# JosephCatrambone/pixelbox

Measured on NVIDIA B200. Metric: corpus_GB_per_s_scanned, higher is better.
Workload: dtype u8 x s16 -> int32 (IDP.2A), f32 replay on candidates

## Files before the change

include/pixelbox_b200.h:

```cpp
#ifndef PIXELBOX_B200_H
#define PIXELBOX_B200_H

#include <stddef.h>
#include <stdint.h>

#ifdef __cplusplus
extern "C" {
#endif

#if defined(_WIN32)
#define PBX_API __declspec(dllexport)
#else
#define PBX_API __attribute__((visibility("default")))
#endif

#define PBX_OK 0
#define PBX_E_INVALID (-1)
#define PBX_E_DIM (-2)
#define PBX_E_OOM (-3)
#define PBX_E_CUDA (-4)
#define PBX_E_NO_DEVICE (-5)
#define PBX_E_CAPACITY (-6)
#define PBX_E_K (-7)
#define PBX_E_INTERNAL (-8)

#define PBX_MAX_DIM 4096u
#define PBX_MAX_K 2048u
#define PBX_MAX_ROWS 0xFFFFF000ull
#define PBX_MAX_SHARDS 64u

#define PBX_COUNT_EXCHANGE_TIMEOUT 0xFFFFFFFFu
#define PBX_COUNT_EXACT_LAUNCH_FAILED 0xFFFFFFFEu
#define PBX_COUNT_FILTER_UNSORTED 0xFFFFFFFDu

#define PBX_FILTER_INCLUDE 0u
#define PBX_FILTER_EXCLUDE 1u

#define PBX_DEFAULT_MAX_DIST 1e3
#define PBX_DEFAULT_K 100u

typedef struct pbx_corpus pbx_corpus;

typedef struct pbx_hit {
    int64_t image_id;
    float dist;
    int32_t dot;
    int32_t norm2;
    uint32_t flags;
} pbx_hit;

typedef struct pbx_stats {
    uint64_t rows;
    uint64_t capacity_rows;
    uint32_t dim;
    uint32_t row_pitch;
    uint64_t queries;
    uint64_t exact_passes;
    float last_search_ms;
    float last_scan_ms;
    uint64_t last_bytes_scanned;
    int32_t device;
    int32_t sm_count;
    int32_t scan_grid;
    int32_t reserved;
    uint64_t batched_queries;
} pbx_stats;

PBX_API int pbx_corpus_create(uint32_t dim, uint64_t capacity_hint, int device, pbx_corpus** out);
PBX_API void pbx_corpus_destroy(pbx_corpus* c);

PBX_API int pbx_corpus_load(pbx_corpus* c, const int64_t* image_ids, const uint8_t* hashes, uint64_t n);

PBX_API int pbx_corpus_append(pbx_corpus* c, const int64_t* image_ids, const uint8_t* hashes, uint64_t n);
PBX_API int pbx_corpus_flush(pbx_corpus* c);
PBX_API int pbx_corpus_append_device(pbx_corpus* c, const int64_t* d_image_ids, const uint8_t* d_hashes, uint64_t n, void* cuda_stream);

PBX_API int pbx_corpus_remove(pbx_corpus* c, const int64_t* image_ids, uint64_t n, uint64_t* out_removed);

PBX_API int pbx_corpus_fill_synthetic(pbx_corpus* c, uint64_t n, uint64_t seed, uint64_t first_row);

PBX_API int pbx_corpus_size(const pbx_corpus* c, uint64_t* n_rows);
PBX_API int pbx_corpus_dim(const pbx_corpus* c, uint32_t* dim);

PBX_API int pbx_corpus_read_rows(const pbx_corpus* c, uint64_t first, uint64_t n, int64_t* image_ids, uint8_t* hashes);

PBX_API int pbx_corpus_synchronize(pbx_corpus* c);

PBX_API int pbx_search(pbx_corpus* c, const uint8_t* queries, uint32_t nq, uint32_t k, double max_dist,
                       int64_t* out_ids, float* out_dist, int32_t* out_dot, int32_t* out_norm2,
                       uint32_t* out_count);

PBX_API int pbx_search_hits(pbx_corpus* c, const uint8_t* queries, uint32_t nq, uint32_t k, double max_dist,
                            pbx_hit* out_hits, uint32_t* out_count);

PBX_API int pbx_search_device(pbx_corpus* c, const uint8_t* d_queries, uint32_t nq, uint32_t k, double max_dist,
                              pbx_hit* d_hits, uint32_t* d_count, void* cuda_stream);

PBX_API int pbx_search_filtered(pbx_corpus* c, const uint8_t* queries, uint32_t nq, uint32_t k, double max_dist,
                                int64_t* out_ids, float* out_dist, int32_t* out_dot, int32_t* out_norm2, uint32_t* out_count,
                                const int64_t* filter_ids, uint64_t n_filter, uint32_t filter_mode);
PBX_API int pbx_search_device_filtered(pbx_corpus* c, const uint8_t* d_queries, uint32_t nq, uint32_t k, double max_dist,
                                       pbx_hit* d_hits, uint32_t* d_count, void* cuda_stream,
                                       const int64_t* d_filter_ids, uint64_t n_filter, uint32_t filter_mode);

PBX_API int pbx_merge_hits(const pbx_hit* gathered, const uint32_t* counts, uint32_t n_shards, uint32_t nq, uint32_t k,
                           pbx_hit* out_hits, uint32_t* out_count);

PBX_API int pbx_merge_hits_device(int device, const pbx_hit* d_gathered, const uint32_t* d_counts, uint32_t n_shards,
                                  uint32_t nq, uint32_t k, pbx_hit* d_out_hits, uint32_t* d_out_count, void* cuda_stream);

typedef struct pbx_sharded pbx_sharded;
PBX_API int pbx_sharded_create(uint32_t dim, uint64_t capacity_hint, const int* devices, int n_devices, pbx_sharded** out);
PBX_API void pbx_sharded_destroy(pbx_sharded* s);
PBX_API int pbx_sharded_load(pbx_sharded* s, const int64_t* image_ids, const uint8_t* hashes, uint64_t n);
PBX_API int pbx_sharded_append(pbx_sharded* s, const int64_t* image_ids, const uint8_t* hashes, uint64_t n);
PBX_API int pbx_sharded_remove(pbx_sharded* s, const int64_t* image_ids, uint64_t n, uint64_t* out_removed);
PBX_API int pbx_sharded_fill_synthetic(pbx_sharded* s, uint64_t rows_per_shard, uint64_t seed);
PBX_API int pbx_sharded_size(const pbx_sharded* s, uint64_t* n_rows);
PBX_API int pbx_sharded_shards(const pbx_sharded* s, uint32_t* n_shards);
PBX_API int pbx_sharded_shard(pbx_sharded* s, uint32_t index, pbx_corpus** out);
PBX_API int pbx_sharded_search(pbx_sharded* s, const uint8_t* queries, uint32_t nq, uint32_t k, double max_dist,
                               int64_t* out_ids, float* out_dist, int32_t* out_dot, int32_t* out_norm2, uint32_t* out_count);
PBX_API int pbx_sharded_search_hits(pbx_sharded* s, const uint8_t* queries, uint32_t nq, uint32_t k, double max_dist,
                                    pbx_hit* out_hits, uint32_t* out_count);
PBX_API int pbx_sharded_search_filtered(pbx_sharded* s, const uint8_t* queries, uint32_t nq, uint32_t k, double max_dist,
                                        int64_t* out_ids, float* out_dist, int32_t* out_dot, int32_t* out_norm2, uint32_t* out_count,
                                        const int64_t* filter_ids, uint64_t n_filter, uint32_t filter_mode);

typedef struct pbx_exchange pbx_exchange;
PBX_API int pbx_exchange_create(int device, uint32_t rank, uint32_t world, uint32_t max_records, uint32_t max_queries,
                                pbx_exchange** out);
PBX_API int pbx_exchange_handle(pbx_exchange* x, void* out_handle_64_bytes);
PBX_API int pbx_exchange_connect(pbx_exchange* x, const void* all_handles );
PBX_API int pbx_exchange_allgather_merge(pbx_exchange* x, const pbx_hit* d_local, uint32_t nq, uint32_t k, pbx_hit* d_out,
                                         uint32_t* d_out_count, void* cuda_stream);
PBX_API int pbx_exchange_search_hits(pbx_exchange* x, pbx_corpus* c, const uint8_t* queries, uint32_t nq, uint32_t k, double max_dist,
                                     pbx_hit* out_hits, uint32_t* out_count);
PBX_API int pbx_exchange_search_hits_filtered(pbx_exchange* x, pbx_corpus* c, const uint8_t* queries, uint32_t nq, uint32_t k,
                                              double max_dist, pbx_hit* out_hits, uint32_t* out_count,
                                              const int64_t* filter_ids, uint64_t n_filter, uint32_t filter_mode);
PBX_API void pbx_exchange_destroy(pbx_exchange* x);

PBX_API int pbx_cosine_distance_pairs(int device, const uint8_t* a, const uint8_t* b, uint64_t n, uint32_t dim,
                                      float* out_dist, int32_t* out_dot, int32_t* out_norm2_a, int32_t* out_norm2_b);

PBX_API int pbx_byte_distance_pairs(int device, const uint8_t* a, const uint8_t* b, uint64_t n, uint32_t dim,
                                    float* out_dist, uint32_t* out_l1);
PBX_API int pbx_hamming_distance_pairs(int device, const uint8_t* a, const uint8_t* b, uint64_t n, uint32_t dim,
                                       float* out_dist, uint32_t* out_bits);

PBX_API int pbx_quantize(int device, const float* embeddings, uint64_t n, uint8_t* out);
PBX_API int pbx_quantize_device(int device, const float* d_embeddings, uint64_t n, uint8_t* d_out, void* cuda_stream);

PBX_API int pbx_get_stats(const pbx_corpus* c, pbx_stats* out);
PBX_API int pbx_set_candidate_slack(pbx_corpus* c, uint32_t slack);
PBX_API int pbx_set_profiling(pbx_corpus* c, int enabled);
PBX_API int pbx_set_batch_min(pbx_corpus* c, uint32_t min_queries);
PBX_API int pbx_set_scan_ctas_per_sm(pbx_corpus* c, uint32_t ctas_per_sm);
PBX_API int pbx_int8_peak(int device, double* out_tops);
PBX_API const char* pbx_last_error(void);
PBX_API const char* pbx_version(void);
PBX_API int pbx_device_count(void);

#ifdef __cplusplus
}
#endif
#endif
```

pixelbox_b200/_native.py:

```python
from __future__ import annotations

import ctypes
import os

import numpy as np

HERE = os.path.dirname(os.path.abspath(__file__))
SO_PATH = os.environ.get("PBX_SO", os.path.join(HERE, "lib", "libpixelbox_b200.so"))

PBX_OK = 0
ERROR_NAMES = {
    -1: "PBX_E_INVALID", -2: "PBX_E_DIM", -3: "PBX_E_OOM", -4: "PBX_E_CUDA", -5: "PBX_E_NO_DEVICE",
    -6: "PBX_E_CAPACITY", -7: "PBX_E_K", -8: "PBX_E_INTERNAL",
}
PBX_MAX_DIM = 4096
PBX_MAX_K = 2048
DEFAULT_MAX_DIST = 1e3
DEFAULT_K = 100
PBX_FILTER_INCLUDE = 0
PBX_FILTER_EXCLUDE = 1
PBX_COUNT_FILTER_UNSORTED = 0xFFFFFFFD

EXPORTS = [
    "pbx_corpus_create", "pbx_corpus_destroy", "pbx_corpus_load", "pbx_corpus_append", "pbx_corpus_flush", "pbx_corpus_append_device",
    "pbx_quantize_device", "pbx_corpus_fill_synthetic", "pbx_corpus_remove", "pbx_sharded_remove",
    "pbx_corpus_size", "pbx_corpus_dim", "pbx_corpus_read_rows", "pbx_corpus_synchronize", "pbx_search", "pbx_search_hits", "pbx_search_device",
    "pbx_search_filtered", "pbx_search_device_filtered", "pbx_sharded_search_filtered", "pbx_exchange_search_hits_filtered",
    "pbx_merge_hits", "pbx_merge_hits_device", "pbx_exchange_create", "pbx_exchange_handle", "pbx_exchange_connect",
    "pbx_exchange_allgather_merge", "pbx_exchange_search_hits", "pbx_exchange_destroy",
    "pbx_sharded_create", "pbx_sharded_destroy", "pbx_sharded_load", "pbx_sharded_append", "pbx_sharded_fill_synthetic", "pbx_sharded_size",
    "pbx_sharded_shards", "pbx_sharded_shard", "pbx_sharded_search", "pbx_sharded_search_hits", "pbx_cosine_distance_pairs", "pbx_byte_distance_pairs", "pbx_hamming_distance_pairs", "pbx_quantize", "pbx_get_stats", "pbx_set_candidate_slack",
    "pbx_set_profiling", "pbx_set_batch_min", "pbx_set_scan_ctas_per_sm", "pbx_int8_peak", "pbx_last_error", "pbx_version", "pbx_device_count",
]

HIT_DTYPE = np.dtype([("image_id", "<i8"), ("dist", "<f4"), ("dot", "<i4"), ("norm2", "<i4"), ("flags", "<u4")], align=True)
assert HIT_DTYPE.itemsize == 24


class PbxStats(ctypes.Structure):
    _fields_ = [
        ("rows", ctypes.c_uint64), ("capacity_rows", ctypes.c_uint64), ("dim", ctypes.c_uint32),
        ("row_pitch", ctypes.c_uint32), ("queries", ctypes.c_uint64), ("exact_passes", ctypes.c_uint64),
        ("last_search_ms", ctypes.c_float), ("last_scan_ms", ctypes.c_float), ("last_bytes_scanned", ctypes.c_uint64),
        ("device", ctypes.c_int32), ("sm_count", ctypes.c_int32), ("scan_grid", ctypes.c_int32), ("reserved", ctypes.c_int32),
        ("batched_queries", ctypes.c_uint64),
    ]


class PbxError(RuntimeError):
    def __init__(self, code: int, message: str):
        self.code = code
        self.name = ERROR_NAMES.get(code, f"PBX_E_{code}")
        super().__init__(f"{self.name}: {message}")


_lib = None


def lib() -> ctypes.CDLL:
    global _lib
    if _lib is not None:
        return _lib
    if not os.path.exists(SO_PATH):
        raise ImportError(f"{SO_PATH} is missing: build it with `python -m pixelbox_b200.build` "
                          "(nvcc, sm_100a). pixelbox_b200 has no CPU or PyTorch fallback.")
    L = ctypes.CDLL(SO_PATH)
    vp, u8p = ctypes.c_void_p, ctypes.c_void_p
    u32, u64, i32, f64 = ctypes.c_uint32, ctypes.c_uint64, ctypes.c_int, ctypes.c_double
    sig = {
        "pbx_corpus_create": (i32, [u32, u64, i32, ctypes.POINTER(vp)]),
        "pbx_corpus_destroy": (None, [vp]),
        "pbx_corpus_load": (i32, [vp, vp, u8p, u64]),
        "pbx_corpus_append": (i32, [vp, vp, u8p, u64]),
        "pbx_corpus_flush": (i32, [vp]),
        "pbx_corpus_append_device": (i32, [vp, vp, vp, u64, vp]),
        "pbx_quantize_device": (i32, [i32, vp, u64, vp, vp]),
        "pbx_corpus_fill_synthetic": (i32, [vp, u64, u64, u64]),
        "pbx_corpus_remove": (i32, [vp, vp, u64, ctypes.POINTER(u64)]),
        "pbx_sharded_remove": (i32, [vp, vp, u64, ctypes.POINTER(u64)]),
        "pbx_corpus_size": (i32, [vp, ctypes.POINTER(u64)]),
        "pbx_corpus_dim": (i32, [vp, ctypes.POINTER(u32)]),
        "pbx_corpus_read_rows": (i32, [vp, u64, u64, vp, u8p]),
        "pbx_corpus_synchronize": (i32, [vp]),
        "pbx_search": (i32, [vp, u8p, u32, u32, f64, vp, vp, vp, vp, vp]),
        "pbx_search_hits": (i32, [vp, u8p, u32, u32, f64, vp, vp]),
        "pbx_search_device": (i32, [vp, vp, u32, u32, f64, vp, vp, vp]),
        "pbx_search_filtered": (i32, [vp, u8p, u32, u32, f64, vp, vp, vp, vp, vp, vp, u64, u32]),
        "pbx_search_device_filtered": (i32, [vp, vp, u32, u32, f64, vp, vp, vp, vp, u64, u32]),
        "pbx_merge_hits": (i32, [vp, vp, u32, u32, u32, vp, vp]),
        "pbx_merge_hits_device": (i32, [i32, vp, vp, u32, u32, u32, vp, vp, vp]),
        "pbx_exchange_create": (i32, [i32, u32, u32, u32, u32, ctypes.POINTER(vp)]),
        "pbx_exchange_handle": (i32, [vp, vp]),
        "pbx_exchange_connect": (i32, [vp, vp]),
        "pbx_exchange_allgather_merge": (i32, [vp, vp, u32, u32, vp, vp, vp]),
        "pbx_exchange_search_hits": (i32, [vp, vp, u8p, u32, u32, f64, vp, vp]),
        "pbx_exchange_search_hits_filtered": (i32, [vp, vp, u8p, u32, u32, f64, vp, vp, vp, u64, u32]),
        "pbx_exchange_destroy": (None, [vp]),
        "pbx_sharded_create": (i32, [u32, u64, vp, i32, ctypes.POINTER(vp)]),
        "pbx_sharded_destroy": (None, [vp]),
        "pbx_sharded_load": (i32, [vp, vp, u8p, u64]),
        "pbx_sharded_append": (i32, [vp, vp, u8p, u64]),
        "pbx_sharded_fill_synthetic": (i32, [vp, u64, u64]),
        "pbx_sharded_size": (i32, [vp, ctypes.POINTER(u64)]),
        "pbx_sharded_shards": (i32, [vp, ctypes.POINTER(u32)]),
        "pbx_sharded_shard": (i32, [vp, u32, ctypes.POINTER(vp)]),
        "pbx_sharded_search": (i32, [vp, u8p, u32, u32, f64, vp, vp, vp, vp, vp]),
        "pbx_sharded_search_hits": (i32, [vp, u8p, u32, u32, f64, vp, vp]),
        "pbx_sharded_search_filtered": (i32, [vp, u8p, u32, u32, f64, vp, vp, vp, vp, vp, vp, u64, u32]),
        "pbx_cosine_distance_pairs": (i32, [i32, u8p, u8p, u64, u32, vp, vp, vp, vp]),
        "pbx_byte_distance_pairs": (i32, [i32, u8p, u8p, u64, u32, vp, vp]),
        "pbx_hamming_distance_pairs": (i32, [i32, u8p, u8p, u64, u32, vp, vp]),
        "pbx_quantize": (i32, [i32, vp, u64, u8p]),
        "pbx_get_stats": (i32, [vp, ctypes.POINTER(PbxStats)]),
        "pbx_set_candidate_slack": (i32, [vp, u32]),
        "pbx_set_profiling": (i32, [vp, i32]),
        "pbx_set_batch_min": (i32, [vp, u32]),
        "pbx_set_scan_ctas_per_sm": (i32, [vp, u32]),
        "pbx_int8_peak": (i32, [i32, ctypes.POINTER(ctypes.c_double)]),
        "pbx_last_error": (ctypes.c_char_p, []),
        "pbx_version": (ctypes.c_char_p, []),
        "pbx_device_count": (i32, []),
    }
    for name, (res, args) in sig.items():
        fn = getattr(L, name)
        fn.restype = res
        fn.argtypes = args
    _lib = L
    return L


def check(rc: int) -> None:
    if rc != PBX_OK:
        raise PbxError(rc, lib().pbx_last_error().decode("utf-8", "replace"))


def filter_args(within, excluding):
    if within is not None and excluding is not None:
        raise ValueError("pass `within` or `excluding`, not both")
    ids = within if within is not None else excluding
    ids = np.ascontiguousarray(np.asarray(ids, dtype=np.int64)).reshape(-1)
    return ids, (PBX_FILTER_INCLUDE if within is not None else PBX_FILTER_EXCLUDE)


def ptr(a) -> ctypes.c_void_p:
    if a is None:
        return ctypes.c_void_p(0)
    return ctypes.c_void_p(a.ctypes.data)
```

pixelbox_b200/csrc/api.cu:

```cuda
#include <atomic>
#include <algorithm>
#include <cmath>
#include <cstdarg>
#include <cstdio>
#include <cstdlib>
#include <cstring>
#include <limits>
#include <mutex>
#include <new>
#include <type_traits>
#include <vector>

#include "finalize.cuh"
#include "batch.cuh"
#include "remove.cuh"

using namespace pbx;

static thread_local char g_err[512] = "";

static int fail(int code, const char* fmt, ...) {
    va_list ap;
    va_start(ap, fmt);
    vsnprintf(g_err, sizeof(g_err), fmt, ap);
    va_end(ap);
    return code;
}

#define CU_TRY(expr)                                                                               \
    do {                                                                                           \
        cudaError_t e__ = (expr);                                                                  \
        if (e__ != cudaSuccess)                                                                    \
            return fail(e__ == cudaErrorMemoryAllocation ? PBX_E_OOM : PBX_E_CUDA, "%s failed: %s (%s:%d)", #expr, \
                        cudaGetErrorString(e__), __FILE__, __LINE__);                              \
    } while (0)

struct VmmApi {
    CUresult (*reserve)(CUdeviceptr*, size_t, size_t, CUdeviceptr, unsigned long long) = nullptr;
    CUresult (*free_)(CUdeviceptr, size_t) = nullptr;
    CUresult (*create)(CUmemGenericAllocationHandle*, size_t, const CUmemAllocationProp*, unsigned long long) = nullptr;
    CUresult (*release)(CUmemGenericAllocationHandle) = nullptr;
    CUresult (*map)(CUdeviceptr, size_t, size_t, CUmemGenericAllocationHandle, unsigned long long) = nullptr;
    CUresult (*unmap)(CUdeviceptr, size_t) = nullptr;
    CUresult (*set_access)(CUdeviceptr, size_t, const CUmemAccessDesc*, size_t) = nullptr;
    CUresult (*granularity)(size_t*, const CUmemAllocationProp*, CUmemAllocationGranularity_flags) = nullptr;
    bool ok = false;
};
static const VmmApi& vmm_api() {
    static VmmApi api;
    static std::once_flag once;
    std::call_once(once, [] {
        if (getenv("PBX_NO_VMM")) return;
        cudaDriverEntryPointQueryResult q;
        auto get = [&](const char* name, void** fn) { return cudaGetDriverEntryPoint(name, fn, cudaEnableDefault, &q) == cudaSuccess && *fn != nullptr; };
        api.ok = get("cuMemAddressReserve", (void**)&api.reserve) && get("cuMemAddressFree", (void**)&api.free_) && get("cuMemCreate", (void**)&api.create) &&
                 get("cuMemRelease", (void**)&api.release) && get("cuMemMap", (void**)&api.map) && get("cuMemUnmap", (void**)&api.unmap) &&
                 get("cuMemSetAccess", (void**)&api.set_access) && get("cuMemGetAllocationGranularity", (void**)&api.granularity);
        cudaGetLastError();
    });
    return api;
}
struct VmmArray {
    CUdeviceptr base = 0;
    size_t reserved = 0, mapped = 0, gran = 0;
    std::vector<std::pair<CUmemGenericAllocationHandle, size_t>> chunks;
};
static CUmemAllocationProp vmm_prop(int device) {
    CUmemAllocationProp prop = {};
    prop.type = CU_MEM_ALLOCATION_TYPE_PINNED;
    prop.location.type = CU_MEM_LOCATION_TYPE_DEVICE;
    prop.location.id = device;
    return prop;
}
static bool vmm_reserve(VmmArray& a, int device, size_t bytes) {
    const VmmApi& api = vmm_api();
    const CUmemAllocationProp prop = vmm_prop(device);
    if (api.granularity(&a.gran, &prop, CU_MEM_ALLOC_GRANULARITY_RECOMMENDED) != CUDA_SUCCESS || a.gran == 0) return false;
    a.reserved = (bytes + a.gran - 1) / a.gran * a.gran;
    return api.reserve(&a.base, a.reserved, 0, 0, 0) == CUDA_SUCCESS;
}
static int vmm_grow(VmmArray& a, int device, size_t need, size_t* from, size_t* to) {
    *from = *to = a.mapped;
    if (need <= a.mapped) return PBX_OK;
    if (need > a.reserved) return fail(PBX_E_CAPACITY, "shard outgrew the address range reserved for it (%zu > %zu bytes)", need, a.reserved);
    const VmmApi& api = vmm_api();
    const size_t add = (need - a.mapped + a.gran - 1) / a.gran * a.gran;
    const CUmemAllocationProp prop = vmm_prop(device);
    CUmemGenericAllocationHandle h;
    CUresult r = api.create(&h, add, &prop, 0);
    if (r != CUDA_SUCCESS) return fail(PBX_E_OOM, "cannot back %zu more bytes on device %d (cuMemCreate: %d)", add, device, (int)r);
    r = api.map(a.base + a.mapped, add, 0, h, 0);
    if (r == CUDA_SUCCESS) {
        CUmemAccessDesc acc = {};
        acc.location.type = CU_MEM_LOCATION_TYPE_DEVICE;
        acc.location.id = device;
        acc.flags = CU_MEM_ACCESS_FLAGS_PROT_READWRITE;
        r = api.set_access(a.base + a.mapped, add, &acc, 1);
        if (r != CUDA_SUCCESS) api.unmap(a.base + a.mapped, add);
    }
    if (r != CUDA_SUCCESS) { api.release(h); return fail(PBX_E_CUDA, "mapping %zu bytes failed (%d)", add, (int)r); }
    a.chunks.emplace_back(h, add);
    *to = a.mapped + add;
    a.mapped += add;
    return PBX_OK;
}
static void vmm_release(VmmArray& a) {
    const VmmApi& api = vmm_api();
    if (a.base) {
        if (a.mapped) api.unmap(a.base, a.mapped);
        for (auto& c : a.chunks) api.release(c.first);
        api.free_(a.base, a.reserved);
    }
    a = VmmArray();
}

struct pbx_corpus {
    int device = 0;
    int sm_count = 0;
    uint32_t dim = 0, pitch = 0, pitch16 = 0;
    std::atomic<uint64_t> n{0};
    std::atomic<uint64_t> capacity{0};
    uint8_t* d_rows = nullptr;
    float* d_inv = nullptr;
    int* d_rsum = nullptr;
    float4* d_bmeta = nullptr;
    bool use_vmm = false;
    VmmArray v_rows, v_inv, v_rsum, v_ids, v_bmeta;
    uint64_t reserved_rows = 0;
    std::vector<uint8_t> pend_rows;
    std::vector<int64_t> pend_ids;
    std::atomic<uint64_t> pending{0};
    int64_t* d_ids = nullptr;

    cudaStream_t stream = nullptr;
    cudaStream_t copy_stream = nullptr;
    cudaEvent_t ev_chain = nullptr;
    cudaEvent_t ev_t0 = nullptr, ev_t1 = nullptr;
    cudaEvent_t ev_s0 = nullptr, ev_s1 = nullptr;
    float last_scan_ms = 0.f;
    bool chain_valid = false;

    uint32_t max_nq = 0;
    uint8_t* d_queries = nullptr;
    int16_t* d_q16 = nullptr;
    uint8_t* d_qbytes = nullptr;
    QueryHeader* d_qh = nullptr;
    SearchStatus* d_status = nullptr;
    unsigned char* d_split = nullptr;
    bool split_finalize = true;
    size_t split_min_bytes = 256u * 1024u;
    pbx_hit* d_hits = nullptr;
    size_t hits_cap = 0;
    void* d_cand = nullptr;
    size_t cand_bytes = 0;
    uint32_t* d_cand_cnt = nullptr;
    uint32_t* d_tile_counter = nullptr;
    uint32_t* d_hist = nullptr;
    unsigned long long* d_exact_passes = nullptr;
    uint32_t* d_allow = nullptr;
    size_t allow_words = 0;
    u64* d_filter_words = nullptr;
    int64_t* d_filter_ids = nullptr;
    size_t filter_ids_cap = 0;
    const uint32_t* cur_allow = nullptr;
    const u64* cur_allowed = nullptr;
    uint8_t* h_queries = nullptr;
    size_t h_queries_cap = 0;
    pbx_hit* h_hits = nullptr;
    size_t h_hits_cap = 0;
    bool zero_copy = true;
    uint32_t* h_flag = nullptr;
    uint32_t flag_seq = 0;
    uint32_t* cur_done_flag = nullptr;
    uint32_t cur_done_seq = 0;
    uint8_t* h_stage = nullptr;
    size_t h_stage_cap = 0, stage_rows = 0;
    cudaEvent_t ev_stage[2] = {nullptr, nullptr};

    std::mutex mu;
    std::mutex append_mu;
    std::mutex grow_mu;
    cudaStream_t grow_stream = nullptr;

    uint32_t slack = 0;
    uint32_t ctas_per_sm = 0;
    uint64_t queries = 0;
    float last_search_ms = 0.f;
    uint64_t last_bytes = 0;
    int last_grid = 0;
    uint32_t last_n = 0;
    uint64_t rows_generation = 0;
    uint32_t batch_pad = 0;
    uint8_t* d_qpad = nullptr;
    int* d_colterm = nullptr;
    float* d_thr = nullptr;
    uint32_t* d_bcnt = nullptr;
    uint32_t* d_boverflow = nullptr;
    u64* d_bcand = nullptr;
    uint32_t batch_cap = 0;
    uint32_t* d_bhist = nullptr;
    float* d_binvq = nullptr;
    float* d_seedlb = nullptr;
    CUtensorMap map_rows, map_q;
    uint64_t map_rows_gen = ~0ull;
    uint32_t map_q_pad = 0, map_q_box = 0, map_rows_box = 0;
    uint32_t batch_cg = 0;

    uint32_t batch_min = 2;
    uint64_t batched_queries = 0;
    bool scan_timed = false;
    bool profiling = false;
};

constexpr size_t kStageMinRows = 2048;
static int ensure_stage(pbx_corpus* c, size_t rows_per_slot);

static uint32_t default_keep(uint32_t k, uint32_t slack) {
    uint32_t s = slack ? slack : std::max<uint32_t>(156u, k / 4u);
    uint32_t keep = k + s;
    if (!slack) keep = (keep + 31u) & ~31u;
    return std::min<uint32_t>(keep, kMaxKeep);
}

static uint32_t batch_keep(uint32_t k, uint32_t slack) {
    if (slack) return std::min<uint32_t>(k + slack, kMaxKeep);
    const uint32_t keep = (k + std::max<uint32_t>(28u, k / 4u) + 31u) & ~31u;
    return std::min<uint32_t>(keep, kMaxKeep);
}

static float certificate_margin(uint32_t dim) {
    return (float)((4.0 * dim + 3232.0) * std::ldexp(1.0, -24));
}

static int free_corpus_buffers(pbx_corpus* c) {
    if (c->use_vmm) {
        vmm_release(c->v_rows); vmm_release(c->v_inv); vmm_release(c->v_rsum); vmm_release(c->v_ids); vmm_release(c->v_bmeta);
        c->d_rows = nullptr; c->d_inv = nullptr; c->d_ids = nullptr; c->d_rsum = nullptr; c->d_bmeta = nullptr;
        c->capacity = 0;
        c->use_vmm = false;
        return PBX_OK;
    }
    cudaFree(c->d_rows); cudaFree(c->d_inv); cudaFree(c->d_ids); cudaFree(c->d_rsum); cudaFree(c->d_bmeta);
    c->d_rows = nullptr; c->d_inv = nullptr; c->d_ids = nullptr; c->d_rsum = nullptr; c->d_bmeta = nullptr;
    c->capacity = 0;
    return PBX_OK;
}

static int reserve_rows_vmm(pbx_corpus* c, uint64_t want) {
    struct Arr { VmmArray* a; size_t elem; } arrs[5] = {{&c->v_rows, (size_t)c->pitch}, {&c->v_inv, sizeof(float)}, {&c->v_rsum, sizeof(int)},
                                                        {&c->v_ids, sizeof(int64_t)}, {&c->v_bmeta, sizeof(float4)}};
    for (int i = 0; i < 5; ++i) {
        const size_t need = i == 4 ? (size_t)(want / 32) * arrs[i].elem : (size_t)want * arrs[i].elem;
        size_t from = 0, to = 0;
        int rc = vmm_grow(*arrs[i].a, c->device, need, &from, &to);
        if (rc != PBX_OK) return rc;
        if (to > from) CU_TRY(cudaMemsetAsync(reinterpret_cast<void*>(arrs[i].a->base + from), 0, to - from, c->grow_stream));
    }
    CU_TRY(cudaStreamSynchronize(c->grow_stream));
    c->capacity = want;
    return PBX_OK;
}

static int reserve_rows(pbx_corpus* c, uint64_t rows) {
    if (rows <= c->capacity) return PBX_OK;
    if (rows > PBX_MAX_ROWS) return fail(PBX_E_CAPACITY, "shard would hold %llu rows (max %llu)", (unsigned long long)rows, (unsigned long long)PBX_MAX_ROWS);
    const uint64_t cap_now = c->capacity.load();
    uint64_t want = std::max<uint64_t>(rows, cap_now + cap_now / 2);
    if (cap_now) want = std::max<uint64_t>(want, cap_now + (32u << 20) / c->pitch);
    want = (want + kTileRows - 1) / kTileRows * kTileRows;
    if (c->use_vmm) {
        want = std::min<uint64_t>(want, c->reserved_rows);
        if (rows > c->reserved_rows) return fail(PBX_E_CAPACITY, "shard would hold %llu rows; its address range was reserved for %llu", (unsigned long long)rows, (unsigned long long)c->reserved_rows);
        int rc = reserve_rows_vmm(c, want);
        if (rc != PBX_OK && want > rows) {
            want = (rows + kTileRows - 1) / kTileRows * kTileRows;
            rc = reserve_rows_vmm(c, want);
        }
        return rc;
    }
    uint8_t* nr = nullptr; float* ni = nullptr; int64_t* nid = nullptr; int* ns = nullptr; float4* nb = nullptr;
    auto alloc_all = [&](uint64_t rows_) {
        cudaError_t e_ = cudaMalloc(&nr, rows_ * c->pitch);
        if (e_ == cudaSuccess) e_ = cudaMalloc(&ni, rows_ * sizeof(float));
        if (e_ == cudaSuccess) e_ = cudaMalloc(&nid, rows_ * sizeof(int64_t));
        if (e_ == cudaSuccess) e_ = cudaMalloc(&ns, rows_ * sizeof(int));
        if (e_ == cudaSuccess) e_ = cudaMalloc(&nb, rows_ / 32 * sizeof(float4));
        return e_;
    };
    auto free_all = [&]() {
        cudaFree(nr); cudaFree(ni); cudaFree(nid); cudaFree(ns); cudaFree(nb);
        nr = nullptr; ni = nullptr; nid = nullptr; ns = nullptr; nb = nullptr;
        cudaGetLastError();
    };
    cudaError_t e = alloc_all(want);
    if (e != cudaSuccess && want > rows) {
        free_all();
        want = (rows + kTileRows - 1) / kTileRows * kTileRows;
        e = alloc_all(want);
    }
    if (e != cudaSuccess) {
        free_all();
        return fail(PBX_E_OOM, "cannot allocate %llu rows x %u bytes on device %d: %s", (unsigned long long)want, c->pitch, c->device, cudaGetErrorString(e));
    }
    const uint64_t n = c->n.load();
    e = cudaDeviceSynchronize();
    if (e == cudaSuccess && n) {
        e = cudaMemcpyAsync(nr, c->d_rows, n * c->pitch, cudaMemcpyDeviceToDevice, c->stream);
        if (e == cudaSuccess) e = cudaMemcpyAsync(ni, c->d_inv, n * sizeof(float), cudaMemcpyDeviceToDevice, c->stream);
        if (e == cudaSuccess) e = cudaMemcpyAsync(nid, c->d_ids, n * sizeof(int64_t), cudaMemcpyDeviceToDevice, c->stream);
        if (e == cudaSuccess) e = cudaMemcpyAsync(ns, c->d_rsum, n * sizeof(int), cudaMemcpyDeviceToDevice, c->stream);
    }
// ... 47 lines not shown
        CU_TRY(cudaMalloc(&c->d_hits, need * sizeof(pbx_hit)));
        c->hits_cap = need;
    }
    if (need > c->h_hits_cap) {
        cudaFreeHost(c->h_hits);
        c->h_hits = nullptr; c->h_hits_cap = 0;
        CU_TRY(cudaMallocHost(&c->h_hits, need * sizeof(pbx_hit)));
        c->h_hits_cap = need;
    }
    return PBX_OK;
}

static int ensure_cand(pbx_corpus* c, size_t bytes) {
    if (bytes <= c->cand_bytes) return PBX_OK;
    CU_TRY(cudaDeviceSynchronize());
    cudaFree(c->d_cand); c->d_cand = nullptr; c->cand_bytes = 0;
    CU_TRY(cudaMalloc(&c->d_cand, bytes));
    c->cand_bytes = bytes;
    return PBX_OK;
}

static int ensure_filter_scratch(pbx_corpus* c, size_t words, uint64_t n_ids) {
    if (!c->d_filter_words) CU_TRY(cudaMalloc(&c->d_filter_words, 2 * sizeof(u64)));
    if (words > c->allow_words) {
        words = std::max(words, c->allow_words + c->allow_words / 2);
        CU_TRY(cudaDeviceSynchronize());
        cudaFree(c->d_allow); c->d_allow = nullptr; c->allow_words = 0;
        CU_TRY(cudaMalloc(&c->d_allow, words * sizeof(uint32_t)));
        c->allow_words = words;
    }
    if (n_ids > c->filter_ids_cap) {
        const uint64_t want = std::max<uint64_t>(n_ids, c->filter_ids_cap + c->filter_ids_cap / 2);
        CU_TRY(cudaDeviceSynchronize());
        cudaFree(c->d_filter_ids); c->d_filter_ids = nullptr; c->filter_ids_cap = 0;
        CU_TRY(cudaMalloc(&c->d_filter_ids, want * sizeof(int64_t)));
        c->filter_ids_cap = want;
    }
    return PBX_OK;
}

template <typename Kern>
static cudaError_t allow_smem(Kern kern, size_t bytes) {
    return cudaFuncSetAttribute(kern, cudaFuncAttributeMaxDynamicSharedMemorySize, (int)bytes);
}
constexpr uint64_t kBatchMaxRows = 0x7FFFF000ull;
constexpr uint32_t kBatchSegTilesLarge = 98304;
constexpr uint32_t kBatchSeedTiles = 256;
constexpr size_t kBatchSmemLimit = 232448 - 1024;
static cudaError_t init_kernel_attributes() {
    const size_t scan_cap = 8192 * sizeof(KeyX) + PBX_MAX_DIM * 2 + 1024;
    const size_t fin_cap = 200 * 1024;
    cudaError_t e = cudaSuccess;
#define PBX_ALLOW(LL, CC)                                                                                       \
    if (e == cudaSuccess) e = allow_smem(scan_kernel<LL, CC, false>, scan_cap);                                 \
    if (e == cudaSuccess) e = allow_smem(scan_kernel<LL, CC, false, scan_minb(LL * CC), false, true>, scan_cap); \
    if (e == cudaSuccess) e = allow_smem(scan_kernel<LL, CC, true>, scan_cap);
    PBX_ALLOW(1, 1) PBX_ALLOW(2, 1) PBX_ALLOW(4, 1) PBX_ALLOW(8, 1) PBX_ALLOW(16, 1) PBX_ALLOW(32, 1) PBX_ALLOW(32, 2) PBX_ALLOW(32, 4)
#undef PBX_ALLOW
#define PBX_ALLOW_M(LL, CC, MM)                                                                   \
    if (e == cudaSuccess) e = allow_smem(scan_kernel<LL, CC, false, MM>, scan_cap);               \
    if (e == cudaSuccess) e = allow_smem(scan_kernel<LL, CC, false, MM, false, true>, scan_cap);  \
    if (e == cudaSuccess) e = allow_smem(scan_kernel<LL, CC, true, MM>, scan_cap);
    PBX_EXTRA_SHAPES(PBX_ALLOW_M)
#undef PBX_ALLOW_M
#define PBX_ALLOW_R(LL, CC, MM)                                                                  \
    if (e == cudaSuccess) e = allow_smem(scan_kernel<LL, CC, false, MM, true>, scan_cap);        \
    if (e == cudaSuccess) e = allow_smem(scan_kernel<LL, CC, false, MM, true, true>, scan_cap);
    PBX_RAGGED_SHAPES(PBX_ALLOW_R)
#undef PBX_ALLOW_R
    if (e == cudaSuccess) e = allow_smem(scan_kernel<16, 1, false, 3>, scan_cap);
    if (e == cudaSuccess) e = allow_smem(scan_kernel<16, 1, false, 4>, scan_cap);
    if (e == cudaSuccess) e = allow_smem(scan_kernel<16, 1, false, 3, false, true>, scan_cap);
    if (e == cudaSuccess) e = allow_smem(scan_kernel<16, 1, false, 4, false, true>, scan_cap);
    if (e == cudaSuccess) e = allow_smem(scan_generic_kernel<false>, scan_cap);
    if (e == cudaSuccess) e = allow_smem(scan_generic_kernel<true>, scan_cap);
    if (e == cudaSuccess) e = allow_smem(prep_seed_kernel, PBX_MAX_DIM * 2 + 1024);
    if (e == cudaSuccess) e = allow_smem(finalize_kernel<false>, fin_cap);
    if (e == cudaSuccess) e = allow_smem(replay_kernel, (size_t)PBX_MAX_DIM * 6 + (size_t)kReplayRows * (kReplaySlice16 + 2) * 16);
    if (e == cudaSuccess) e = allow_smem(finalize_kernel<true>, fin_cap);
    if (e == cudaSuccess) e = allow_smem(batch_mma_kernel<1, false>, kBatchSmemLimit);
    if (e == cudaSuccess) e = allow_smem(batch_mma_kernel<1, true>, kBatchSmemLimit);
    if (e == cudaSuccess) e = allow_smem(batch_mma_kernel<2, false>, kBatchSmemLimit);
    if (e == cudaSuccess) e = allow_smem(batch_mma_kernel<2, true>, kBatchSmemLimit);
    if (e == cudaSuccess) e = allow_smem(batch_finalize_kernel, batch_finalize_smem(1024));
    if (e == cudaSuccess) e = allow_smem(batch_seed_select_kernel, (size_t)kBatchSeedTiles * 8u * sizeof(u64));
    if (e == cudaSuccess) e = allow_smem(batch_tighten_kernel, kBatchCapLarge * sizeof(u64));
    if (e == cudaSuccess) e = allow_smem(finalize_exact_kernel, fin_cap);
    return e;
}

extern "C" int pbx_device_count(void) {
    int n = 0;
    if (cudaGetDeviceCount(&n) != cudaSuccess) { cudaGetLastError(); return 0; }
    int ok = 0;
    for (int d = 0; d < n; ++d) {
        int major = 0;
        if (cudaDeviceGetAttribute(&major, cudaDevAttrComputeCapabilityMajor, d) == cudaSuccess && major == 10) ok++;
    }
    return ok;
}

extern "C" const char* pbx_last_error(void) { return g_err; }
extern "C" const char* pbx_version(void) { return "pixelbox_b200 0.1.0 (sm_100a)"; }

extern "C" int pbx_corpus_create(uint32_t dim, uint64_t capacity_hint, int device, pbx_corpus** out) {
    if (!out) return fail(PBX_E_INVALID, "out is NULL");
    *out = nullptr;
    if (dim == 0 || dim > PBX_MAX_DIM) return fail(PBX_E_DIM, "dim %u outside [1, %u]", dim, PBX_MAX_DIM);
    int ndev = 0;
    if (cudaGetDeviceCount(&ndev) != cudaSuccess || ndev == 0) {
        cudaGetLastError();
        return fail(PBX_E_NO_DEVICE, "no CUDA device visible: pixelbox_b200 has no CPU fallback");
    }
    if (device < 0 || device >= ndev) return fail(PBX_E_INVALID, "device %d out of range (have %d)", device, ndev);
    int major = 0, minor = 0;
    CU_TRY(cudaDeviceGetAttribute(&major, cudaDevAttrComputeCapabilityMajor, device));
    CU_TRY(cudaDeviceGetAttribute(&minor, cudaDevAttrComputeCapabilityMinor, device));
    if (major != 10) return fail(PBX_E_NO_DEVICE, "device %d is sm_%d%d; this library is built for sm_100a (B200) only", device, major, minor);
    CU_TRY(cudaSetDevice(device));
    pbx_corpus* c = new (std::nothrow) pbx_corpus();
    if (!c) return fail(PBX_E_OOM, "host allocation failed");
    c->device = device;
    c->dim = dim;
    c->split_finalize = getenv("PBX_NO_SPLIT_FINALIZE") == nullptr;
    if (const char* e = getenv("PBX_SPLIT_MIN_BYTES")) c->split_min_bytes = (size_t)atoll(e);
    c->zero_copy = getenv("PBX_NO_ZEROCOPY") == nullptr;
    if (const char* e = getenv("PBX_BATCH_CG")) c->batch_cg = atoi(e) == 1 ? 1u : (atoi(e) == 2 ? 2u : 0u);
    c->pitch = (dim + 15u) & ~15u;
    c->pitch16 = c->pitch / 16u;
    cudaDeviceGetAttribute(&c->sm_count, cudaDevAttrMultiProcessorCount, device);
    cudaError_t e = cudaStreamCreateWithFlags(&c->stream, cudaStreamNonBlocking);
    if (e == cudaSuccess) e = cudaStreamCreateWithFlags(&c->copy_stream, cudaStreamNonBlocking);
    if (e == cudaSuccess) e = cudaStreamCreateWithFlags(&c->grow_stream, cudaStreamNonBlocking);
    if (e == cudaSuccess) e = cudaEventCreateWithFlags(&c->ev_chain, cudaEventDisableTiming);
    if (e == cudaSuccess) e = cudaEventCreate(&c->ev_t0);
    if (e == cudaSuccess) e = cudaEventCreate(&c->ev_t1);
    if (e == cudaSuccess) e = cudaEventCreate(&c->ev_s0);
    if (e == cudaSuccess) e = cudaEventCreate(&c->ev_s1);
    if (e == cudaSuccess) e = cudaEventCreateWithFlags(&c->ev_stage[0], cudaEventDisableTiming);
    if (e == cudaSuccess) e = cudaEventCreateWithFlags(&c->ev_stage[1], cudaEventDisableTiming);
    if (e == cudaSuccess) e = init_kernel_attributes();
    if (e == cudaSuccess) {
        size_t cur = 0;
        if (cudaDeviceGetLimit(&cur, cudaLimitDevRuntimePendingLaunchCount) == cudaSuccess && cur < 8192)
            e = cudaDeviceSetLimit(cudaLimitDevRuntimePendingLaunchCount, 8192);
    }
    if (e == cudaSuccess) e = cudaMallocHost(&c->h_flag, 64);
    if (e == cudaSuccess) *c->h_flag = 0;
    if (e == cudaSuccess) e = cudaMalloc(&c->d_cand_cnt, kMaxScanGrid * sizeof(uint32_t));
    if (e == cudaSuccess) e = cudaMalloc(&c->d_tile_counter, 512);
    if (e == cudaSuccess) e = cudaMemset(c->d_tile_counter, 0, 512);
    if (e == cudaSuccess) e = cudaMalloc(&c->d_hist, 2 * kHistBins * sizeof(uint32_t));
    if (e == cudaSuccess) e = cudaMemset(c->d_hist, 0, 2 * kHistBins * sizeof(uint32_t));
    if (e == cudaSuccess) { c->d_exact_passes = reinterpret_cast<unsigned long long*>(reinterpret_cast<char*>(c->d_tile_counter) + 256); }
    if (e != cudaSuccess) {
        int rc = fail(PBX_E_CUDA, "corpus setup failed: %s", cudaGetErrorString(e));
        pbx_corpus_destroy(c);
        return rc;
    }
    if (vmm_api().ok) {
        size_t free_b = 0, total_b = 0;
        cudaMemGetInfo(&free_b, &total_b);
        const uint64_t per_row = (uint64_t)c->pitch + 4 + 4 + 8 + 1;
        uint64_t max_rows = std::min<uint64_t>(PBX_MAX_ROWS, std::max<uint64_t>((uint64_t)total_b / per_row, capacity_hint) + kTileRows);
        max_rows = (max_rows + kTileRows - 1) / kTileRows * kTileRows;
        c->use_vmm = vmm_reserve(c->v_rows, device, max_rows * c->pitch) && vmm_reserve(c->v_inv, device, max_rows * sizeof(float)) &&
                     vmm_reserve(c->v_rsum, device, max_rows * sizeof(int)) && vmm_reserve(c->v_ids, device, max_rows * sizeof(int64_t)) &&
                     vmm_reserve(c->v_bmeta, device, max_rows / 32 * sizeof(float4));
        if (c->use_vmm) {
            c->reserved_rows = max_rows;
            c->d_rows = reinterpret_cast<uint8_t*>(c->v_rows.base); c->d_inv = reinterpret_cast<float*>(c->v_inv.base);
            c->d_rsum = reinterpret_cast<int*>(c->v_rsum.base); c->d_ids = reinterpret_cast<int64_t*>(c->v_ids.base);
            c->d_bmeta = reinterpret_cast<float4*>(c->v_bmeta.base);
        } else {
            vmm_release(c->v_rows); vmm_release(c->v_inv); vmm_release(c->v_rsum); vmm_release(c->v_ids); vmm_release(c->v_bmeta);
        }
    }
    {
        std::lock_guard<std::mutex> lk(c->mu);
        int rc = reserve_rows(c, std::max<uint64_t>(capacity_hint, 1));
        if (rc == PBX_OK) rc = ensure_stage(c, kStageMinRows);
        if (rc != PBX_OK) { pbx_corpus_destroy(c); return rc; }
    }
    *out = c;
    return PBX_OK;
}

extern "C" void pbx_corpus_destroy(pbx_corpus* c) {
    if (!c) return;
    cudaSetDevice(c->device);
    cudaDeviceSynchronize();
    free_corpus_buffers(c);
    cudaFree(c->d_queries); cudaFree(c->d_q16); cudaFree(c->d_qbytes); cudaFree(c->d_qh); cudaFree(c->d_status); cudaFree(c->d_split);
    cudaFree(c->d_qpad); cudaFree(c->d_colterm); cudaFree(c->d_thr); cudaFree(c->d_bcnt); cudaFree(c->d_boverflow); cudaFree(c->d_bcand);
    cudaFree(c->d_bhist); cudaFree(c->d_binvq); cudaFree(c->d_seedlb);
    cudaFree(c->d_hits); cudaFree(c->d_cand); cudaFree(c->d_cand_cnt); cudaFree(c->d_tile_counter); cudaFree(c->d_hist);
    cudaFree(c->d_allow); cudaFree(c->d_filter_words); cudaFree(c->d_filter_ids);
    cudaFreeHost(c->h_queries); cudaFreeHost(c->h_hits); cudaFreeHost(c->h_stage); cudaFreeHost(c->h_flag);
    if (c->ev_chain) cudaEventDestroy(c->ev_chain);
    if (c->ev_t0) cudaEventDestroy(c->ev_t0);
    if (c->ev_t1) cudaEventDestroy(c->ev_t1);
    if (c->ev_s0) cudaEventDestroy(c->ev_s0);
    if (c->ev_s1) cudaEventDestroy(c->ev_s1);
    if (c->ev_stage[0]) cudaEventDestroy(c->ev_stage[0]);
    if (c->ev_stage[1]) cudaEventDestroy(c->ev_stage[1]);
    if (c->stream) cudaStreamDestroy(c->stream);
    if (c->copy_stream) cudaStreamDestroy(c->copy_stream);
    if (c->grow_stream) cudaStreamDestroy(c->grow_stream);
    cudaGetLastError();
    delete c;
}

extern "C" int pbx_corpus_size(const pbx_corpus* c, uint64_t* n_rows) {
    if (!c || !n_rows) return fail(PBX_E_INVALID, "NULL argument");
    *n_rows = c->n.load() + c->pending.load(std::memory_order_acquire);
    return PBX_OK;
}
extern "C" int pbx_corpus_synchronize(pbx_corpus* c) {
    if (!c) return fail(PBX_E_INVALID, "corpus is NULL");
    CU_TRY(cudaSetDevice(c->device));
    CU_TRY(cudaStreamSynchronize(c->stream));
    return PBX_OK;
}
extern "C" int pbx_corpus_dim(const pbx_corpus* c, uint32_t* dim) {
    if (!c || !dim) return fail(PBX_E_INVALID, "NULL argument");
    *dim = c->dim;
    return PBX_OK;
}

static int ensure_stage(pbx_corpus* c, size_t rows_per_slot) {
    const size_t per_row = (size_t)c->pitch + sizeof(int64_t);
    const size_t need = rows_per_slot * per_row * 2;
    if (c->h_stage_cap >= need) return PBX_OK;
    CU_TRY(cudaStreamSynchronize(c->copy_stream));
    cudaFreeHost(c->h_stage); c->h_stage = nullptr; c->h_stage_cap = 0; c->stage_rows = 0;
    CU_TRY(cudaMallocHost(&c->h_stage, need));
    c->h_stage_cap = need;
    c->stage_rows = rows_per_slot;
    return PBX_OK;
}

static int upload_rows(pbx_corpus* c, uint64_t at, const int64_t* ids, const uint8_t* hashes, uint64_t n) {
    const size_t max_stage_rows = std::max<size_t>(kStageMinRows, (size_t)(8u << 20) / c->pitch);
    const size_t per_row = (size_t)c->pitch + sizeof(int64_t);
    {
        size_t want = kStageMinRows;
        while (want < n && want < max_stage_rows) want *= 2;
        int rc0 = ensure_stage(c, std::min(want, max_stage_rows));
        if (rc0 != PBX_OK) return rc0;
    }
    const size_t stage_rows = c->stage_rows;
    cudaEvent_t* done = c->ev_stage;
    int rc = PBX_OK;
    uint64_t off = 0;
    int slot = 0;
    bool used[2] = {false, false};
    while (off < n && rc == PBX_OK) {
        const uint64_t m = std::min<uint64_t>(stage_rows, n - off);
        uint8_t* hs = c->h_stage + (size_t)slot * stage_rows * per_row;
        int64_t* hid = reinterpret_cast<int64_t*>(hs + stage_rows * c->pitch);
        if (used[slot]) cudaEventSynchronize(done[slot]);
        if (c->pitch == c->dim) {
            memcpy(hs, hashes + off * c->dim, m * c->dim);
        } else {
            memset(hs, 0, m * c->pitch);
            for (uint64_t r = 0; r < m; ++r) memcpy(hs + r * c->pitch, hashes + (off + r) * c->dim, c->dim);
        }
        memcpy(hid, ids + off, m * sizeof(int64_t));
        cudaError_t e = cudaMemcpyAsync(c->d_rows + (at + off) * c->pitch, hs, m * c->pitch, cudaMemcpyHostToDevice, c->copy_stream);
        if (e == cudaSuccess) e = cudaMemcpyAsync(c->d_ids + at + off, hid, m * sizeof(int64_t), cudaMemcpyHostToDevice, c->copy_stream);
        if (e == cudaSuccess) {
            const unsigned warps_per_block = 8;
            const unsigned blocks = (unsigned)((m + warps_per_block - 1) / warps_per_block);
            row_meta_kernel<<<blocks, warps_per_block * 32, 0, c->copy_stream>>>(reinterpret_cast<const uint4*>(c->d_rows), c->pitch16, c->dim,
                                                                                at + off, m, c->d_inv, c->d_rsum);
            e = cudaGetLastError();
        }
        if (e == cudaSuccess) e = cudaEventRecord(done[slot], c->copy_stream);
        if (e != cudaSuccess) rc = fail(PBX_E_CUDA, "row upload failed: %s", cudaGetErrorString(e));
        used[slot] = true;
        slot ^= 1;
        off += m;
    }
    if (rc == PBX_OK && n) {
        const uint64_t b0 = at / 32, b1 = (at + n + 31) / 32;
        block_meta_kernel<<<(unsigned)((b1 - b0 + 7) / 8), 256, 0, c->copy_stream>>>(c->d_inv, c->d_rsum, c->dim, b0, b1 - b0, at + n, c->d_bmeta);
        if (cudaGetLastError() != cudaSuccess) rc = fail(PBX_E_CUDA, "block metadata launch failed");
    }
    cudaError_t e = cudaStreamSynchronize(c->copy_stream);
    if (rc == PBX_OK && e != cudaSuccess) rc = fail(PBX_E_CUDA, "row upload failed: %s", cudaGetErrorString(e));
    return rc;
}

static int append_locked(pbx_corpus* c, const int64_t* image_ids, const uint8_t* hashes, uint64_t n) {
    CU_TRY(cudaSetDevice(c->device));
    const uint64_t at = c->n.load();
    if (at + n > c->capacity) {
        int rc;
        if (c->use_vmm) {
            rc = grow_mapped(c, at + n);
        } else {
            std::lock_guard<std::mutex> lk(c->mu);
            rc = reserve_rows(c, at + n);
        }
        if (rc != PBX_OK) return rc;
    }
    int rc = upload_rows(c, at, image_ids, hashes, n);
// ... 82 lines not shown
    if (n && (!image_ids || !hashes)) return fail(PBX_E_INVALID, "NULL ids or hashes with n > 0");
    std::lock_guard<std::mutex> alk(c->append_mu);
    {
        std::lock_guard<std::mutex> lk(c->mu);
        CU_TRY(cudaSetDevice(c->device));
        CU_TRY(cudaDeviceSynchronize());
        c->n.store(0);
        c->pend_ids.clear(); c->pend_rows.clear(); c->pending.store(0);
    }
    return n ? append_locked(c, image_ids, hashes, n) : PBX_OK;
}

extern "C" int pbx_corpus_fill_synthetic(pbx_corpus* c, uint64_t n, uint64_t seed, uint64_t first_row) {
    if (!c) return fail(PBX_E_INVALID, "corpus is NULL");
    std::lock_guard<std::mutex> alk(c->append_mu);
    std::lock_guard<std::mutex> lk(c->mu);
    CU_TRY(cudaSetDevice(c->device));
    CU_TRY(cudaDeviceSynchronize());
    c->n.store(0);
    c->pend_ids.clear(); c->pend_rows.clear(); c->pending.store(0);
    int rc = c->use_vmm ? grow_mapped(c, std::max<uint64_t>(n, 1)) : reserve_rows(c, std::max<uint64_t>(n, 1));
    if (rc != PBX_OK) return rc;
    if (n == 0) return PBX_OK;
    const uint64_t step = 1ull << 24;
    for (uint64_t off = 0; off < n; off += step) {
        const uint64_t m = std::min<uint64_t>(step, n - off);
        synth_fill_kernel<<<c->sm_count * 8, 256, 0, c->stream>>>(c->d_rows, c->pitch, c->dim, off, m, seed, first_row + off, c->d_ids);
        const unsigned blocks = (unsigned)((m + 7) / 8);
        row_meta_kernel<<<blocks, 256, 0, c->stream>>>(reinterpret_cast<const uint4*>(c->d_rows), c->pitch16, c->dim, off, m, c->d_inv, c->d_rsum);
        const uint64_t b0 = off / 32, b1 = (off + m + 31) / 32;
        block_meta_kernel<<<(unsigned)((b1 - b0 + 7) / 8), 256, 0, c->stream>>>(c->d_inv, c->d_rsum, c->dim, b0, b1 - b0, off + m, c->d_bmeta);
    }
    CU_TRY(cudaGetLastError());
    CU_TRY(cudaStreamSynchronize(c->stream));
    c->n.store(n);
    return PBX_OK;
}

extern "C" int pbx_corpus_read_rows(const pbx_corpus* cc, uint64_t first, uint64_t n, int64_t* image_ids, uint8_t* hashes) {
    pbx_corpus* c = const_cast<pbx_corpus*>(cc);
    if (!c) return fail(PBX_E_INVALID, "corpus is NULL");
    { int frc = flush_pending(c); if (frc != PBX_OK) return frc; }
    const uint64_t size_now = c->n.load();
    if (n > size_now || first > size_now - n) return fail(PBX_E_INVALID, "rows [%llu, %llu) outside the corpus", (unsigned long long)first, (unsigned long long)(first + n));
    if (n == 0) return PBX_OK;
    std::lock_guard<std::mutex> lk(c->mu);
    CU_TRY(cudaSetDevice(c->device));
    if (image_ids) CU_TRY(cudaMemcpy(image_ids, c->d_ids + first, n * sizeof(int64_t), cudaMemcpyDeviceToHost));
    if (hashes) CU_TRY(cudaMemcpy2D(hashes, c->dim, c->d_rows + first * c->pitch, c->pitch, c->dim, n, cudaMemcpyDeviceToHost));
    return PBX_OK;
}

static int sorted_request(const int64_t* image_ids, uint64_t n, std::vector<int64_t>* out) {
    try { out->assign(image_ids, image_ids + n); } catch (...) { return fail(PBX_E_OOM, "host allocation failed"); }
    if (!std::is_sorted(out->begin(), out->end())) std::sort(out->begin(), out->end());
    out->erase(std::unique(out->begin(), out->end()), out->end());
    return PBX_OK;
}

static int remove_sorted(pbx_corpus* c, const std::vector<int64_t>& req, uint64_t* out_removed) {
    std::lock_guard<std::mutex> alk(c->append_mu);
    int rc = flush_pending_locked(c);
    if (rc != PBX_OK) return rc;
    std::lock_guard<std::mutex> lk(c->mu);
    CU_TRY(cudaSetDevice(c->device));
    const uint64_t n = c->n.load();
    if (n == 0 || req.empty()) return PBX_OK;
    cudaStream_t s = c->copy_stream;
    if (c->chain_valid) CU_TRY(cudaStreamWaitEvent(s, c->ev_chain, 0));
    const uint64_t tiles = (n + kRemoveTileRows - 1) / kRemoveTileRows;
    const size_t req_bytes = req.size() * sizeof(int64_t), flag_bytes = (n + 31) / 32 * sizeof(uint32_t);
    const size_t off_cnt = (req_bytes + 15) / 16 * 16, off_flags = off_cnt + 16, off_tiles = off_flags + (flag_bytes + 15) / 16 * 16;
    unsigned char* scratch = nullptr;
    uint32_t* pairs = nullptr;
    CU_TRY(cudaMallocAsync(reinterpret_cast<void**>(&scratch), off_tiles + 2 * tiles * sizeof(uint32_t), s));
    int64_t* d_req = reinterpret_cast<int64_t*>(scratch);
    u64* d_removed = reinterpret_cast<u64*>(scratch + off_cnt);
    uint32_t* d_pairs = reinterpret_cast<uint32_t*>(scratch + off_cnt + 8);
    uint32_t* d_flags = reinterpret_cast<uint32_t*>(scratch + off_flags);
    uint32_t* d_tile_holes = reinterpret_cast<uint32_t*>(scratch + off_tiles);
    uint32_t* d_tile_srcs = d_tile_holes + tiles;
    u64 m = 0;
    cudaError_t e = cudaMemcpyAsync(d_req, req.data(), req_bytes, cudaMemcpyHostToDevice, s);
    if (e == cudaSuccess) e = cudaMemsetAsync(d_removed, 0, sizeof(u64), s);
    if (e == cudaSuccess) {
        mark_ids_kernel<<<(unsigned)tiles, kRemoveTileRows, 0, s>>>(c->d_ids, n, d_req, req.size(), 0u, d_flags, d_removed);
        e = cudaGetLastError();
    }
    if (e == cudaSuccess) e = cudaMemcpyAsync(&m, d_removed, sizeof(u64), cudaMemcpyDeviceToHost, s);
    if (e == cudaSuccess) e = cudaStreamSynchronize(s);
    if (e == cudaSuccess && m > n) { cudaFreeAsync(scratch, s); cudaStreamSynchronize(s); return fail(PBX_E_INTERNAL, "removal counted %llu of %llu rows", (unsigned long long)m, (unsigned long long)n); }
    const uint64_t n_keep = n - m;
    const uint64_t max_pairs = std::min<uint64_t>(m, n_keep);
    if (e == cudaSuccess && max_pairs) e = cudaMallocAsync(reinterpret_cast<void**>(&pairs), 2 * max_pairs * sizeof(uint32_t), s);
    if (e == cudaSuccess && max_pairs) {
        uint32_t* d_holes = pairs;
        uint32_t* d_srcs = pairs + max_pairs;
        remove_count_kernel<<<(unsigned)tiles, kRemoveTileRows, 0, s>>>(d_flags, n, n_keep, d_tile_holes, d_tile_srcs);
        remove_scan_kernel<<<1, 1024, 0, s>>>(d_tile_holes, d_tile_srcs, (uint32_t)tiles, d_pairs);
        remove_place_kernel<<<(unsigned)tiles, kRemoveTileRows, 0, s>>>(d_flags, n, n_keep, d_tile_holes, d_tile_srcs, d_holes, d_srcs);
        const uint64_t chunks = max_pairs * c->pitch16;
        const unsigned grid = (unsigned)std::min<uint64_t>((chunks + 255) / 256, (uint64_t)c->sm_count * 8);
        remove_move_kernel<<<grid, 256, 0, s>>>(d_holes, d_srcs, d_pairs, c->pitch16, reinterpret_cast<uint4*>(c->d_rows), c->d_ids, c->d_inv, c->d_rsum);
        e = cudaGetLastError();
    }
    if (e == cudaSuccess && m && n_keep) {
        const uint64_t blocks = (n_keep + 31) / 32;
        block_meta_kernel<<<(unsigned)((blocks + 7) / 8), 256, 0, s>>>(c->d_inv, c->d_rsum, c->dim, 0, blocks, n_keep, c->d_bmeta);
        e = cudaGetLastError();
    }
    if (pairs) cudaFreeAsync(pairs, s);
    cudaFreeAsync(scratch, s);
    const cudaError_t e2 = cudaStreamSynchronize(s);
    if (e == cudaSuccess) e = e2;
    if (e != cudaSuccess) return fail(PBX_E_CUDA, "removal failed: %s", cudaGetErrorString(e));
    c->n.store(n_keep);
    if (out_removed) *out_removed = m;
    return PBX_OK;
}

extern "C" int pbx_corpus_remove(pbx_corpus* c, const int64_t* image_ids, uint64_t n, uint64_t* out_removed) {
    if (out_removed) *out_removed = 0;
    if (!c) return fail(PBX_E_INVALID, "corpus is NULL");
    if (n && !image_ids) return fail(PBX_E_INVALID, "NULL image_ids with n > 0");
    if (n == 0) return PBX_OK;
    std::vector<int64_t> req;
    int rc = sorted_request(image_ids, n, &req);
    return rc == PBX_OK ? remove_sorted(c, req, out_removed) : rc;
}

__global__ void empty_result_kernel(pbx_hit* hits, uint32_t* counts, uint32_t nq, uint32_t k) {
    const uint32_t total = nq * k;
    for (uint32_t i = blockIdx.x * blockDim.x + threadIdx.x; i < total; i += gridDim.x * blockDim.x) {
        pbx_hit h; h.image_id = INT64_MAX; h.dist = __int_as_float(0x7f800000); h.dot = 0; h.norm2 = 0; h.flags = 0;
        hits[i] = h;
    }
    for (uint32_t i = blockIdx.x * blockDim.x + threadIdx.x; i < nq; i += gridDim.x * blockDim.x) counts[i] = 0;
}

template <typename P>
static cudaError_t launch_pdl(void (*kern)(const P), int grid, int block, size_t smem, cudaStream_t s, const P& params) {
    cudaLaunchConfig_t cfg = {};
    cfg.gridDim = dim3((unsigned)grid);
    cfg.blockDim = dim3((unsigned)block);
    cfg.dynamicSmemBytes = smem;
    cfg.stream = s;
    cudaLaunchAttribute attr[1];
    attr[0].id = cudaLaunchAttributeProgrammaticStreamSerialization;
    attr[0].val.programmaticStreamSerializationAllowed = 1;
    cfg.attrs = attr;
    cfg.numAttrs = 1;
    return cudaLaunchKernelEx(&cfg, kern, params);
}

template <bool EXACT, bool FILTER>
static cudaError_t launch_scan_as(const pbx_corpus* c, const ScanParams& p, int grid, size_t smem, cudaStream_t s) {
    static_assert(!(EXACT && FILTER), "the exact pass has no FILTER instantiation");
#define PBX_SCAN_CASE(LL, CC)                                                                                                     \
    {                                                                                                                             \
        return launch_pdl<ScanParams>(scan_kernel<LL, CC, EXACT, scan_minb(LL * CC), false, FILTER>, grid, kScanThreads, smem, s, p); \
    }
    switch (c->pitch16) {
        case 1: PBX_SCAN_CASE(1, 1)
        case 2: PBX_SCAN_CASE(2, 1)
        case 4: PBX_SCAN_CASE(4, 1)
        case 8: PBX_SCAN_CASE(8, 1)
        case 16:
            if constexpr (!EXACT) {
                if (c->ctas_per_sm == 3 || c->ctas_per_sm == 0) return launch_pdl<ScanParams>(scan_kernel<16, 1, false, 3, false, FILTER>, grid, kScanThreads, smem, s, p);
                if (c->ctas_per_sm >= 4) return launch_pdl<ScanParams>(scan_kernel<16, 1, false, 4, false, FILTER>, grid, kScanThreads, smem, s, p);
            }
            PBX_SCAN_CASE(16, 1)
        case 32: PBX_SCAN_CASE(32, 1)
        case 64: PBX_SCAN_CASE(32, 2)
        case 128: PBX_SCAN_CASE(32, 4)
#define PBX_SCAN_CASE_M(LL, CC, MM) case (LL) * (CC): return launch_pdl<ScanParams>(scan_kernel<LL, CC, EXACT, MM, false, FILTER>, grid, kScanThreads, smem, s, p);
        PBX_EXTRA_SHAPES(PBX_SCAN_CASE_M)
#undef PBX_SCAN_CASE_M
        default: {
            if constexpr (!EXACT) {
#define PBX_SCAN_CASE_R(LL, CC, MM) \
    if (c->pitch16 <= (LL) * (CC)) return launch_pdl<ScanParams>(scan_kernel<LL, CC, false, MM, true, FILTER>, grid, kScanThreads, smem, s, p);
                PBX_RAGGED_SHAPES(PBX_SCAN_CASE_R)
#undef PBX_SCAN_CASE_R
            }
            size_t sm = smem + (size_t)c->pitch16 * 32;
            return launch_pdl<ScanParams>(scan_generic_kernel<EXACT>, grid, kScanThreads, sm, s, p);
        }
    }
#undef PBX_SCAN_CASE
}

template <bool EXACT>
static cudaError_t launch_scan(const pbx_corpus* c, const ScanParams& p, int grid, size_t smem, cudaStream_t s) {
    if constexpr (!EXACT) {
        if (p.allow) return launch_scan_as<false, true>(c, p, grid, smem, s);
    }
    return launch_scan_as<EXACT, false>(c, p, grid, smem, s);
}

static bool fast_shape(uint32_t pitch16) {
    if ((pitch16 & (pitch16 - 1)) == 0 && pitch16 <= 256) return true;
#define PBX_IS_SHAPE(LL, CC, MM) if (pitch16 == (LL) * (CC)) return true;
    PBX_EXTRA_SHAPES(PBX_IS_SHAPE)
#undef PBX_IS_SHAPE
    return false;
}

static int scan_grid(const pbx_corpus* c) {
    const bool pow2 = (c->pitch16 & (c->pitch16 - 1)) == 0;
    uint32_t per_sm = c->ctas_per_sm ? c->ctas_per_sm
                      : c->pitch16 >= 256          ? 1u
                      : (c->pitch16 > 128 && !fast_shape(c->pitch16)) ? 1u
                      : (c->pitch16 < 8 && !pow2)  ? 4u
                      : !pow2                      ? 2u
                      : (c->pitch16 == 16 || c->pitch16 == 4) ? 3u : (c->pitch16 > 16) ? 2u : 4u;
    int g = c->sm_count * (int)per_sm;
    return std::min<int>(g, (int)kMaxScanGrid);
}

typedef CUresult (*EncodeTiledFn)(CUtensorMap*, CUtensorMapDataType, cuuint32_t, void*, const cuuint64_t*, const cuuint64_t*,
                                  const cuuint32_t*, const cuuint32_t*, CUtensorMapInterleave, CUtensorMapSwizzle,
                                  CUtensorMapL2promotion, CUtensorMapFloatOOBfill);

static EncodeTiledFn encode_tiled_fn() {
    static EncodeTiledFn fn = nullptr;
    if (!fn) {
        void* p = nullptr;
        cudaDriverEntryPointQueryResult qres;
        if (cudaGetDriverEntryPoint("cuTensorMapEncodeTiled", &p, cudaEnableDefault, &qres) == cudaSuccess) fn = (EncodeTiledFn)p;
    }
    return fn;
}

static int make_u8_map(CUtensorMap* m, void* base, uint64_t rows, uint32_t pitch, uint32_t w, uint32_t box_rows) {
    EncodeTiledFn enc = encode_tiled_fn();
    if (!enc) return fail(PBX_E_CUDA, "cuTensorMapEncodeTiled is not available from this driver");
    cuuint64_t dims[2] = {(cuuint64_t)pitch, (cuuint64_t)rows};
    cuuint64_t strides[1] = {(cuuint64_t)pitch};
    cuuint32_t box[2] = {w, box_rows};
    cuuint32_t estr[2] = {1, 1};
    const CUtensorMapSwizzle sw = w == 128 ? CU_TENSOR_MAP_SWIZZLE_128B : (w == 64 ? CU_TENSOR_MAP_SWIZZLE_64B : CU_TENSOR_MAP_SWIZZLE_32B);
    CUresult r = enc(m, CU_TENSOR_MAP_DATA_TYPE_UINT8, 2, base, dims, strides, box, estr, CU_TENSOR_MAP_INTERLEAVE_NONE, sw,
                     CU_TENSOR_MAP_L2_PROMOTION_L2_256B, CU_TENSOR_MAP_FLOAT_OOB_FILL_NONE);
    if (r != CUDA_SUCCESS) return fail(PBX_E_CUDA, "cuTensorMapEncodeTiled failed (%d)", (int)r);
    return PBX_OK;
}

struct BatchPlan {
    uint32_t cg;
    uint32_t tn;
    uint32_t w, kc;
    uint32_t qg;
    uint32_t groups;
    uint32_t nq_pad;
    uint32_t stages;
    size_t smem;
    int grid;
};

static bool batch_plan(const pbx_corpus* c, uint32_t nq, uint32_t cg, BatchPlan* out) {
    BatchPlan bp;
    const uint32_t pitch = c->pitch;
    if (pitch % 32 != 0 || pitch > 1024) return false;
    bp.cg = cg;
    bp.tn = 256u;
    bp.w = pitch % 128 == 0 ? 128u : (pitch % 64 == 0 ? 64u : 32u);
    bp.kc = pitch / bp.w;
    const uint32_t stage_bytes = (bp.tn / bp.cg) * bp.w;
    uint32_t want = ((nq + bp.cg - 1) / bp.cg + 127u) / 128u * 128u;
    uint32_t qg = std::min<uint32_t>(std::min<uint32_t>(want, kBatchMaxQG), std::max<uint32_t>(128u, (128u * 1024u / pitch) / 128u * 128u));
    for (;; qg -= 128) {
        const size_t fixed = 1024 + (size_t)qg * pitch + batch_smem_fixed(qg, bp.tn);
        if (fixed < kBatchSmemLimit) {
            const uint32_t stages = (uint32_t)std::min<size_t>(kBatchMaxStages, (kBatchSmemLimit - fixed) / stage_bytes);
            const uint32_t need = qg > 128 ? bp.kc + 1 : 2u;
            if (stages >= need) {
                bp.qg = qg; bp.stages = stages; bp.smem = fixed + (size_t)stages * stage_bytes;
                break;
            }
        }
        if (qg == 128) return false;
    }
    bp.groups = (nq + bp.cg * bp.qg - 1) / (bp.cg * bp.qg);
    bp.nq_pad = bp.groups * bp.cg * bp.qg;
    const uint32_t clusters = std::max<uint32_t>(bp.groups, ((uint32_t)c->sm_count / bp.cg) / bp.groups * bp.groups);
    bp.grid = (int)(clusters * bp.cg);
    *out = bp;
    return true;
}

static uint32_t batch_cap_for(uint32_t keep) { return keep * 8u <= kBatchCap ? kBatchCap : kBatchCapLarge; }

static void batch_seed_geometry(uint32_t n, uint32_t tn, uint32_t* n_tiles, uint32_t* step) {
    const uint32_t full = n / tn;
    *n_tiles = std::min<uint32_t>(full, kBatchSeedTiles);
    *step = *n_tiles ? full / *n_tiles : 1u;
}

static bool batch_choose(const pbx_corpus* c, uint32_t nq, uint32_t n, uint32_t keep, BatchPlan* out) {
    const uint32_t first = c->batch_cg ? c->batch_cg : (nq <= 128u ? 1u : 2u);
    const uint32_t order[2] = {first, 3u - first};
    for (int i = 0; i < (c->batch_cg ? 1 : 2); ++i) {
        BatchPlan bp;
        if (!batch_plan(c, nq, order[i], &bp)) continue;
        if (!c->batch_cg && i == 0 && order[i] == 1u && bp.stages < 4u) continue;
        uint32_t seed_tiles, seed_step;
        batch_seed_geometry(n, bp.tn, &seed_tiles, &seed_step);
        if (seed_tiles * (bp.tn / 32u) < keep + keep / 2u) continue;
        *out = bp;
        return true;
    }
    return false;
}

static bool batch_eligible(const pbx_corpus* c, uint32_t nq, uint32_t n, uint32_t k) {
    const uint32_t keep = batch_keep(k, c->slack);
    BatchPlan bp;
    return nq >= c->batch_min && keep * 8u <= kBatchCapLarge && n <= kBatchMaxRows && batch_choose(c, std::min<uint32_t>(nq, 1024u), n, keep, &bp);
}

static int ensure_batch_scratch(pbx_corpus* c, uint32_t nq_pad, uint32_t cap) {
    if (nq_pad <= c->batch_pad && cap <= c->batch_cap) return PBX_OK;
    nq_pad = std::max(nq_pad, c->batch_pad);
    cap = std::max(cap, c->batch_cap);
    CU_TRY(cudaDeviceSynchronize());
    cudaFree(c->d_qpad); cudaFree(c->d_colterm); cudaFree(c->d_thr); cudaFree(c->d_bcnt); cudaFree(c->d_boverflow); cudaFree(c->d_bcand);
    cudaFree(c->d_bhist); cudaFree(c->d_binvq); c->d_bhist = nullptr; c->d_binvq = nullptr;
    c->d_qpad = nullptr; c->d_colterm = nullptr; c->d_thr = nullptr; c->d_bcnt = nullptr; c->d_boverflow = nullptr; c->d_bcand = nullptr;
    c->batch_pad = 0; c->map_q_pad = 0; c->batch_cap = 0;
    CU_TRY(cudaMalloc(&c->d_qpad, (size_t)nq_pad * c->pitch));
    CU_TRY(cudaMalloc(&c->d_colterm, (size_t)nq_pad * sizeof(int)));
    CU_TRY(cudaMalloc(&c->d_thr, (size_t)nq_pad * sizeof(float)));
    CU_TRY(cudaMalloc(&c->d_bcnt, (size_t)nq_pad * sizeof(uint32_t)));
    CU_TRY(cudaMalloc(&c->d_boverflow, (size_t)nq_pad * sizeof(uint32_t)));
    CU_TRY(cudaMalloc(&c->d_bcand, (size_t)nq_pad * cap * sizeof(u64)));
    CU_TRY(cudaMalloc(&c->d_bhist, (size_t)nq_pad * kBatchHistBins * sizeof(uint32_t)));
    CU_TRY(cudaMalloc(&c->d_binvq, (size_t)nq_pad * sizeof(float)));
    cudaFree(c->d_seedlb); c->d_seedlb = nullptr;
    CU_TRY(cudaMalloc(&c->d_seedlb, (size_t)kBatchSeedTiles * 8u * nq_pad * sizeof(float)));
    c->batch_pad = nq_pad;
    c->batch_cap = cap;
    return PBX_OK;
}

static bool finalize_stage_layout(size_t avail_bytes, uint32_t keep, uint32_t pitch16, uint32_t* group, uint32_t* slice16, size_t* bytes) {
    uint32_t g = std::min<uint32_t>(keep, (uint32_t)kFinalThreads);
    if (g == 0) g = 1;
    while (g > 32 && avail_bytes / g < 48) g /= 2;
    if (avail_bytes / g < 48) return false;
    const uint32_t s16 = (uint32_t)std::min<size_t>(pitch16, (avail_bytes / g - 32) / 16);
// ... 137 lines not shown
        BatchFinalizeParams fp;
        memset(&fp, 0, sizeof(fp));
        fp.x = exact_launch(xs);
        fp.bcand = c->d_bcand; fp.bcnt = c->d_bcnt; fp.boverflow = c->d_boverflow; fp.bticket = c->d_tile_counter + 100;
        fp.bcap = cap; fp.nq = nq; fp.keep = keep; fp.k = k; fp.n = n; fp.n_allowed = c->cur_allowed; fp.dim = c->dim; fp.pitch = pitch;
        fp.rows = c->d_rows; fp.ids = c->d_ids; fp.qbytes = c->d_qbytes; fp.q16 = c->d_q16; fp.qh = c->d_qh;
        fp.max_dist = max_dist; fp.margin = certificate_margin(c->dim);
        fp.hits = d_hits; fp.count = d_count; fp.status = c->d_status;
        batch_finalize_kernel<<<nq, (keep + 31u) & ~31u, batch_finalize_smem(pitch), s>>>(fp);
        CU_TRY(cudaGetLastError());
    } else {
        const uint32_t chunk = kFinalThreads;
        const uint32_t cap_merge = std::max<uint32_t>(next_pow2(keep + chunk), kBatchCap);
        const size_t off_sorted = (size_t)cap_merge * sizeof(u64);
        const size_t off_dots = 2 * off_sorted;
        const size_t off_q = (off_dots + (size_t)keep * 20 + 15) & ~(size_t)15;
        const size_t off_stage = (off_q + (size_t)pitch * 6 + 15) & ~(size_t)15;
        const size_t fin_budget = 200 * 1024;
        uint32_t stage_rows = 0, slice16 = 0;
        size_t stage_bytes = 0;
        if (off_stage >= fin_budget || !finalize_stage_layout(fin_budget - off_stage, keep, pitch / 16, &stage_rows, &slice16, &stage_bytes))
            return fail(PBX_E_INTERNAL, "finalize layout does not fit shared memory (k=%u dim=%u)", k, c->dim);
        const size_t fin_smem = off_stage + stage_bytes;
        FinalizeParams fp;
        memset(&fp, 0, sizeof(fp));
        fp.grid = (uint32_t)grid_scan; fp.keep = keep; fp.cap = cap_merge; fp.chunk = chunk; fp.k = k; fp.n = n; fp.n_allowed = c->cur_allowed;
        fp.dim = c->dim; fp.pitch = pitch; fp.stage_rows = stage_rows; fp.slice16 = slice16;
        fp.off_sorted = (uint32_t)off_sorted; fp.off_ent = 0; fp.off_dots = (uint32_t)off_dots; fp.off_q = (uint32_t)off_q; fp.off_stage = (uint32_t)off_stage;
        fp.rows = c->d_rows; fp.ids = c->d_ids; fp.qbytes = c->d_qbytes; fp.q16 = c->d_q16; fp.qh = c->d_qh;
        fp.max_dist = max_dist; fp.margin = certificate_margin(c->dim);
        fp.hits = d_hits; fp.count = d_count; fp.status = c->d_status; fp.tile_counter = c->d_tile_counter;
        fp.hist = c->d_hist; fp.cand = nullptr; fp.cand_cnt = nullptr;
        fp.bcand = c->d_bcand; fp.bcnt = c->d_bcnt; fp.boverflow = c->d_boverflow; fp.bticket = c->d_tile_counter + 100;
        fp.bcap = cap; fp.nq = nq;
        fp.x = exact_launch(xs);
        finalize_kernel<true><<<nq, kFinalThreads, fin_smem, s>>>(fp);
        CU_TRY(cudaGetLastError());
    }
#ifndef PBX_USE_CDP
    {
        std::vector<SearchStatus> hs(nq);
        CU_TRY(cudaStreamSynchronize(s));
        CU_TRY(cudaMemcpy(hs.data(), c->d_status, (size_t)nq * sizeof(SearchStatus), cudaMemcpyDeviceToHost));
        for (uint32_t q = 0; q < nq; ++q) {
            if (!hs[q].need_exact) continue;
            const ExactSetup xq = exact_setup(c, q, k, max_dist, n, d_hits, d_count);
            CU_TRY(launch_scan<true>(c, xq.scan, xq.grid, xq.scan_smem, s));
            finalize_exact_kernel<<<1, kFinalThreads, xq.fin_smem, s>>>(xq.fin);
            CU_TRY(cudaGetLastError());
        }
    }
#endif
    c->batched_queries += nq;
    c->last_grid = bp.grid;
    return PBX_OK;
}

struct SearchFilter {
    const int64_t* ids;
    uint64_t n;
    uint32_t mode;
    bool device;
};

static int check_filter_args(const int64_t* ids, uint64_t n, uint32_t mode) {
    if (n && !ids) return fail(PBX_E_INVALID, "filter_ids is NULL with n_filter = %llu", (unsigned long long)n);
    if (mode != PBX_FILTER_INCLUDE && mode != PBX_FILTER_EXCLUDE) return fail(PBX_E_INVALID, "unknown filter mode %u", mode);
    if (n > PBX_MAX_ROWS) return fail(PBX_E_INVALID, "n_filter = %llu exceeds PBX_MAX_ROWS", (unsigned long long)n);
    return PBX_OK;
}

static int host_filter(const int64_t* ids, uint64_t n, uint32_t mode, std::vector<int64_t>* sorted, SearchFilter* f, const SearchFilter** out) {
    *out = nullptr;
    int rc = check_filter_args(ids, n, mode);
    if (rc != PBX_OK) return rc;
    if (mode == PBX_FILTER_EXCLUDE && n == 0) return PBX_OK;
    if (n) { rc = sorted_request(ids, n, sorted); if (rc != PBX_OK) return rc; }
    f->ids = sorted->data(); f->n = sorted->size(); f->mode = mode; f->device = false;
    *out = f;
    return PBX_OK;
}

static int enqueue_filter_mark(pbx_corpus* c, const SearchFilter& f, uint32_t n, cudaStream_t s) {
    const size_t words = ((size_t)n + kTileRows - 1) / kTileRows * kTileRows / 32;
    int rc = ensure_filter_scratch(c, std::max<size_t>(words, 1), f.device ? 0 : f.n);
    if (rc != PBX_OK) return rc;
    const int64_t* d_set = f.ids;
    if (!f.device && f.n) {
        CU_TRY(cudaMemcpyAsync(c->d_filter_ids, f.ids, f.n * sizeof(int64_t), cudaMemcpyHostToDevice, s));
        d_set = c->d_filter_ids;
    }
    CU_TRY(cudaMemsetAsync(c->d_filter_words, 0, 2 * sizeof(u64), s));
    if (f.device && f.n > 1) {
        const unsigned blocks = (unsigned)std::min<uint64_t>((f.n + 255) / 256, (uint64_t)c->sm_count * 8);
        ids_unsorted_kernel<<<blocks, 256, 0, s>>>(d_set, f.n, reinterpret_cast<uint32_t*>(c->d_filter_words + 1));
        CU_TRY(cudaGetLastError());
    }
    if (n) {
        mark_ids_kernel<<<(n + kMarkTileRows - 1) / kMarkTileRows, kMarkTileRows, 0, s>>>(c->d_ids, n, d_set, f.n,
                                                                                       f.mode == PBX_FILTER_EXCLUDE ? 1u : 0u, c->d_allow, c->d_filter_words);
        CU_TRY(cudaGetLastError());
    }
    c->cur_allow = c->d_allow;
    c->cur_allowed = c->d_filter_words;
    return PBX_OK;
}

static int enqueue_search(pbx_corpus* c, const uint8_t* d_queries, uint32_t nq, uint32_t k, double max_dist, pbx_hit* d_hits,
                          uint32_t* d_count, cudaStream_t s, bool timed, uint32_t* done_flag = nullptr, uint32_t done_seq = 0,
                          const SearchFilter* filter = nullptr) {
    const uint32_t n = (uint32_t)c->n.load();
    c->cur_done_flag = done_flag; c->cur_done_seq = done_seq;
    c->cur_allow = nullptr; c->cur_allowed = nullptr;
    c->last_n = n;
    c->scan_timed = false;
    if (c->chain_valid) CU_TRY(cudaStreamWaitEvent(s, c->ev_chain, 0));
    if (timed) CU_TRY(cudaEventRecord(c->ev_t0, s));
    if (filter) {
        int rc = enqueue_filter_mark(c, *filter, n, s);
        if (rc != PBX_OK) return rc;
    }
    if (n == 0) {
        empty_result_kernel<<<64, 256, 0, s>>>(d_hits, d_count, nq, k);
        CU_TRY(cudaGetLastError());
    } else if (batch_eligible(c, nq, n, k)) {
        for (uint32_t q0 = 0; q0 < nq; q0 += 1024) {
            const uint32_t b = std::min<uint32_t>(1024u, nq - q0);
            int rc = enqueue_search_batched(c, d_queries + (size_t)q0 * c->dim, b, k, max_dist, d_hits + (size_t)q0 * k, d_count + q0, s, n);
            if (rc != PBX_OK) return rc;
        }
    } else {
        int rc = ensure_query_scratch(c, nq);
        if (rc != PBX_OK) return rc;
        const int grid = scan_grid(c);
        const uint32_t keep = std::min<uint32_t>(default_keep(k, c->slack), kMaxKeep);
        const uint32_t cap_scan = next_pow2(keep + 2 * kTileRows);
        const int seed_grid = c->sm_count;
        const bool seeded = (uint64_t)n >= (uint64_t)seed_grid * kSeedThreads * 8;
        const uint32_t chunk = std::min<uint32_t>(4u, std::max<uint32_t>(1u, (2u * (uint32_t)grid + kFinalThreads - 1) / kFinalThreads)) * kFinalThreads;
        const uint32_t cap_merge = next_pow2(keep + chunk);
        rc = ensure_cand(c, (size_t)std::max<uint32_t>(keep, k) * grid * sizeof(KeyX));
        if (rc != PBX_OK) return rc;
        const float margin = certificate_margin(c->dim);
        const size_t off_sorted = (size_t)cap_merge * sizeof(u64);
        const size_t off_dots = 2 * off_sorted;
        const size_t off_q = (off_dots + (size_t)keep * 20 + 15) & ~(size_t)15;
        const size_t off_stage = (off_q + (size_t)c->pitch * 6 + 15) & ~(size_t)15;
        const size_t fin_budget = 200 * 1024;
        uint32_t stage_rows = 0, slice16 = 0;
        size_t stage_bytes = 0;
        if (off_stage >= fin_budget || !finalize_stage_layout(fin_budget - off_stage, keep, c->pitch16, &stage_rows, &slice16, &stage_bytes))
            return fail(PBX_E_INTERNAL, "finalize layout does not fit shared memory (k=%u dim=%u)", k, c->dim);
        const size_t fin_smem = off_stage + stage_bytes;

        for (uint32_t q = 0; q < nq; ++q) {
            ScanParams sp;
            sp.rows = reinterpret_cast<const uint4*>(c->d_rows);
            sp.inv_norm = c->d_inv;
            sp.ids = c->d_ids;
            sp.n = n;
            sp.pitch16 = c->pitch16;
            sp.dim = c->dim;
            sp.q16 = c->d_q16 + (size_t)q * c->pitch;
            sp.qbytes = c->d_qbytes + (size_t)q * c->pitch;
            sp.qh = c->d_qh + q;
            sp.keep = keep;
            sp.cap = cap_scan;
            sp.cand = c->d_cand;
            sp.cand_cnt = c->d_cand_cnt;
            sp.tile_counter = c->d_tile_counter;
            sp.hist = c->d_hist;
            sp.status = c->d_status + q;
            sp.max_dist = max_dist;
            sp.allow = c->cur_allow;
            {
                PrepSeedParams ps;
                ps.query = d_queries + (size_t)q * c->dim;
                ps.dim = c->dim; ps.pitch = c->pitch; ps.pitch16 = c->pitch16;
                ps.q16 = c->d_q16 + (size_t)q * c->pitch;
                ps.qbytes = c->d_qbytes + (size_t)q * c->pitch;
                ps.qh = c->d_qh + q;
                ps.rows = sp.rows; ps.inv_norm = sp.inv_norm; ps.n = n; ps.keep = keep;
                ps.do_seed = seeded ? 1u : 0u;
                ps.seed_hist = c->d_hist + kHistBins; ps.ticket = c->d_tile_counter + 96; ps.gbin = c->d_tile_counter + 32;
                ps.allow = c->cur_allow;
                CU_TRY(launch_pdl<PrepSeedParams>(prep_seed_kernel, seeded ? seed_grid : 1, kSeedThreads, (size_t)c->pitch * 2, s, ps));
            }
            const bool time_scan = timed && q + 1 == nq;
            if (time_scan) CU_TRY(cudaEventRecord(c->ev_s0, s));
            CU_TRY(launch_scan<false>(c, sp, grid, (size_t)cap_scan * sizeof(u64), s));
            if (time_scan) { CU_TRY(cudaEventRecord(c->ev_s1, s)); c->scan_timed = true; }

            FinalizeParams fp;
            fp.cand = reinterpret_cast<const u64*>(c->d_cand);
            fp.cand_cnt = c->d_cand_cnt;
            fp.grid = (uint32_t)grid;
            fp.keep = keep;
            fp.cap = cap_merge;
            fp.k = k;
            fp.n = n;
            fp.n_allowed = c->cur_allowed;
            fp.dim = c->dim;
            fp.pitch = c->pitch;
            fp.rows = c->d_rows;
            fp.ids = c->d_ids;
            fp.qbytes = sp.qbytes;
            fp.q16 = sp.q16;
            fp.chunk = chunk;
            fp.hist = c->d_hist;
            fp.stage_rows = stage_rows;
            fp.slice16 = slice16;
            fp.off_sorted = (uint32_t)off_sorted;
            fp.off_ent = 0;
            fp.off_dots = (uint32_t)off_dots;
            fp.off_q = (uint32_t)off_q;
            fp.off_stage = (uint32_t)off_stage;
            fp.qh = c->d_qh + q;
            fp.max_dist = max_dist;
            fp.margin = margin;
            fp.hits = d_hits + (size_t)q * k;
            fp.count = d_count + q;
            fp.status = c->d_status + q;
            fp.tile_counter = c->d_tile_counter;
            fp.done_flag = c->cur_done_flag; fp.done_seq = c->cur_done_seq;
            const ExactSetup xs = exact_setup(c, q, k, max_dist, n, d_hits, d_count);
            const ScanParams& spx = xs.scan;
            const FinalizeExactParams& xp = xs.fin;
            (void)spx; (void)xp;
            fp.x = exact_launch(xs);
            fp.phase = 0;
            fp.x_keys = reinterpret_cast<u64*>(c->d_split);
            fp.x_sbs = reinterpret_cast<float*>(c->d_split + (size_t)kMaxKeep * 8);
            fp.x_fdots = fp.x_sbs + kMaxKeep;
            fp.x_dots = reinterpret_cast<int*>(fp.x_fdots + kMaxKeep);
            fp.x_norms = fp.x_dots + kMaxKeep;
            fp.x_meta = reinterpret_cast<uint32_t*>(fp.x_norms + kMaxKeep);
            if (c->split_finalize && (size_t)keep * c->pitch >= c->split_min_bytes) {
                fp.phase = 1;
                CU_TRY(launch_pdl<FinalizeParams>(finalize_kernel<false>, 1, kFinalThreads, fin_smem, s, fp));
                ReplayParams rp;
                rp.keys = fp.x_keys; rp.meta = fp.x_meta; rp.rows = c->d_rows; rp.qbytes = sp.qbytes; rp.q16 = sp.q16; rp.qh = sp.qh;
                rp.dim = c->dim; rp.pitch = c->pitch;
                rp.sbs = fp.x_sbs; rp.fdots = fp.x_fdots; rp.dots = fp.x_dots; rp.norms = fp.x_norms;
                const size_t rsm = (size_t)c->pitch * 6 + (size_t)kReplayRows * (kReplaySlice16 + 2) * 16;
                replay_kernel<<<(keep + kReplayRows - 1) / kReplayRows, kReplayThreads, rsm, s>>>(rp);
                CU_TRY(cudaGetLastError());
                fp.phase = 2;
                finalize_kernel<false><<<1, kFinalThreads, fin_smem, s>>>(fp);
                CU_TRY(cudaGetLastError());
            } else {
                CU_TRY(launch_pdl<FinalizeParams>(finalize_kernel<false>, 1, kFinalThreads, fin_smem, s, fp));
            }
#ifndef PBX_USE_CDP
            CU_TRY(launch_scan<true>(c, spx, grid, xs.scan_smem, s));
            finalize_exact_kernel<<<1, kFinalThreads, xs.fin_smem, s>>>(xp);
            CU_TRY(cudaGetLastError());
#endif
        }
        c->last_grid = grid;
    }
    if (filter && filter->device) {
        filter_unsorted_count_kernel<<<(nq + 255) / 256, 256, 0, s>>>(reinterpret_cast<const uint32_t*>(c->d_filter_words + 1), d_count, nq,
                                                                      PBX_COUNT_FILTER_UNSORTED);
        CU_TRY(cudaGetLastError());
    }
    if (timed) CU_TRY(cudaEventRecord(c->ev_t1, s));
    CU_TRY(cudaEventRecord(c->ev_chain, s));
    c->chain_valid = true;
    c->queries += nq;
    c->last_bytes = (uint64_t)n * c->dim * nq;
    return PBX_OK;
}

static int check_search_args(const pbx_corpus* c, const void* queries, uint32_t nq, uint32_t k) {
    if (!c) return fail(PBX_E_INVALID, "corpus is NULL");
    if (nq && !queries) return fail(PBX_E_INVALID, "queries is NULL");
    if (k == 0) return fail(PBX_E_INVALID, "k must be >= 1");
    if (k > PBX_MAX_K) return fail(PBX_E_K, "k = %u exceeds PBX_MAX_K = %u", k, PBX_MAX_K);
    return PBX_OK;
}

static int search_device_impl(pbx_corpus* c, const uint8_t* d_queries, uint32_t nq, uint32_t k, double max_dist, pbx_hit* d_hits,
                              uint32_t* d_count, void* cuda_stream, const SearchFilter* filter) {
    int rc = check_search_args(c, d_queries, nq, k);
    if (rc != PBX_OK) return rc;
    if (nq == 0) return PBX_OK;
    if (!d_hits || !d_count) return fail(PBX_E_INVALID, "NULL output");
    rc = flush_pending(c);
    if (rc != PBX_OK) return rc;
    std::lock_guard<std::mutex> lk(c->mu);
    CU_TRY(cudaSetDevice(c->device));
    cudaStream_t s = cuda_stream ? static_cast<cudaStream_t>(cuda_stream) : c->stream;
    return enqueue_search(c, d_queries, nq, k, max_dist, d_hits, d_count, s, false, nullptr, 0, filter);
}

extern "C" int pbx_search_device(pbx_corpus* c, const uint8_t* d_queries, uint32_t nq, uint32_t k, double max_dist, pbx_hit* d_hits,
                                 uint32_t* d_count, void* cuda_stream) {
    return search_device_impl(c, d_queries, nq, k, max_dist, d_hits, d_count, cuda_stream, nullptr);
}

extern "C" int pbx_search_device_filtered(pbx_corpus* c, const uint8_t* d_queries, uint32_t nq, uint32_t k, double max_dist, pbx_hit* d_hits,
                                          uint32_t* d_count, void* cuda_stream, const int64_t* d_filter_ids, uint64_t n_filter,
                                          uint32_t filter_mode) {
    int rc = check_filter_args(d_filter_ids, n_filter, filter_mode);
    if (rc != PBX_OK) return rc;
    const SearchFilter f = {d_filter_ids, n_filter, filter_mode, true};
    return search_device_impl(c, d_queries, nq, k, max_dist, d_hits, d_count, cuda_stream,
                              filter_mode == PBX_FILTER_EXCLUDE && n_filter == 0 ? nullptr : &f);
}

static int search_hits_impl(pbx_corpus* c, const uint8_t* queries, uint32_t nq, uint32_t k, double max_dist, pbx_hit* out_hits,
                            uint32_t* out_count, const SearchFilter* filter) {
    int rc = check_search_args(c, queries, nq, k);
    if (rc != PBX_OK) return rc;
    if (nq == 0) return PBX_OK;
    if (!out_hits || !out_count) return fail(PBX_E_INVALID, "NULL output");
    rc = flush_pending(c);
    if (rc != PBX_OK) return rc;
    std::lock_guard<std::mutex> lk(c->mu);
    CU_TRY(cudaSetDevice(c->device));
    const uint32_t batch_max = 1024;
    float total_ms = 0.f;
    uint64_t total_bytes = 0;
    for (uint32_t q0 = 0; q0 < nq; q0 += batch_max) {
        const uint32_t b = std::min<uint32_t>(batch_max, nq - q0);
        rc = ensure_query_scratch(c, b);
        if (rc != PBX_OK) return rc;
        rc = ensure_hits(c, (size_t)b * k, b);
        if (rc != PBX_OK) return rc;
        const size_t qbytes = (size_t)b * c->dim;
        if (qbytes > c->h_queries_cap) {
            cudaFreeHost(c->h_queries); c->h_queries = nullptr; c->h_queries_cap = 0;
            CU_TRY(cudaMallocHost(&c->h_queries, std::max<size_t>(qbytes, 64 * 1024)));
            c->h_queries_cap = std::max<size_t>(qbytes, 64 * 1024);
        }
        memcpy(c->h_queries, queries + (size_t)q0 * c->dim, qbytes);
        const uint32_t n_now0 = (uint32_t)c->n.load();
        const bool direct = c->zero_copy && b == 1 && n_now0 > 0 && !batch_eligible(c, 1, n_now0, k);
        const uint8_t* q_dev = c->d_queries;
        pbx_hit* hits_dev = c->d_hits;
        if (direct) {
            void* dh = nullptr;
            if (cudaHostGetDevicePointer(&dh, c->h_hits, 0) == cudaSuccess) hits_dev = static_cast<pbx_hit*>(dh);
            else cudaGetLastError();
        }
        const bool polled = direct && hits_dev != c->d_hits;
        CU_TRY(cudaMemcpyAsync(c->d_queries, c->h_queries, qbytes, cudaMemcpyHostToDevice, c->stream));
        uint32_t* d_cnt = reinterpret_cast<uint32_t*>(hits_dev + (size_t)b * k);
        uint32_t* h_cnt = reinterpret_cast<uint32_t*>(c->h_hits + (size_t)b * k);
        const size_t back_bytes = (size_t)b * k * sizeof(pbx_hit) + (size_t)b * sizeof(uint32_t);
        uint32_t* flag_dev = nullptr;
        if (polled) {
            void* df = nullptr;
            if (cudaHostGetDevicePointer(&df, c->h_flag, 0) != cudaSuccess) return fail(PBX_E_CUDA, "completion flag is not device-visible");
            flag_dev = static_cast<uint32_t*>(df);
            ++c->flag_seq;
        }
        rc = enqueue_search(c, q_dev, b, k, max_dist, hits_dev, d_cnt, c->stream, c->profiling, flag_dev, c->flag_seq, filter);
        if (rc != PBX_OK) return rc;
        if (polled) {
            volatile uint32_t* flag = c->h_flag;
            for (uint32_t spins = 1; *flag != c->flag_seq; ++spins) {
                if ((spins & 0xFFFFu) == 0) {
                    const cudaError_t qe = cudaStreamQuery(c->stream);
                    if (qe == cudaSuccess) break;
                    if (qe != cudaErrorNotReady) return fail(PBX_E_CUDA, "search failed: %s", cudaGetErrorString(qe));
                }
            }
            std::atomic_thread_fence(std::memory_order_acquire);
            if (*flag != c->flag_seq) return fail(PBX_E_INTERNAL, "search finished without publishing its result");
            if (c->profiling) CU_TRY(cudaEventSynchronize(c->ev_t1));
        } else {
            CU_TRY(cudaMemcpyAsync(c->h_hits, c->d_hits, back_bytes, cudaMemcpyDeviceToHost, c->stream));
            CU_TRY(cudaStreamSynchronize(c->stream));
        }
        {
            uint32_t failed = 0;
            const uint32_t n_now = (uint32_t)c->n.load();
            for (uint32_t q = 0; q < b; ++q) {
                if (h_cnt[q] != PBX_COUNT_EXACT_LAUNCH_FAILED) continue;
                c->cur_done_flag = nullptr;
                const ExactSetup xs = exact_setup(c, q, k, max_dist, std::min<uint32_t>(n_now, c->last_n), hits_dev, d_cnt);
                CU_TRY(launch_scan<true>(c, xs.scan, xs.grid, xs.scan_smem, c->stream));
                finalize_exact_kernel<<<1, kFinalThreads, xs.fin_smem, c->stream>>>(xs.fin);
                CU_TRY(cudaGetLastError());
                ++failed;
            }
            if (failed) {
                if (!polled) CU_TRY(cudaMemcpyAsync(c->h_hits, c->d_hits, back_bytes, cudaMemcpyDeviceToHost, c->stream));
                CU_TRY(cudaStreamSynchronize(c->stream));
// ... 328 lines not shown
}

extern "C" int pbx_cosine_distance_pairs(int device, const uint8_t* a, const uint8_t* b, uint64_t n, uint32_t dim, float* out_dist,
                                         int32_t* out_dot, int32_t* out_norm2_a, int32_t* out_norm2_b) {
    if (dim == 0 || dim > PBX_MAX_DIM) return fail(PBX_E_DIM, "dim %u outside [1, %u]", dim, PBX_MAX_DIM);
    if (n == 0) return PBX_OK;
    if (!a || !b || !out_dist) return fail(PBX_E_INVALID, "NULL argument");
    if (pbx_device_count() == 0) return fail(PBX_E_NO_DEVICE, "no sm_100 device: pixelbox_b200 has no CPU fallback");
    CU_TRY(cudaSetDevice(device));
    uint8_t *da = nullptr, *db = nullptr;
    float* dd = nullptr;
    int* di = nullptr;
    int rc = PBX_OK;
    cudaError_t e = cudaMalloc(&da, n * dim);
    if (e == cudaSuccess) e = cudaMalloc(&db, n * dim);
    if (e == cudaSuccess) e = cudaMalloc(&dd, n * sizeof(float));
    if (e == cudaSuccess) e = cudaMalloc(&di, 3 * n * sizeof(int));
    if (e == cudaSuccess) e = cudaMemcpy(da, a, n * dim, cudaMemcpyHostToDevice);
    if (e == cudaSuccess) e = cudaMemcpy(db, b, n * dim, cudaMemcpyHostToDevice);
    if (e == cudaSuccess) {
        pair_distance_kernel<<<(unsigned)((n + 127) / 128), 128>>>(da, db, n, dim, dd, di, di + n, di + 2 * n);
        e = cudaGetLastError();
    }
    if (e == cudaSuccess) e = cudaMemcpy(out_dist, dd, n * sizeof(float), cudaMemcpyDeviceToHost);
    if (e == cudaSuccess && out_dot) e = cudaMemcpy(out_dot, di, n * sizeof(int), cudaMemcpyDeviceToHost);
    if (e == cudaSuccess && out_norm2_a) e = cudaMemcpy(out_norm2_a, di + n, n * sizeof(int), cudaMemcpyDeviceToHost);
    if (e == cudaSuccess && out_norm2_b) e = cudaMemcpy(out_norm2_b, di + 2 * n, n * sizeof(int), cudaMemcpyDeviceToHost);
    if (e != cudaSuccess) rc = fail(e == cudaErrorMemoryAllocation ? PBX_E_OOM : PBX_E_CUDA, "pair distance failed: %s", cudaGetErrorString(e));
    cudaFree(da); cudaFree(db); cudaFree(dd); cudaFree(di);
    return rc;
}

static int pair_byte_hamming(int device, const uint8_t* a, const uint8_t* b, uint64_t n, uint32_t dim, int which, float* out_dist,
                             uint32_t* out_int) {
    if (dim == 0 || dim > PBX_MAX_DIM) return fail(PBX_E_DIM, "dim %u outside [1, %u]", dim, PBX_MAX_DIM);
    if (n == 0) return PBX_OK;
    if (!a || !b || !out_dist) return fail(PBX_E_INVALID, "NULL argument");
    if (pbx_device_count() == 0) return fail(PBX_E_NO_DEVICE, "no sm_100 device: pixelbox_b200 has no CPU fallback");
    CU_TRY(cudaSetDevice(device));
    uint8_t *da = nullptr, *db = nullptr;
    float* dd = nullptr;
    uint32_t* di = nullptr;
    cudaError_t e = cudaMalloc(&da, n * dim);
    if (e == cudaSuccess) e = cudaMalloc(&db, n * dim);
    if (e == cudaSuccess) e = cudaMalloc(&dd, n * sizeof(float));
    if (e == cudaSuccess) e = cudaMalloc(&di, n * sizeof(uint32_t));
    if (e == cudaSuccess) e = cudaMemcpy(da, a, n * dim, cudaMemcpyHostToDevice);
    if (e == cudaSuccess) e = cudaMemcpy(db, b, n * dim, cudaMemcpyHostToDevice);
    if (e == cudaSuccess) {
        const unsigned blocks = (unsigned)((n * 32 + 255) / 256);
        if (which == 0) pair_byte_hamming_kernel<<<blocks, 256>>>(da, db, n, dim, dd, di, nullptr, nullptr);
        else pair_byte_hamming_kernel<<<blocks, 256>>>(da, db, n, dim, nullptr, nullptr, dd, di);
        e = cudaGetLastError();
    }
    if (e == cudaSuccess) e = cudaMemcpy(out_dist, dd, n * sizeof(float), cudaMemcpyDeviceToHost);
    if (e == cudaSuccess && out_int) e = cudaMemcpy(out_int, di, n * sizeof(uint32_t), cudaMemcpyDeviceToHost);
    cudaFree(da); cudaFree(db); cudaFree(dd); cudaFree(di);
    if (e != cudaSuccess) return fail(e == cudaErrorMemoryAllocation ? PBX_E_OOM : PBX_E_CUDA, "pair distance failed: %s", cudaGetErrorString(e));
    return PBX_OK;
}

extern "C" int pbx_byte_distance_pairs(int device, const uint8_t* a, const uint8_t* b, uint64_t n, uint32_t dim, float* out_dist,
                                       uint32_t* out_l1) {
    if (n > (1ull << 26)) return fail(PBX_E_INVALID, "at most 2^26 pairs per call");
    return pair_byte_hamming(device, a, b, n, dim, 0, out_dist, out_l1);
}

extern "C" int pbx_hamming_distance_pairs(int device, const uint8_t* a, const uint8_t* b, uint64_t n, uint32_t dim, float* out_dist,
                                          uint32_t* out_bits) {
    if (n > (1ull << 26)) return fail(PBX_E_INVALID, "at most 2^26 pairs per call");
    return pair_byte_hamming(device, a, b, n, dim, 1, out_dist, out_bits);
}

extern "C" int pbx_quantize(int device, const float* embeddings, uint64_t n, uint8_t* out) {
    if (n == 0) return PBX_OK;
    if (!embeddings || !out) return fail(PBX_E_INVALID, "NULL argument");
    if (pbx_device_count() == 0) return fail(PBX_E_NO_DEVICE, "no sm_100 device: pixelbox_b200 has no CPU fallback");
    CU_TRY(cudaSetDevice(device));
    float* din = nullptr;
    uint8_t* dout = nullptr;
    cudaError_t e = cudaMalloc(&din, n * sizeof(float));
    if (e == cudaSuccess) e = cudaMalloc(&dout, n);
    if (e == cudaSuccess) e = cudaMemcpy(din, embeddings, n * sizeof(float), cudaMemcpyHostToDevice);
    if (e == cudaSuccess) {
        quantize_kernel<<<(unsigned)std::min<uint64_t>((n + 255) / 256, 65535), 256>>>(din, n, dout);
        e = cudaGetLastError();
    }
    if (e == cudaSuccess) e = cudaMemcpy(out, dout, n, cudaMemcpyDeviceToHost);
    cudaFree(din); cudaFree(dout);
    if (e != cudaSuccess) return fail(e == cudaErrorMemoryAllocation ? PBX_E_OOM : PBX_E_CUDA, "quantize failed: %s", cudaGetErrorString(e));
    return PBX_OK;
}

extern "C" int pbx_quantize_device(int device, const float* d_embeddings, uint64_t n, uint8_t* d_out, void* cuda_stream) {
    if (n == 0) return PBX_OK;
    if (!d_embeddings || !d_out) return fail(PBX_E_INVALID, "NULL argument");
    if (pbx_device_count() == 0) return fail(PBX_E_NO_DEVICE, "no sm_100 device: pixelbox_b200 has no CPU fallback");
    CU_TRY(cudaSetDevice(device));
    quantize_kernel<<<(unsigned)std::min<uint64_t>((n + 255) / 256, 65535), 256, 0, static_cast<cudaStream_t>(cuda_stream)>>>(d_embeddings, n, d_out);
    CU_TRY(cudaGetLastError());
    return PBX_OK;
}

extern "C" int pbx_int8_peak(int device, double* out_tops) {
    if (!out_tops) return fail(PBX_E_INVALID, "out_tops is NULL");
    if (pbx_device_count() == 0) return fail(PBX_E_NO_DEVICE, "no sm_100 device: pixelbox_b200 has no CPU fallback");
    CU_TRY(cudaSetDevice(device));
    int sms = 0;
    CU_TRY(cudaDeviceGetAttribute(&sms, cudaDevAttrMultiProcessorCount, device));
    sms &= ~1;
    const size_t smem = 4 * 128 * 128 + 1024;
    CU_TRY(cudaFuncSetAttribute(batch_peak_kernel, cudaFuncAttributeMaxDynamicSharedMemorySize, (int)smem));
    cudaLaunchConfig_t cfg = {};
    cfg.gridDim = dim3((unsigned)sms);
    cfg.blockDim = dim3(128);
    cfg.dynamicSmemBytes = smem;
    cudaLaunchAttribute attr[1];
    attr[0].id = cudaLaunchAttributeClusterDimension;
    attr[0].val.clusterDim.x = 2; attr[0].val.clusterDim.y = 1; attr[0].val.clusterDim.z = 1;
    cfg.attrs = attr;
    cfg.numAttrs = 1;
    cudaEvent_t e0 = nullptr, e1 = nullptr;
    CU_TRY(cudaEventCreate(&e0));
    CU_TRY(cudaEventCreate(&e1));
    const int iters = 20000;
    float best = 0.f;
    cudaError_t e = cudaSuccess;
    for (int rep = 0; rep < 4 && e == cudaSuccess; ++rep) {
        e = cudaEventRecord(e0);
        if (e == cudaSuccess) e = cudaLaunchKernelEx(&cfg, batch_peak_kernel, iters);
        if (e == cudaSuccess) e = cudaEventRecord(e1);
        if (e == cudaSuccess) e = cudaEventSynchronize(e1);
        float ms = 0.f;
        if (e == cudaSuccess) e = cudaEventElapsedTime(&ms, e0, e1);
        if (e == cudaSuccess && rep > 0 && (best == 0.f || ms < best)) best = ms;
    }
    cudaEventDestroy(e0); cudaEventDestroy(e1);
    if (e != cudaSuccess) return fail(PBX_E_CUDA, "int8 peak measurement failed: %s", cudaGetErrorString(e));
    *out_tops = 2.0 * 128.0 * 256.0 * 256.0 * (double)iters * (double)sms / ((double)best * 1e-3) / 1e12;
    return PBX_OK;
}

extern "C" int pbx_get_stats(const pbx_corpus* cc, pbx_stats* out) {
    pbx_corpus* c = const_cast<pbx_corpus*>(cc);
    if (!c || !out) return fail(PBX_E_INVALID, "NULL argument");
    std::lock_guard<std::mutex> lk(c->mu);
    memset(out, 0, sizeof(*out));
    out->rows = c->n.load() + c->pending.load();
    out->capacity_rows = c->capacity.load();
    out->reserved = c->use_vmm ? 1 : 0;
    out->dim = c->dim;
    out->row_pitch = c->pitch;
    out->queries = c->queries;
    unsigned long long xp = 0;
    CU_TRY(cudaSetDevice(c->device));
    CU_TRY(cudaMemcpy(&xp, c->d_exact_passes, sizeof(xp), cudaMemcpyDeviceToHost));
    out->exact_passes = xp;
    out->last_search_ms = c->last_search_ms;
    out->last_scan_ms = c->last_scan_ms;
    out->last_bytes_scanned = c->last_bytes;
    out->device = c->device;
    out->sm_count = c->sm_count;
    out->scan_grid = c->last_grid ? c->last_grid : scan_grid(c);
    out->batched_queries = c->batched_queries;
    return PBX_OK;
}

extern "C" int pbx_set_candidate_slack(pbx_corpus* c, uint32_t slack) {
    if (!c) return fail(PBX_E_INVALID, "corpus is NULL");
    std::lock_guard<std::mutex> lk(c->mu);
    c->slack = slack;
    return PBX_OK;
}

extern "C" int pbx_set_profiling(pbx_corpus* c, int enabled) {
    if (!c) return fail(PBX_E_INVALID, "corpus is NULL");
    std::lock_guard<std::mutex> lk(c->mu);
    c->profiling = enabled != 0;
    return PBX_OK;
}

extern "C" int pbx_set_batch_min(pbx_corpus* c, uint32_t min_queries) {
    if (!c) return fail(PBX_E_INVALID, "corpus is NULL");
    std::lock_guard<std::mutex> lk(c->mu);
    c->batch_min = min_queries ? min_queries : 2u;
    return PBX_OK;
}

extern "C" int pbx_set_scan_ctas_per_sm(pbx_corpus* c, uint32_t ctas_per_sm) {
    if (!c) return fail(PBX_E_INVALID, "corpus is NULL");
    if (ctas_per_sm > 8) return fail(PBX_E_INVALID, "ctas_per_sm must be <= 8");
    std::lock_guard<std::mutex> lk(c->mu);
    c->ctas_per_sm = ctas_per_sm;
    return PBX_OK;
}

#ifdef PBX_BATCH_PROF
extern "C" __attribute__((visibility("default"))) int pbx_debug_batch_profile(unsigned long long* out, int reset) {
    if (out && cudaMemcpyFromSymbol(out, g_batch_prof, sizeof(unsigned long long) * 2048 * 12) != cudaSuccess) return -1;
    if (reset) {
        static unsigned long long zeros[2048 * 12];
        if (cudaMemcpyToSymbol(g_batch_prof, zeros, sizeof(zeros)) != cudaSuccess) return -1;
    }
    return 0;
}
#endif
#ifdef PBX_EXP_PROFILE
extern "C" __attribute__((visibility("default"))) int pbx_debug_fin_profile(long long* out) {
    return cudaMemcpyFromSymbol(out, g_fin_prof, sizeof(long long) * 16) == cudaSuccess ? 0 : -1;
}
extern "C" __attribute__((visibility("default"))) int pbx_debug_scan_profile(unsigned long long* out, int reset) {
    if (out && cudaMemcpyFromSymbol(out, g_scan_prof, sizeof(unsigned long long) * kMaxScanGrid * 8) != cudaSuccess) return -1;
    if (reset) {
        static unsigned long long zeros[kMaxScanGrid * 8];
        if (cudaMemcpyToSymbol(g_scan_prof, zeros, sizeof(zeros)) != cudaSuccess) return -1;
    }
    return 0;
}
#endif

#include "sharded.inl"
```

pixelbox_b200/csrc/rerank.cuh:

```cuda
#pragma once
#include "scan.cuh"
#include "../../include/pixelbox_b200.h"

namespace pbx {

struct FinalizeExactParams {
    const KeyX* cand;
    const uint32_t* cand_cnt;
    uint32_t grid;
    uint32_t k;
    uint32_t cap;
    uint32_t dim;
    uint32_t pitch;
    const uint8_t* rows;
    const uint8_t* qbytes;
    pbx_hit* hits;
    uint32_t* count;
    const SearchStatus* status;
    uint32_t* tile_counter;
    unsigned long long* exact_passes;
    uint32_t* done_flag;
    uint32_t done_seq;
};
__global__ void finalize_exact_kernel(const FinalizeExactParams p);
// ... 72 lines not shown
            __syncthreads();
        }
}

__device__ inline void merge_rounds(const FinalizeParams& p, TopBuf<u64>& tb, const uint32_t* s_listcnt, uint32_t maxcnt,
                                    uint32_t* s_pushed) {
    const uint32_t total = maxcnt * p.grid;
    for (uint32_t base = 0; base < total; base += p.chunk) {
        if (*tb.cnt + p.chunk > p.cap) tb.compact();
        const u64 tau = *tb.tau;
        __syncthreads();
        if (threadIdx.x == 0) *s_pushed = 0;
        __syncthreads();
        bool any = false;
        for (uint32_t x = 0; x < p.chunk / kFinalThreads; ++x) {
            const uint32_t e = base + x * kFinalThreads + threadIdx.x;
            bool pass = false;
            u64 key = 0;
            if (e < total) {
                const uint32_t rank = e / p.grid, b = e - rank * p.grid;
                if (rank < s_listcnt[b]) { key = p.cand[e]; pass = key > tau; }
            }
            tb.push_warp(pass, key);
            any |= pass;
        }
        if (any) *s_pushed = 1;
        __syncthreads();
        if (*s_pushed == 0 && p.chunk >= 2 * p.grid) break;
    }
    __syncthreads();
    tb.compact();
}

__device__ __forceinline__ void fold16(const uint4& v, const float* qa, const float* lut, float& s, float& d) {
    const uint32_t w[4] = {v.x, v.y, v.z, v.w};
#pragma unroll
    for (int i = 0; i < 4; ++i) {
        const float4 a = *reinterpret_cast<const float4*>(qa + 4 * i);
        const float av[4] = {a.x, a.y, a.z, a.w};
#pragma unroll
        for (int b = 0; b < 4; ++b) {
            const float fb = lut[(w[i] >> (8 * b)) & 255u];
            s = ref_fold(s, fb, fb);
            d = ref_fold(d, av[b], fb);
        }
    }
}

__device__ __forceinline__ void replay_chunk(const uint4& v, uint32_t ch, uint32_t full, uint32_t dim, const float* s_qa,
                                             const int16_t* s_q16, const float* s_lut, float& s, float& d, int& acc, unsigned& s1,
                                             unsigned& s2) {
    if (ch < full) {
        fold16(v, s_qa + 16 * ch, s_lut, s, d);
    } else {
        const uint32_t w[4] = {v.x, v.y, v.z, v.w};
        for (uint32_t i = 16 * ch; i < dim; ++i) {
            const uint32_t o = i - 16 * ch;
            const float fb = s_lut[(w[o >> 2] >> (8 * (o & 3))) & 255u];
            s = ref_fold(s, fb, fb);
            d = ref_fold(d, s_qa[i], fb);
        }
    }
    const int4 qa4 = *reinterpret_cast<const int4*>(s_q16 + 16 * ch), qb4 = *reinterpret_cast<const int4*>(s_q16 + 16 * ch + 8);
    const int qq[8] = {qa4.x, qa4.y, qa4.z, qa4.w, qb4.x, qb4.y, qb4.z, qb4.w};
    acc = dot16(v, qq, acc);
    s1 = dp4a_uu(v.x, 0x01010101u, s1); s1 = dp4a_uu(v.y, 0x01010101u, s1);
    s1 = dp4a_uu(v.z, 0x01010101u, s1); s1 = dp4a_uu(v.w, 0x01010101u, s1);
    s2 = dp4a_uu(v.x, v.x, s2); s2 = dp4a_uu(v.y, v.y, s2);
    s2 = dp4a_uu(v.z, v.z, s2); s2 = dp4a_uu(v.w, v.w, s2);
}

constexpr uint32_t kReplayRows = 32, kReplayThreads = 256, kReplaySlice16 = 31;
struct ReplayParams {
    const u64* keys;
    const uint32_t* meta;
    const uint8_t* rows;
    const uint8_t* qbytes;
    const int16_t* q16;
    const QueryHeader* qh;
    uint32_t dim, pitch;
    float* sbs;
    float* fdots;
    int* dots;
    int* norms;
};

__global__ void __launch_bounds__(kReplayThreads)
replay_kernel(const ReplayParams p) {
    extern __shared__ __align__(16) unsigned char rsm[];
    float* s_qa = reinterpret_cast<float*>(rsm);
    int16_t* s_q16 = reinterpret_cast<int16_t*>(rsm + 4 * (size_t)p.pitch);
    unsigned char* stage = rsm + 6 * (size_t)p.pitch;
    __shared__ float s_lut[256];
    __shared__ uint32_t s_rows[kReplayRows];
    const uint32_t tid = threadIdx.x;
    const uint32_t nc = p.meta[0];
    const uint32_t c0 = blockIdx.x * kReplayRows;
    if (c0 >= nc) return;
    const uint32_t cb = min(kReplayRows, nc - c0);
    s_lut[tid] = ref_decode(tid);
    if (tid < cb) s_rows[tid] = key64_row(p.keys[c0 + tid]);
    for (uint32_t i = tid; i < p.pitch / 8; i += blockDim.x)
        reinterpret_cast<uint4*>(s_q16)[i] = __ldg(reinterpret_cast<const uint4*>(p.q16) + i);
    __syncthreads();
    for (uint32_t i = tid; i < p.pitch; i += blockDim.x) s_qa[i] = s_lut[p.qbytes[i]];
    __syncthreads();
    const uint32_t pitch16 = p.pitch / 16, full = p.dim >> 4;
    constexpr uint32_t srow = (kReplaySlice16 + 2) * 16;
    float s = 0.0f, d = 0.0f;
    int acc = 0;
    unsigned s1 = 0, s2 = 0;
    for (uint32_t ch0 = 0; ch0 < pitch16; ch0 += kReplaySlice16) {
        const uint32_t w16 = min(kReplaySlice16, pitch16 - ch0);
        const uint32_t total16 = cb * w16;
        for (uint32_t e0 = tid; e0 < total16; e0 += 4 * blockDim.x) {
            uint4 v[4];
#pragma unroll
            for (uint32_t u = 0; u < 4; ++u) {
                const uint32_t e = e0 + u * blockDim.x;
                if (e < total16) {
                    const uint32_t ci = e / w16, ch = e - ci * w16;
                    v[u] = __ldg(reinterpret_cast<const uint4*>(p.rows + (size_t)s_rows[ci] * p.pitch) + ch0 + ch);
                }
            }
#pragma unroll
            for (uint32_t u = 0; u < 4; ++u) {
                const uint32_t e = e0 + u * blockDim.x;
                if (e < total16) {
                    const uint32_t ci = e / w16, ch = e - ci * w16;
                    *reinterpret_cast<uint4*>(stage + (size_t)ci * srow + 16 * ch) = v[u];
                }
            }
        }
        __syncthreads();
        if (tid < cb) {
            const unsigned char* r = stage + (size_t)tid * srow;
            for (uint32_t cl = 0; cl < w16; ++cl)
                replay_chunk(*reinterpret_cast<const uint4*>(r + 16 * cl), ch0 + cl, full, p.dim, s_qa, s_q16, s_lut, s, d, acc, s1, s2);
        }
        __syncthreads();
    }
    if (tid < cb) {
        p.sbs[c0 + tid] = s;
        p.fdots[c0 + tid] = d;
        p.dots[c0 + tid] = 2 * acc - 255 * p.qh->sum_cq;
        p.norms[c0 + tid] = (int)(4u * s2 - 1020u * s1 + 65025u * p.dim);
    }
}


#ifdef PBX_USE_CDP
__device__ inline bool launch_exact_tail(const ExactLaunch& x) {
#define PBX_X_CASE(LL, CC) \
    case LL * CC: scan_kernel<LL, CC, true><<<x.grid, kScanThreads, x.scan_smem, cudaStreamTailLaunch>>>(x.scan); break;
    switch (x.scan.pitch16) {
        PBX_X_CASE(1, 1) PBX_X_CASE(2, 1) PBX_X_CASE(4, 1) PBX_X_CASE(8, 1) PBX_X_CASE(16, 1) PBX_X_CASE(32, 1)
        PBX_X_CASE(32, 2) PBX_X_CASE(32, 4)
#define PBX_X_CASE_M(LL, CC, MM) \
    case (LL) * (CC): scan_kernel<LL, CC, true, MM><<<x.grid, kScanThreads, x.scan_smem, cudaStreamTailLaunch>>>(x.scan); break;
        PBX_EXTRA_SHAPES(PBX_X_CASE_M)
#undef PBX_X_CASE_M
        default:
            scan_generic_kernel<true><<<x.grid, kScanThreads, x.scan_smem + x.scan.pitch16 * 32, cudaStreamTailLaunch>>>(x.scan);
            break;
    }
#undef PBX_X_CASE
    if (cudaGetLastError() != cudaSuccess) return false;
    finalize_exact_kernel<<<1, kFinalThreads, x.fin_smem, cudaStreamTailLaunch>>>(x.fin);
    return cudaGetLastError() == cudaSuccess;
}
#endif

#ifdef PBX_EXP_PROFILE
__device__ long long g_fin_prof[16];
#define PBX_FIN_STAMP(i) do { if (threadIdx.x == 0) g_fin_prof[i] = clock64(); } while (0)
#else
#define PBX_FIN_STAMP(i) do { } while (0)
#endif

__device__ inline void block_order_keys(u64* buf, u64* sorted, uint32_t m) {
    const uint32_t tid = threadIdx.x;
    if (m <= kFinalThreads) {
        const uint32_t tpe = min(32u, (uint32_t)kFinalThreads / next_pow2(m < 2 ? 2 : m));
        const uint32_t e = tid / tpe, sub = tid - e * tpe;
        const u64 me = e < m ? buf[e] : 0ull;
        uint32_t rank = 0;
        if (e < m) {
#pragma unroll 4
            for (uint32_t j = sub; j < m; j += tpe) rank += (buf[j] > me) ? 1u : 0u;
        }
        for (uint32_t off = tpe >> 1; off; off >>= 1) rank += __shfl_xor_sync(0xFFFFFFFFu, rank, off);
        if (e < m && sub == 0) sorted[rank] = me;
        __syncthreads();
    } else if (m <= 2 * kFinalThreads) {
        for (uint32_t t = tid; t < m; t += blockDim.x) {
            const u64 me = buf[t];
            uint32_t rank = 0;
            for (uint32_t j = 0; j < m; ++j) rank += (buf[j] > me) ? 1u : 0u;
            sorted[rank] = me;
        }
        __syncthreads();
    } else {
        const uint32_t m2 = next_pow2(m);
        for (uint32_t i = m + tid; i < m2; i += blockDim.x) buf[i] = 0ull;
        __syncthreads();
        block_sort_desc<u64>(buf, m2);
        for (uint32_t i = tid; i < m; i += blockDim.x) sorted[i] = buf[i];
        __syncthreads();
    }
}

__device__ inline void block_min_key(const u64* a, uint32_t n, u64* s_out, u64* s_scratch ) {
    u64 m = ~0ull;
    for (uint32_t i = threadIdx.x; i < n; i += blockDim.x) m = a[i] < m ? a[i] : m;
    for (int off = 16; off; off >>= 1) {
        const u64 o = __shfl_xor_sync(0xFFFFFFFFu, m, off);
        m = o < m ? o : m;
    }
    if ((threadIdx.x & 31) == 0) s_scratch[threadIdx.x >> 5] = m;
    __syncthreads();
    if (threadIdx.x == 0) {
        u64 r = ~0ull;
        for (uint32_t w = 0; w < (blockDim.x + 31) / 32; ++w) r = s_scratch[w] < r ? s_scratch[w] : r;
        *s_out = r;
    }
    __syncthreads();
}

__device__ inline uint32_t block_candidates(u64* buf, u64* sorted, uint32_t m, uint32_t keep, uint32_t k, uint32_t cap,
                                            uint32_t* s_cnt, u64* s_tau, SelectScratch* s_sel, u64* s_scratch,
                                            float* s_kappa_k, float* s_kappa_last) {
    if (m <= kFinalThreads) {
        block_order_keys(buf, sorted, m);
        const uint32_t nc = m < keep ? m : keep;
        if (threadIdx.x == 0) {
            *s_kappa_k = (nc >= k && k > 0) ? key64_kappa(sorted[k - 1]) : 0.0f;
            *s_kappa_last = nc > 0 ? key64_kappa(sorted[nc - 1]) : 0.0f;
        }
        __syncthreads();
        return nc;
    }
    TopBuf<u64> tb{buf, s_cnt, s_tau, cap, keep};
    if (threadIdx.x == 0) *s_cnt = m;
    __syncthreads();
    if (m > keep) block_select_top(tb, s_sel);
    const uint32_t nc = *s_cnt;
    for (uint32_t i = threadIdx.x; i < nc; i += blockDim.x) sorted[i] = buf[i];
    __syncthreads();
    __shared__ u64 s_min;
    block_min_key(sorted, nc, &s_min, s_scratch);
    if (threadIdx.x == 0) *s_kappa_last = key64_kappa(s_min);
    if (nc > k && k > 0) {
        TopBuf<u64> tk{buf, s_cnt, s_tau, cap, k};
        block_select_top(tk, s_sel);
        block_min_key(buf, k, &s_min, s_scratch);
        if (threadIdx.x == 0) *s_kappa_k = key64_kappa(s_min);
    } else if (threadIdx.x == 0) {
        *s_kappa_k = (nc == k && k > 0) ? key64_kappa(s_min) : 0.0f;
    }
    __syncthreads();
    return nc;
}

template <bool BATCH>
__global__ void __launch_bounds__(kFinalThreads, 1)
finalize_kernel(const FinalizeParams p) {
    PBX_FIN_STAMP(0);
    extern __shared__ __align__(16) unsigned char smem_raw[];
    u64* buf = reinterpret_cast<u64*>(smem_raw);
    u64* sorted = reinterpret_cast<u64*>(smem_raw + p.off_sorted);
    RerankEntry* ent = reinterpret_cast<RerankEntry*>(smem_raw + p.off_ent);
    int* dots = reinterpret_cast<int*>(smem_raw + p.off_dots);
    int* norms = dots + p.keep;
    float* dists = reinterpret_cast<float*>(norms + p.keep);
    float* sbs = dists + p.keep;
    float* fdots = sbs + p.keep;
    float* s_qa = reinterpret_cast<float*>(smem_raw + p.off_q);
    int16_t* s_q16 = reinterpret_cast<int16_t*>(smem_raw + p.off_q + 4 * p.pitch);
    unsigned char* stage = smem_raw + p.off_stage;

    __shared__ uint32_t s_cnt, s_pushed, s_maxcnt, s_nonplateau, s_bstar, s_mprime, s_total, s_odlo, s_odhi;
    __shared__ u64 s_tau;
    __shared__ float s_lut[256];
    __shared__ float s_kappa_k, s_kappa_last, s_sa;
    __shared__ uint32_t s_listcnt[kMaxScanGrid];
    __shared__ uint32_t s_warp[32];
    __shared__ u64 s_scratch64[32];

    const uint32_t tid = threadIdx.x, lane = tid & 31, warp = tid >> 5;
    const uint32_t q = BATCH ? blockIdx.x : 0u;
    const int16_t* q16_g = p.q16 + (size_t)q * p.pitch;
    const uint8_t* qbytes_g = p.qbytes + (size_t)q * p.pitch;
    QueryHeader* qh_g = p.qh + q;
    pbx_hit* hits_g = p.hits + (size_t)q * p.k;
    uint32_t* count_g = p.count + q;
    SearchStatus* status_g = p.status + q;
    __shared__ SelectScratch s_sel;
    if (tid < 256) s_lut[tid] = ref_decode(tid);
    if (tid == 0) { s_cnt = 0; s_tau = 0ull; s_maxcnt = 0; s_nonplateau = 0; s_pushed = 0; s_bstar = 0; s_mprime = 0; s_odlo = 0xFFFFFFFFu; s_odhi = 0u; }
    pdl_wait();
    for (uint32_t i = tid; i < p.pitch / 8; i += blockDim.x)
        reinterpret_cast<uint4*>(s_q16)[i] = __ldg(reinterpret_cast<const uint4*>(q16_g) + i);
    __syncthreads();
    for (uint32_t i = tid; i < p.pitch; i += blockDim.x) s_qa[i] = s_lut[qbytes_g[i]];
    uint32_t nc;
    if (!BATCH && p.phase == 2) {
        nc = p.x_meta[0];
        for (uint32_t i = tid; i < nc; i += blockDim.x) sorted[i] = p.x_keys[i];
        if (tid == 0) { s_kappa_k = __uint_as_float(p.x_meta[1]); s_kappa_last = __uint_as_float(p.x_meta[2]); }
        __syncthreads();
    } else if constexpr (!BATCH) {
        for (uint32_t b = tid; b < p.grid; b += blockDim.x) {
            uint32_t c = p.cand_cnt[b];
            s_listcnt[b] = c;
            atomicMax(&s_maxcnt, c);
        }

        PBX_FIN_STAMP(1);
        constexpr uint32_t BPT = kHistBins / kFinalThreads;
        uint32_t h[BPT];
    #pragma unroll
        for (uint32_t i = 0; i < BPT; ++i) {
            h[i] = __ldcg(p.hist + (size_t)tid * BPT + i);
            p.hist[(size_t)tid * BPT + i] = 0;
        }
        uint32_t mine = 0;
    #pragma unroll
        for (uint32_t i = 0; i < BPT; ++i) mine += h[i];
        uint32_t incl = mine;
    #pragma unroll
        for (int off = 1; off < 32; off <<= 1) {
            uint32_t v = __shfl_down_sync(0xFFFFFFFFu, incl, off);
            if (lane + off < 32) incl += v;
        }
        if (lane == 0) s_warp[warp] = incl;
        __syncthreads();
        uint32_t above = incl - mine;
        for (uint32_t w = warp + 1; w < kFinalThreads / 32; ++w) above += s_warp[w];
        if (tid == 0) { uint32_t t = 0; for (uint32_t w = 0; w < kFinalThreads / 32; ++w) t += s_warp[w]; s_total = t; }
        if (above < p.keep && above + mine >= p.keep) {
            uint32_t run = above;
    #pragma unroll
            for (int i = BPT - 1; i >= 0; --i) {
                run += h[i];
                if (run >= p.keep) { s_bstar = tid * BPT + i; s_mprime = run; break; }
            }
        }
        __syncthreads();
        if (s_total < p.keep && tid == 0) { s_bstar = 0; s_mprime = s_total; }
        __syncthreads();

        PBX_FIN_STAMP(2);
        const uint32_t mprime = s_mprime, bstar = s_bstar;
        if (mprime <= p.cap) {
            for (uint32_t b = tid; b < p.grid; b += blockDim.x) {
                const uint32_t len = s_listcnt[b];
                for (uint32_t r0 = 0; r0 < len; r0 += 4) {
                    u64 key[4];
    #pragma unroll
                    for (uint32_t i = 0; i < 4; ++i) key[i] = (r0 + i < len) ? p.cand[(size_t)(r0 + i) * p.grid + b] : 0ull;
                    uint32_t take = 0;
    #pragma unroll
                    for (uint32_t i = 0; i < 4; ++i)
                        if (take == i && r0 + i < len && kappa_bin(key64_kappa(key[i])) >= bstar) take = i + 1;
                    if (take) {
                        const uint32_t at = atomicAdd(&s_cnt, take);
    #pragma unroll
                        for (uint32_t i = 0; i < 4; ++i) if (i < take) buf[at + i] = key[i];
                    }
                    if (take < 4) break;
                }
            }
            __syncthreads();
            PBX_FIN_STAMP(3);
            const uint32_t m = s_cnt;
            nc = block_candidates(buf, sorted, m, p.keep, p.k, p.cap, &s_cnt, &s_tau, &s_sel, s_scratch64, &s_kappa_k, &s_kappa_last);
        } else {
            TopBuf<u64> tb{buf, &s_cnt, &s_tau, p.cap, p.keep};
            merge_rounds(p, tb, s_listcnt, s_maxcnt, &s_pushed);
            nc = s_cnt < p.keep ? s_cnt : p.keep;
            for (uint32_t i = tid; i < nc; i += blockDim.x) sorted[i] = buf[i];
            __syncthreads();
            if (tid == 0) {
                s_kappa_k = (nc >= p.k && p.k > 0) ? key64_kappa(sorted[p.k - 1]) : 0.0f;
                s_kappa_last = nc > 0 ? key64_kappa(sorted[nc - 1]) : 0.0f;
            }
            __syncthreads();
        }
    } else {
        __syncthreads();
        const uint32_t c = min(min(p.bcnt[q], p.bcap), p.cap);
        const float inv_q = qh_g->inv_q;
        const u64* src = p.bcand + (size_t)q * p.bcap;
        for (uint32_t i = tid; i < c; i += blockDim.x) {
            const u64 e = src[i];
            buf[i] = make_key64(__fmul_rn(key64_kappa(e), inv_q), key64_row(e));
        }
        if (tid == 0) s_cnt = c;
        __syncthreads();
        if (c > p.keep) {
            TopBuf<u64> tb{buf, &s_cnt, &s_tau, p.cap, p.keep};
            block_select_top(tb, &s_sel);
        }
        const uint32_t m = s_cnt;
        nc = block_candidates(buf, sorted, m, p.keep, p.k, p.cap, &s_cnt, &s_tau, &s_sel, s_scratch64, &s_kappa_k, &s_kappa_last);
    }

    PBX_FIN_STAMP(4);
    if (!BATCH && p.phase == 1) {
        for (uint32_t i = tid; i < nc; i += blockDim.x) p.x_keys[i] = sorted[i];
        if (tid == 0) { p.x_meta[0] = nc; p.x_meta[1] = __float_as_uint(s_kappa_k); p.x_meta[2] = __float_as_uint(s_kappa_last); }
        return;
    }
    {
        float* sq = reinterpret_cast<float*>(buf);
        for (uint32_t i = tid; i < p.dim; i += blockDim.x) { const float a = s_qa[i]; sq[i] = __fmul_rn(a, a); }
        __syncthreads();
        if (tid == kFinalThreads - 1) {
            float sa = 0.0f;
            uint32_t i = 0;
            for (; i + 8 <= p.dim; i += 8) {
                const float4 x = *reinterpret_cast<const float4*>(sq + i), y = *reinterpret_cast<const float4*>(sq + i + 4);
                sa = __fadd_rn(sa, x.x); sa = __fadd_rn(sa, x.y); sa = __fadd_rn(sa, x.z); sa = __fadd_rn(sa, x.w);
                sa = __fadd_rn(sa, y.x); sa = __fadd_rn(sa, y.y); sa = __fadd_rn(sa, y.z); sa = __fadd_rn(sa, y.w);
            }
            for (; i < p.dim; ++i) sa = __fadd_rn(sa, sq[i]);
            s_sa = sa;
            qh_g->sa = sa;
        }
    }
    const uint32_t pitch16 = p.pitch / 16, slice16 = p.slice16;
    const uint32_t srow = ((slice16 + 1) | 1u) * 16;
    const uint32_t full = p.dim >> 4;
    const int sum_cq = qh_g->sum_cq;
    constexpr uint32_t kStageBatch = 6;
    if (!BATCH && p.phase == 2) {
        for (uint32_t i = tid; i < nc; i += blockDim.x) {
            sbs[i] = p.x_sbs[i]; fdots[i] = p.x_fdots[i]; dots[i] = p.x_dots[i]; norms[i] = p.x_norms[i];
        }
    } else
    for (uint32_t c0 = 0; c0 < nc; c0 += p.stage_rows) {
        const uint32_t cb = min(p.stage_rows, nc - c0);
        float s = 0.0f, d = 0.0f;
        int acc = 0;
        unsigned s1 = 0, s2 = 0;
        for (uint32_t ch0 = 0; ch0 < pitch16; ch0 += slice16) {
            const uint32_t w16 = min(slice16, pitch16 - ch0);
            const uint32_t total16 = cb * w16;
            for (uint32_t e0 = tid; e0 < total16; e0 += kStageBatch * blockDim.x) {
                uint4 v[kStageBatch];
#pragma unroll
                for (uint32_t u = 0; u < kStageBatch; ++u) {
                    const uint32_t e = e0 + u * blockDim.x;
                    if (e < total16) {
                        const uint32_t ci = e / w16, ch = e - ci * w16;
                        const uint32_t row = key64_row(sorted[c0 + ci]);
                        v[u] = __ldg(reinterpret_cast<const uint4*>(p.rows + (size_t)row * p.pitch) + ch0 + ch);
                    }
                }
#pragma unroll
                for (uint32_t u = 0; u < kStageBatch; ++u) {
                    const uint32_t e = e0 + u * blockDim.x;
                    if (e < total16) {
                        const uint32_t ci = e / w16, ch = e - ci * w16;
                        *reinterpret_cast<uint4*>(stage + (size_t)ci * srow + 16 * ch) = v[u];
                    }
                }
            }
            __syncthreads();
            PBX_FIN_STAMP(5);
            if (tid < cb) {
                const unsigned char* r = stage + (size_t)tid * srow;
                for (uint32_t cl = 0; cl < w16; ++cl)
                    replay_chunk(*reinterpret_cast<const uint4*>(r + 16 * cl), ch0 + cl, full, p.dim, s_qa, s_q16, s_lut, s, d, acc, s1, s2);
            }
            __syncthreads();
        }
        if (tid < cb) {
            sbs[c0 + tid] = s;
            fdots[c0 + tid] = d;
            dots[c0 + tid] = 2 * acc - 255 * sum_cq;
            norms[c0 + tid] = (int)(4u * s2 - 1020u * s1 + 65025u * p.dim);
        }
    }
    __syncthreads();
    PBX_FIN_STAMP(6);
    const float sa = s_sa;
    const uint32_t n2 = next_pow2(nc < 2 ? 2 : nc);
    uint32_t nonplateau = 0;
    int64_t my_id[kMaxKeep / kFinalThreads];
#pragma unroll
    for (uint32_t x = 0; x < kMaxKeep / kFinalThreads; ++x) {
        const uint32_t c = tid + x * kFinalThreads;
        my_id[x] = (c < nc) ? p.ids[key64_row(sorted[c])] : INT64_MAX;
    }
    __syncthreads();
#pragma unroll
    for (uint32_t x = 0; x < kMaxKeep / kFinalThreads; ++x) {
        const uint32_t c = tid + x * kFinalThreads;
        if (c < nc) {
            const float dist = ref_distance(sa, sbs[c], fdots[c]);
            dists[c] = dist;
            RerankEntry e;
            e.od = ord_f32(dist);
            e.slot = c;
            e.id = my_id[x];
            ent[c] = e;
            if (dist < PBX_PLATEAU_DIST) nonplateau++;
        }
    }
    for (uint32_t c = nc + tid; c < n2; c += blockDim.x) {
        RerankEntry e; e.od = 0xFFFFFFFFu; e.slot = 0xFFFFFFFFu; e.id = INT64_MAX;
        ent[c] = e;
    }
    if (nonplateau) atomicAdd(&s_nonplateau, nonplateau);
    if (tid == 0) s_cnt = 0;
    __syncthreads();

    PBX_FIN_STAMP(7);
    uint32_t local = 0;
    if (nc <= kFinalThreads) {
        const uint32_t tpe = min(32u, (uint32_t)kFinalThreads / next_pow2(nc < 2 ? 2 : nc));
        const uint32_t c = tid / tpe, sub = tid - c * tpe;
        RerankEntry me; me.od = 0; me.slot = 0; me.id = 0;
        if (c < nc) me = ent[c];
        uint32_t pos = 0;
        if (c < nc) {
#pragma unroll 4
            for (uint32_t j = sub; j < nc; j += tpe) pos += rerank_before(ent[j], me) ? 1u : 0u;
        }
        for (uint32_t off = tpe >> 1; off; off >>= 1) pos += __shfl_xor_sync(0xFFFFFFFFu, pos, off);
        if (c < nc && sub == 0) {
            const float dist = dists[c];
            const bool ok = (double)dist < p.max_dist;
            if (ok) local = 1;
            if (pos < p.k) {
                pbx_hit hh;
                if (ok) { hh.image_id = me.id; hh.dist = dist; hh.dot = dots[c]; hh.norm2 = norms[c]; hh.flags = 0; }
                else { hh.image_id = INT64_MAX; hh.dist = __int_as_float(0x7f800000); hh.dot = 0; hh.norm2 = 0; hh.flags = 0; }
                hits_g[pos] = hh;
            }
        }
    } else if ((size_t)nc * sizeof(RerankEntry) <= p.off_sorted) {
        RerankEntry* ent2 = reinterpret_cast<RerankEntry*>(sorted);
        uint32_t* s_base = s_listcnt;
        uint32_t* s_cur = s_listcnt + 1024;
        static_assert(kMaxScanGrid >= 2048 && kFinalThreads == 1024, "bucket order borrows s_listcnt as 2 x 1024 counters");
        uint32_t lo = 0xFFFFFFFFu, hi = 0u;
        for (uint32_t c = tid; c < nc; c += blockDim.x) { const uint32_t od = ent[c].od; lo = min(lo, od); hi = max(hi, od); }
        lo = __reduce_min_sync(0xFFFFFFFFu, lo);
        hi = __reduce_max_sync(0xFFFFFFFFu, hi);
        if (lane == 0) { atomicMin(&s_odlo, lo); atomicMax(&s_odhi, hi); }
        s_base[tid] = 0;
        __syncthreads();
        lo = s_odlo;
        const uint32_t range = s_odhi - lo;
        const uint32_t sh = range < 1024u ? 0u : 22u - (uint32_t)__clz(range);
        for (uint32_t c = tid; c < nc; c += blockDim.x) atomicAdd(&s_base[(ent[c].od - lo) >> sh], 1u);
        __syncthreads();
        {
            const uint32_t v = s_base[tid];
            uint32_t incl = v;
#pragma unroll
            for (int off = 1; off < 32; off <<= 1) {
                const uint32_t o = __shfl_up_sync(0xFFFFFFFFu, incl, off);
                if ((int)lane >= off) incl += o;
            }
            if (lane == 31) s_warp[warp] = incl;
            __syncthreads();
            uint32_t before = 0;
            for (uint32_t w = 0; w < warp; ++w) before += s_warp[w];
            const uint32_t excl = before + incl - v;
            __syncthreads();
            s_base[tid] = excl;
            s_cur[tid] = excl;
        }
        __syncthreads();
        for (uint32_t c = tid; c < nc; c += blockDim.x) {
            const RerankEntry e = ent[c];
            ent2[atomicAdd(&s_cur[(e.od - lo) >> sh], 1u)] = e;
        }
        __syncthreads();
        for (uint32_t i = tid; i < nc; i += blockDim.x) {
            const RerankEntry me = ent2[i];
            const uint32_t b = (me.od - lo) >> sh;
            const uint32_t bs = s_base[b], be = s_cur[b];
            uint32_t pos = bs;
            for (uint32_t j = bs; j < be; ++j) pos += rerank_before(ent2[j], me) ? 1u : 0u;
            const float dist = dists[me.slot];
            const bool ok = (double)dist < p.max_dist;
            if (ok) local++;
            if (pos < p.k) {
                pbx_hit hh;
                if (ok) { hh.image_id = me.id; hh.dist = dist; hh.dot = dots[me.slot]; hh.norm2 = norms[me.slot]; hh.flags = 0; }
                else { hh.image_id = INT64_MAX; hh.dist = __int_as_float(0x7f800000); hh.dot = 0; hh.norm2 = 0; hh.flags = 0; }
                hits_g[pos] = hh;
            }
        }
    } else {
        block_sort_rerank(ent, n2);
        for (uint32_t c = tid; c < nc; c += blockDim.x) {
            const RerankEntry e = ent[c];
            const float dist = dists[e.slot];
            const bool ok = (double)dist < p.max_dist;
            if (ok) local++;
            if (c < p.k) {
                pbx_hit hh;
                if (ok) { hh.image_id = e.id; hh.dist = dist; hh.dot = dots[e.slot]; hh.norm2 = norms[e.slot]; hh.flags = 0; }
                else { hh.image_id = INT64_MAX; hh.dist = __int_as_float(0x7f800000); hh.dot = 0; hh.norm2 = 0; hh.flags = 0; }
                hits_g[c] = hh;
            }
        }
    }
    for (uint32_t c = nc + tid; c < p.k; c += blockDim.x) {
        pbx_hit hh; hh.image_id = INT64_MAX; hh.dist = __int_as_float(0x7f800000); hh.dot = 0; hh.norm2 = 0; hh.flags = 0;
        hits_g[c] = hh;
    }
    if (local) atomicAdd(&s_cnt, local);
    __syncthreads();

    PBX_FIN_STAMP(8);
    if (tid == 0) {
        const uint32_t passing = s_cnt;
        *count_g = passing < p.k ? passing : p.k;
        SearchStatus st;
        st.n_candidates = nc;
        st.reserved = 0;
        st.need_exact = 0;
        st.theta = 0.0f;
        const u64 searchable = p.n_allowed ? *p.n_allowed : (u64)p.n;
        if (searchable > nc) {
            const bool plateau_reachable = p.max_dist > (double)PBX_PLATEAU_DIST && s_nonplateau < p.k;
            const bool separated = (double)s_kappa_last < (double)s_kappa_k - (double)p.margin;
            if (plateau_reachable) { st.need_exact = 1; st.theta = -__int_as_float(0x7f800000); }
            else if (!separated) { st.need_exact = 1; st.theta = (float)((double)s_kappa_k - (double)p.margin - 1e-7); }
        }
        if constexpr (BATCH) {
            if (p.boverflow[q]) { st.need_exact = 1; st.theta = -__int_as_float(0x7f800000); }
        }
        *status_g = st;
        if constexpr (!BATCH) {
            p.tile_counter[0] = 0;
            p.tile_counter[32] = 0;
            bool exact_follows = st.need_exact != 0;
#ifdef PBX_USE_CDP
            if (st.need_exact) { __threadfence(); if (!launch_exact_tail(p.x)) { *count_g = PBX_COUNT_EXACT_LAUNCH_FAILED; exact_follows = false; } }
#endif
            if (p.done_flag && !exact_follows) {
                __threadfence_system();
                *reinterpret_cast<volatile uint32_t*>(p.done_flag) = p.done_seq;
            }
        } else {
            if (st.need_exact) atomicAdd(p.bticket + 1, 1u);
            __threadfence();
            if (atomicAdd(p.bticket, 1u) == gridDim.x - 1) {
                *p.bticket = 0;
                __threadfence();
                const uint32_t n_need = *reinterpret_cast<volatile uint32_t*>(p.bticket + 1);
                p.bticket[1] = 0;
#ifdef PBX_USE_CDP
                for (uint32_t qq = 0; n_need && qq < p.nq; ++qq) {
                    if (*reinterpret_cast<volatile uint32_t*>(&p.status[qq].need_exact) == 0) continue;
                    ExactLaunch x = p.x;
                    x.scan.q16 += (size_t)qq * p.pitch;
                    x.scan.qbytes += (size_t)qq * p.pitch;
                    x.scan.qh += qq;
                    x.scan.status += qq;
                    x.fin.qbytes += (size_t)qq * p.pitch;
                    x.fin.hits += (size_t)qq * p.k;
                    x.fin.count += qq;
                    x.fin.status += qq;
                    if (!launch_exact_tail(x)) p.count[qq] = PBX_COUNT_EXACT_LAUNCH_FAILED;
                }
#endif
            }
        }
    }
}

}
```

pixelbox_b200/csrc/scan.cuh:

```cuda
#pragma once
#include "common.cuh"

namespace pbx {

struct QueryHeader {
    int sum_cq;
    int norm2_q;
    float inv_q;
    float sa;
};

struct SearchStatus {
    uint32_t need_exact;
    float theta;
    uint32_t n_candidates;
    uint32_t reserved;
};

struct ScanParams {
    const uint4* rows;
    const float* inv_norm;
    const int64_t* ids;
    uint32_t n;
    uint32_t pitch16;
    uint32_t dim;
    const int16_t* q16;
    const uint8_t* qbytes;
    const QueryHeader* qh;
    uint32_t keep;
    uint32_t cap;
    void* cand;
    uint32_t* cand_cnt;
    uint32_t* tile_counter;
    uint32_t* hist;
    const SearchStatus* status;
    double max_dist;
    const uint32_t* allow;
};

__device__ __forceinline__ int dot16(const uint4& v, const int* q, int acc) {
    acc = dp2a_lo(q[0], v.x, acc); acc = dp2a_hi(q[1], v.x, acc);
    acc = dp2a_lo(q[2], v.y, acc); acc = dp2a_hi(q[3], v.y, acc);
    acc = dp2a_lo(q[4], v.z, acc); acc = dp2a_hi(q[5], v.z, acc);
    acc = dp2a_lo(q[6], v.w, acc); acc = dp2a_hi(q[7], v.w, acc);
    return acc;
}

template <int L>
__device__ __forceinline__ int transpose_reduce(int (&acc)[L], int j) {
#pragma unroll
    for (int off = L / 2; off >= 1; off >>= 1) {
        const bool up = (j & off) != 0;
#pragma unroll
        for (int i = 0; i < off; ++i) {
            int send = up ? acc[i] : acc[i + off];
            int keep = up ? acc[i + off] : acc[i];
            acc[i] = keep + __shfl_xor_sync(0xFFFFFFFFu, send, off);
        }
    }
    return acc[0];
}

struct ReplayOut {
    float sb, dot;
    int idot, inorm;
};

__device__ __forceinline__ void replay_bytes(uint32_t rv, uint32_t qv, int nbytes, const float* lut, float& s, float& d) {
#pragma unroll
    for (int b = 0; b < 4; ++b) {
        if (b < nbytes) {
            const float fb = lut[(rv >> (8 * b)) & 255u], fa = lut[(qv >> (8 * b)) & 255u];
            s = ref_fold(s, fb, fb);
            d = ref_fold(d, fa, fb);
        }
    }
}

template <bool WITH_INTS>
__device__ __forceinline__ ReplayOut replay_row(const uint8_t* __restrict__ row, const uint8_t* q, const int16_t* q16, uint32_t dim,
                                                int sum_cq, const float* lut) {
    const uint4* r4 = reinterpret_cast<const uint4*>(row);
    const uint32_t* q32 = reinterpret_cast<const uint32_t*>(q);
    const int4* q16v = reinterpret_cast<const int4*>(q16);
    const uint32_t full = dim >> 4, chunks = (dim + 15) >> 4;
    float s = 0.0f, d = 0.0f;
    int acc = 0;
    unsigned s1 = 0, s2 = 0;
    const uint4 zero = make_uint4(0, 0, 0, 0);
    uint4 cur[4], nxt[4];
#pragma unroll
    for (int i = 0; i < 4; ++i) cur[i] = ((uint32_t)i < chunks) ? __ldg(r4 + i) : zero;
    for (uint32_t c = 0; c < chunks; c += 4) {
#pragma unroll
        for (int i = 0; i < 4; ++i) nxt[i] = (c + 4 + i < chunks) ? __ldg(r4 + c + 4 + i) : zero;
#pragma unroll
        for (int i = 0; i < 4; ++i) {
            const uint32_t ci = c + i;
            if (ci < chunks) {
                const uint4 v = cur[i];
                if (ci < full) {
                    replay_bytes(v.x, q32[4 * ci + 0], 4, lut, s, d);
                    replay_bytes(v.y, q32[4 * ci + 1], 4, lut, s, d);
                    replay_bytes(v.z, q32[4 * ci + 2], 4, lut, s, d);
                    replay_bytes(v.w, q32[4 * ci + 3], 4, lut, s, d);
                } else {
                    const int rem = (int)(dim - (ci << 4));
                    replay_bytes(v.x, q32[4 * ci + 0], rem, lut, s, d);
                    replay_bytes(v.y, q32[4 * ci + 1], rem - 4, lut, s, d);
                    replay_bytes(v.z, q32[4 * ci + 2], rem - 8, lut, s, d);
                    replay_bytes(v.w, q32[4 * ci + 3], rem - 12, lut, s, d);
                }
                if constexpr (WITH_INTS) {
                    const int4 a = q16v[2 * ci], b = q16v[2 * ci + 1];
                    const int qq[8] = {a.x, a.y, a.z, a.w, b.x, b.y, b.z, b.w};
                    acc = dot16(v, qq, acc);
                    s1 = dp4a_uu(v.x, 0x01010101u, s1); s1 = dp4a_uu(v.y, 0x01010101u, s1);
                    s1 = dp4a_uu(v.z, 0x01010101u, s1); s1 = dp4a_uu(v.w, 0x01010101u, s1);
                    s2 = dp4a_uu(v.x, v.x, s2); s2 = dp4a_uu(v.y, v.y, s2);
                    s2 = dp4a_uu(v.z, v.z, s2); s2 = dp4a_uu(v.w, v.w, s2);
                }
            }
        }
#pragma unroll
        for (int i = 0; i < 4; ++i) cur[i] = nxt[i];
    }
    ReplayOut o;
    o.sb = s;
    o.dot = d;
    o.idot = 2 * acc - 255 * sum_cq;
    o.inorm = (int)(4u * s2 - 1020u * s1 + 65025u * dim);
    return o;
}

#ifdef PBX_EXP_PROFILE
__device__ unsigned long long g_scan_prof[kMaxScanGrid][8];
#define PBX_PROF_ADD(i, v) do { if (threadIdx.x == 0) g_scan_prof[blockIdx.x][i] += (unsigned long long)(v); } while (0)
#else
#define PBX_PROF_ADD(i, v) do { } while (0)
#endif

template <typename K, bool EXACT>
struct ScanShared {
    uint32_t cnt;
    uint32_t done;
    uint32_t gb;
    uint32_t tile[2];
    K tau;
    float lut[EXACT ? 256 : 1];
    SelectScratch sel;
};

constexpr int scan_minb(int pitch16) { return pitch16 >= 16 ? 2 : 4; }

template <int L, int C, bool EXACT, int MINB = scan_minb(L * C), bool RAGGED = false, bool FILTER = false>
__global__ void __launch_bounds__(kScanThreads, MINB)
scan_kernel(const ScanParams p) {
    static_assert(!(FILTER && EXACT), "the exact pass tests the filter at run time");
    using K = typename std::conditional<EXACT, KeyX, u64>::type;
    constexpr int G = 32 / L;
    constexpr int P16 = L * C;
    const uint32_t PR = RAGGED ? p.pitch16 : (uint32_t)P16;
    extern __shared__ __align__(16) unsigned char smem_raw[];
    K* buf = reinterpret_cast<K*>(smem_raw);
    __shared__ ScanShared<K, EXACT> sh;

    pdl_wait();
    pdl_trigger();
    if constexpr (EXACT) {
        if (p.status->need_exact == 0) return;
        sh.lut[threadIdx.x & 255] = ref_decode(threadIdx.x & 255);
    }
    const int lane = threadIdx.x & 31, warp = threadIdx.x >> 5;
    const int g = lane / L, j = lane % L;
#ifdef PBX_EXP_PROFILE
    const long long t_kernel0 = clock64();
#endif

    int q[C][8];
    bool has_chunk[C];
    uint32_t coff[C];
#pragma unroll
    for (int c = 0; c < C; ++c) {
        has_chunk[c] = !RAGGED || (uint32_t)(j + c * L) < PR;
        coff[c] = has_chunk[c] ? (uint32_t)(j + c * L) : PR - 1u;
        const int4* src = reinterpret_cast<const int4*>(p.q16 + (size_t)(has_chunk[c] ? (j + c * L) : 0) * 16);
        int4 a = __ldg(src), b = __ldg(src + 1);
        if (!has_chunk[c]) { a = make_int4(0, 0, 0, 0); b = a; }
        q[c][0] = a.x; q[c][1] = a.y; q[c][2] = a.z; q[c][3] = a.w;
        q[c][4] = b.x; q[c][5] = b.y; q[c][6] = b.z; q[c][7] = b.w;
    }
    const QueryHeader qh = *p.qh;
    const int bias = -255 * qh.sum_cq;
    float theta = 0.0f;
    if constexpr (EXACT) theta = p.status->theta;

    uint32_t* const gbin = p.tile_counter + 32;
    if (threadIdx.x == 0) { sh.cnt = 0; sh.done = 0; sh.gb = EXACT ? 0u : *reinterpret_cast<volatile uint32_t*>(gbin); sh.tau = KeyOps<K>::lowest(); }
    TopBuf<K> tb{buf, &sh.cnt, &sh.tau, p.cap, p.keep};
    __syncthreads();

    uint32_t gb = sh.gb;
    const uint32_t total_warps = gridDim.x * kScanWarps;

    constexpr uint32_t GRAB = (P16 >= 16) ? 1u : 16u / P16;
    const uint32_t n_chunks = (p.n + kChunkRows - 1) / kChunkRows;
    const uint32_t threshold = p.cap - kTileRows;
    uint32_t cur = 0, end = 0, nxt = 0;
    if (lane == 0) nxt = atomicAdd(p.tile_counter, GRAB);
    bool counted = false;
    for (;;) {
        if (cur == end && !counted) {
            cur = __shfl_sync(0xFFFFFFFFu, nxt, 0);
            end = cur + GRAB;
            if (lane == 0 && cur < n_chunks) nxt = atomicAdd(p.tile_counter, GRAB);
            if constexpr (!EXACT) {
                const uint32_t claim = cur / GRAB;
                if (cur < n_chunks && claim >= total_warps && claim % total_warps == 0 &&
                    ((claim / total_warps) & (claim / total_warps - 1)) == 0) {
                    const uint32_t b = hist_threshold_warp(p.hist, p.keep, lane);
                    if (lane == 0 && b) { atomicMax(gbin, b); atomicMax(&sh.gb, b); }
                }
            }
        }
        const bool have = cur < n_chunks;
        if (have && *reinterpret_cast<volatile uint32_t*>(&sh.cnt) <= threshold) {
            const K tau = sh.tau;
            const uint32_t chunk_row0 = cur * kChunkRows;
            ++cur;
            uint32_t gpoll = 0;
            if constexpr (!EXACT) {
                if (warp == 0 && lane == 0) gpoll = *reinterpret_cast<volatile uint32_t*>(gbin);
            }
            constexpr int UNR = (L * C >= 16) ? 1 : kItersPerChunk;
#pragma unroll UNR
            for (int it = 0; it < kItersPerChunk; ++it) {
                const uint32_t row0 = chunk_row0 + (uint32_t)it * kRowsPerWarpIter;
                const uint32_t my_row = row0 + (uint32_t)(j * G + g);
                uint32_t allow_word = 0;
                if constexpr (FILTER) allow_word = __ldg(p.allow + (row0 >> 5));
                float gthr = -__int_as_float(0x7f800000);
                uint32_t gb_new = 0;
                if constexpr (!EXACT) {
                    gthr = bin_threshold(gb);
                    gb_new = *reinterpret_cast<volatile uint32_t*>(&sh.gb);
                }
#ifdef PBX_EXP_NOMETA
                const float inv_r = 1.0e-4f;
#else
                const float inv_r = __ldg(p.inv_norm + my_row);
#endif
                const uint4* base = p.rows + (size_t)row0 * PR + (size_t)g * PR + (RAGGED ? 0 : j);
                int acc[L];
#pragma unroll
                for (int r = 0; r < L; ++r) {
                    int a = 0;
#pragma unroll
                    for (int c = 0; c < C; ++c) {
                        uint4 v = ldg_stream(base + (size_t)(r * G) * PR + (RAGGED ? coff[c] : (uint32_t)(c * L)));
                        a = dot16(v, q[c], a);
                    }
                    acc[r] = a;
                }
                const int s = transpose_reduce<L>(acc, j);
                const int dot_i = 2 * s + bias;
                const float kappa = __fmul_rn(__fmul_rn((float)dot_i, inv_r), qh.inv_q);
                if constexpr (!EXACT) {
                    const u64 key = make_key64(kappa, my_row);
#ifdef PBX_EXP_NOPUSH
                    if (key == 0x1234567ull) buf[0] = key;
#else
                    bool pass = my_row < p.n && key > tau && kappa_shift(kappa) >= gthr;
                    if constexpr (FILTER) pass = pass && ((allow_word >> (my_row & 31u)) & 1u);
                    tb.push_warp(pass, key);
                    if (pass) atomicAdd(p.hist + kappa_bin(kappa), 1u);
#ifdef PBX_EXP_PROFILE
                    if (pass) atomicAdd(&g_scan_prof[blockIdx.x][0], 1ull);
#endif
#endif
                } else {
                    bool pass = false;
                    KeyX key = KeyOps<KeyX>::lowest();
                    if (my_row < p.n && kappa >= theta && row_allowed(p.allow, my_row)) {
                        const ReplayOut ro = replay_row<false>(reinterpret_cast<const uint8_t*>(p.rows) + (size_t)my_row * ((size_t)PR * 16),
                                                               p.qbytes, p.q16, p.dim, qh.sum_cq, sh.lut);
                        float dist = ref_distance(qh.sa, ro.sb, ro.dot);
                        if ((double)dist < p.max_dist) {
                            key = make_keyx(dist, __ldg(p.ids + my_row), my_row);
                            pass = keyx_gt(key, tau);
                        }
                    }
                    tb.push_warp(pass, key);
                }
                if constexpr (!EXACT) gb = max(gb, gb_new);
            }
            if constexpr (!EXACT) {
                if (warp == 0 && lane == 0 && gpoll > sh.gb) sh.gb = gpoll;
            }
            continue;
        }
        if (!have && !counted) {
            counted = true;
            if (lane == 0) atomicAdd(&sh.done, 1u);
        }
#ifdef PBX_EXP_PROFILE
        const long long t_r0 = clock64();
#endif
        __syncthreads();
#ifdef PBX_EXP_PROFILE
        const long long t_r1 = clock64();
        if constexpr (!EXACT) PBX_PROF_ADD(2, t_r1 - t_r0);
#endif
        if (sh.done == (uint32_t)kScanWarps) break;
        if constexpr (EXACT) tb.compact(); else block_select_top(tb, &sh.sel);
#ifdef PBX_EXP_PROFILE
        if constexpr (!EXACT) { PBX_PROF_ADD(3, clock64() - t_r1); PBX_PROF_ADD(1, 1); }
#endif
    }

    if constexpr (!EXACT) {
        const float gfinal = bin_threshold(max(sh.gb, *reinterpret_cast<volatile uint32_t*>(gbin)));
        PBX_PROF_ADD(5, sh.cnt);
        tb.filter_inplace([gfinal](const u64& e) { return kappa_shift(key64_kappa(e)) >= gfinal; });
        if (sh.cnt > p.keep) block_select_top(tb, &sh.sel);
    }
    if constexpr (!EXACT) PBX_PROF_ADD(6, sh.cnt);
    tb.compact();
    const uint32_t c = sh.cnt < p.keep ? sh.cnt : p.keep;
    K* out = reinterpret_cast<K*>(p.cand);
    for (uint32_t i = threadIdx.x; i < c; i += blockDim.x) out[(size_t)i * gridDim.x + blockIdx.x] = buf[i];
    if (threadIdx.x == 0) p.cand_cnt[blockIdx.x] = c;
#ifdef PBX_EXP_PROFILE
    if constexpr (!EXACT) PBX_PROF_ADD(4, clock64() - t_kernel0);
#endif
}

template <bool EXACT>
__global__ void __launch_bounds__(kScanThreads, 2)
scan_generic_kernel(const ScanParams p) {
    using K = typename std::conditional<EXACT, KeyX, u64>::type;
    extern __shared__ __align__(16) unsigned char smem_raw[];
    K* buf = reinterpret_cast<K*>(smem_raw);
    int4* sq = reinterpret_cast<int4*>(smem_raw + (size_t)p.cap * sizeof(K));
    __shared__ ScanShared<K, EXACT> sh;

    if constexpr (EXACT) {
        if (p.status->need_exact == 0) return;
        sh.lut[threadIdx.x & 255] = ref_decode(threadIdx.x & 255);
    }
    for (uint32_t i = threadIdx.x; i < p.pitch16 * 2; i += blockDim.x) sq[i] = __ldg(reinterpret_cast<const int4*>(p.q16) + i);
    const int lane = threadIdx.x & 31, warp = threadIdx.x >> 5;
    const QueryHeader qh = *p.qh;
    const int bias = -255 * qh.sum_cq;
    float theta = 0.0f;
    if constexpr (EXACT) theta = p.status->theta;
    if (threadIdx.x == 0) { sh.cnt = 0; sh.tau = KeyOps<K>::lowest(); }
    TopBuf<K> tb{buf, &sh.cnt, &sh.tau, p.cap, p.keep};
    const uint32_t n_tiles = (p.n + kTileRows - 1) / kTileRows;

    for (;;) {
        __syncthreads();
        if (threadIdx.x == 0) sh.tile[0] = atomicAdd(p.tile_counter, 1u);
        if (sh.cnt + kTileRows > p.cap) tb.compact();
        __syncthreads();
        const uint32_t tile = sh.tile[0];
        if (tile >= n_tiles) break;
        const K tau = sh.tau;
        for (int it = 0; it < kItersPerTile; ++it) {
            const uint32_t my_row = tile * kTileRows + (uint32_t)(it * kScanWarps + warp) * kRowsPerWarpIter + lane;
            const float inv_r = __ldg(p.inv_norm + my_row);
            const uint4* rp = p.rows + (size_t)my_row * p.pitch16;
            int s = 0;
            for (uint32_t c = 0; c < p.pitch16; ++c) {
                uint4 v = __ldg(rp + c);
                int4 a = sq[2 * c], b = sq[2 * c + 1];
                int qq[8] = {a.x, a.y, a.z, a.w, b.x, b.y, b.z, b.w};
                s = dot16(v, qq, s);
            }
            const int dot_i = 2 * s + bias;
            const float kappa = __fmul_rn(__fmul_rn((float)dot_i, inv_r), qh.inv_q);
            if constexpr (!EXACT) {
                const u64 key = make_key64(kappa, my_row);
                const bool pass = my_row < p.n && key > tau && row_allowed(p.allow, my_row);
                tb.push_warp(pass, key);
                if (pass) atomicAdd(p.hist + kappa_bin(kappa), 1u);
            } else {
                bool pass = false;
                KeyX key = KeyOps<KeyX>::lowest();
                if (my_row < p.n && kappa >= theta && row_allowed(p.allow, my_row)) {
                    const ReplayOut ro = replay_row<false>(reinterpret_cast<const uint8_t*>(p.rows) + (size_t)my_row * ((size_t)p.pitch16 * 16),
                                                           p.qbytes, p.q16, p.dim, qh.sum_cq, sh.lut);
                    float dist = ref_distance(qh.sa, ro.sb, ro.dot);
                    if ((double)dist < p.max_dist) {
                        key = make_keyx(dist, __ldg(p.ids + my_row), my_row);
                        pass = keyx_gt(key, tau);
                    }
                }
                tb.push_warp(pass, key);
            }
        }
    }
    tb.compact();
    const uint32_t c = sh.cnt < p.keep ? sh.cnt : p.keep;
    K* out = reinterpret_cast<K*>(p.cand);
    for (uint32_t i = threadIdx.x; i < c; i += blockDim.x) out[(size_t)i * gridDim.x + blockIdx.x] = buf[i];
    if (threadIdx.x == 0) p.cand_cnt[blockIdx.x] = c;
}

}

#define PBX_EXTRA_SHAPES(X)                                                                  \
    X(1, 3, 2) X(2, 3, 2) X(4, 3, 2) X(8, 3, 2) X(16, 3, 2) X(32, 3, 2)                      \
    X(1, 5, 2) X(2, 5, 2) X(4, 5, 2) X(8, 5, 2) X(16, 5, 2) X(32, 5, 2)                      \
    X(32, 6, 2) X(32, 8, 1)

#define PBX_RAGGED_SHAPES(X) X(8, 1, 4) X(16, 1, 2) X(32, 1, 2) X(32, 2, 2) X(32, 4, 2) X(32, 8, 1)
```

Before: 6317.

## Fuse candidate finalize into the last scan block via grid-completion ticket

Adds a fast-finish path where the last scan CTA to finish, detected with an atomic ticket, runs the candidate merge, f32 replay, rerank and certificate itself. This removes the separate finalize kernel launch. If too many candidates survive, it counts a fallback and tail-launches the regular finalize kernel. The path is enabled only when built with CDP and the finalize is not split. The scan kernel's shared-memory budget is enlarged to fit the finish layout, which may reduce occupancy. The prep-seed kernel also switches from a PDL launch to a plain launch.

```diff
diff --git a/include/pixelbox_b200.h b/include/pixelbox_b200.h
--- a/include/pixelbox_b200.h
+++ b/include/pixelbox_b200.h
@@ -64,6 +64,7 @@
     int32_t scan_grid;
     int32_t reserved;
     uint64_t batched_queries;
+    uint64_t finalize_fallbacks;
 } pbx_stats;
 
 PBX_API int pbx_corpus_create(uint32_t dim, uint64_t capacity_hint, int device, pbx_corpus** out);
diff --git a/pixelbox_b200/_native.py b/pixelbox_b200/_native.py
--- a/pixelbox_b200/_native.py
+++ b/pixelbox_b200/_native.py
@@ -43,7 +43,7 @@
         ("row_pitch", ctypes.c_uint32), ("queries", ctypes.c_uint64), ("exact_passes", ctypes.c_uint64),
         ("last_search_ms", ctypes.c_float), ("last_scan_ms", ctypes.c_float), ("last_bytes_scanned", ctypes.c_uint64),
         ("device", ctypes.c_int32), ("sm_count", ctypes.c_int32), ("scan_grid", ctypes.c_int32), ("reserved", ctypes.c_int32),
-        ("batched_queries", ctypes.c_uint64),
+        ("batched_queries", ctypes.c_uint64), ("finalize_fallbacks", ctypes.c_uint64),
     ]
 
 
diff --git a/pixelbox_b200/csrc/api.cu b/pixelbox_b200/csrc/api.cu
--- a/pixelbox_b200/csrc/api.cu
+++ b/pixelbox_b200/csrc/api.cu
@@ -157,6 +157,7 @@
     uint32_t* d_tile_counter = nullptr;
     uint32_t* d_hist = nullptr;
     unsigned long long* d_exact_passes = nullptr;
+    unsigned long long* d_finalize_fallbacks = nullptr;
     uint32_t* d_allow = nullptr;
     size_t allow_words = 0;
     u64* d_filter_words = nullptr;
@@ -510,7 +511,10 @@
     if (e == cudaSuccess) e = cudaMemset(c->d_tile_counter, 0, 512);
     if (e == cudaSuccess) e = cudaMalloc(&c->d_hist, 2 * kHistBins * sizeof(uint32_t));
     if (e == cudaSuccess) e = cudaMemset(c->d_hist, 0, 2 * kHistBins * sizeof(uint32_t));
-    if (e == cudaSuccess) { c->d_exact_passes = reinterpret_cast<unsigned long long*>(reinterpret_cast<char*>(c->d_tile_counter) + 256); }
+    if (e == cudaSuccess) {
+        c->d_exact_passes = reinterpret_cast<unsigned long long*>(reinterpret_cast<char*>(c->d_tile_counter) + 256);
+        c->d_finalize_fallbacks = c->d_exact_passes + 1;
+    }
     if (e != cudaSuccess) {
         int rc = fail(PBX_E_CUDA, "corpus setup failed: %s", cudaGetErrorString(e));
         pbx_corpus_destroy(c);
@@ -899,13 +903,28 @@
     cfg.numAttrs = 1;
     return cudaLaunchKernelEx(&cfg, kern, params);
 }
+template <typename P, typename F>
+static cudaError_t launch_pdl(void (*kern)(const P, const F), int grid, int block, size_t smem, cudaStream_t s, const P& params, const F& f) {
+    cudaLaunchConfig_t cfg = {};
+    cfg.gridDim = dim3((unsigned)grid);
+    cfg.blockDim = dim3((unsigned)block);
+    cfg.dynamicSmemBytes = smem;
+    cfg.stream = s;
+    cudaLaunchAttribute attr[1];
+    attr[0].id = cudaLaunchAttributeProgrammaticStreamSerialization;
+    attr[0].val.programmaticStreamSerializationAllowed = 1;
+    cfg.attrs = attr;
+    cfg.numAttrs = 1;
+    return cudaLaunchKernelEx(&cfg, kern, params, f);
+}
 
 template <bool EXACT, bool FILTER>
-static cudaError_t launch_scan_as(const pbx_corpus* c, const ScanParams& p, int grid, size_t smem, cudaStream_t s) {
+static cudaError_t launch_scan_as(const pbx_corpus* c, const ScanParams& p, const typename ScanFinish<EXACT>::type& f, int grid, size_t smem,
+                                  cudaStream_t s) {
     static_assert(!(EXACT && FILTER), "the exact pass has no FILTER instantiation");
 #define PBX_SCAN_CASE(LL, CC)                                                                                                     \
     {                                                                                                                             \
-        return launch_pdl<ScanParams>(scan_kernel<LL, CC, EXACT, scan_minb(LL * CC), false, FILTER>, grid, kScanThreads, smem, s, p); \
+        return launch_pdl(scan_kernel<LL, CC, EXACT, scan_minb(LL * CC), false, FILTER>, grid, kScanThreads, smem, s, p, f); \
     }
     switch (c->pitch16) {
         case 1: PBX_SCAN_CASE(1, 1)
@@ -914,36 +933,37 @@
         case 8: PBX_SCAN_CASE(8, 1)
         case 16:
             if constexpr (!EXACT) {
-                if (c->ctas_per_sm == 3 || c->ctas_per_sm == 0) return launch_pdl<ScanParams>(scan_kernel<16, 1, false, 3, false, FILTER>, grid, kScanThreads, smem, s, p);
-                if (c->ctas_per_sm >= 4) return launch_pdl<ScanParams>(scan_kernel<16, 1, false, 4, false, FILTER>, grid, kScanThreads, smem, s, p);
+                if (c->ctas_per_sm == 3 || c->ctas_per_sm == 0) return launch_pdl(scan_kernel<16, 1, false, 3, false, FILTER>, grid, kScanThreads, smem, s, p, f);
+                if (c->ctas_per_sm >= 4) return launch_pdl(scan_kernel<16, 1, false, 4, false, FILTER>, grid, kScanThreads, smem, s, p, f);
             }
             PBX_SCAN_CASE(16, 1)
         case 32: PBX_SCAN_CASE(32, 1)
         case 64: PBX_SCAN_CASE(32, 2)
         case 128: PBX_SCAN_CASE(32, 4)
-#define PBX_SCAN_CASE_M(LL, CC, MM) case (LL) * (CC): return launch_pdl<ScanParams>(scan_kernel<LL, CC, EXACT, MM, false, FILTER>, grid, kScanThreads, smem, s, p);
+#define PBX_SCAN_CASE_M(LL, CC, MM) case (LL) * (CC): return launch_pdl(scan_kernel<LL, CC, EXACT, MM, false, FILTER>, grid, kScanThreads, smem, s, p, f);
         PBX_EXTRA_SHAPES(PBX_SCAN_CASE_M)
 #undef PBX_SCAN_CASE_M
         default: {
             if constexpr (!EXACT) {
 #define PBX_SCAN_CASE_R(LL, CC, MM) \
-    if (c->pitch16 <= (LL) * (CC)) return launch_pdl<ScanParams>(scan_kernel<LL, CC, false, MM, true, FILTER>, grid, kScanThreads, smem, s, p);
+    if (c->pitch16 <= (LL) * (CC)) return launch_pdl(scan_kernel<LL, CC, false, MM, true, FILTER>, grid, kScanThreads, smem, s, p, f);
                 PBX_RAGGED_SHAPES(PBX_SCAN_CASE_R)
 #undef PBX_SCAN_CASE_R
             }
             size_t sm = smem + (size_t)c->pitch16 * 32;
-            return launch_pdl<ScanParams>(scan_generic_kernel<EXACT>, grid, kScanThreads, sm, s, p);
+            return launch_pdl(scan_generic_kernel<EXACT>, grid, kScanThreads, sm, s, p, f);
         }
     }
 #undef PBX_SCAN_CASE
 }
 
 template <bool EXACT>
-static cudaError_t launch_scan(const pbx_corpus* c, const ScanParams& p, int grid, size_t smem, cudaStream_t s) {
+static cudaError_t launch_scan(const pbx_corpus* c, const ScanParams& p, int grid, size_t smem, cudaStream_t s,
+                               const typename ScanFinish<EXACT>::type& f = {}) {
     if constexpr (!EXACT) {
-        if (p.allow) return launch_scan_as<false, true>(c, p, grid, smem, s);
-    }
-    return launch_scan_as<EXACT, false>(c, p, grid, smem, s);
+        if (p.allow) return launch_scan_as<false, true>(c, p, f, grid, smem, s);
+    }
+    return launch_scan_as<EXACT, false>(c, p, f, grid, smem, s);
 }
 
 static bool fast_shape(uint32_t pitch16) {
@@ -1387,6 +1407,37 @@
         if (off_stage >= fin_budget || !finalize_stage_layout(fin_budget - off_stage, keep, c->pitch16, &stage_rows, &slice16, &stage_bytes))
             return fail(PBX_E_INTERNAL, "finalize layout does not fit shared memory (k=%u dim=%u)", k, c->dim);
         const size_t fin_smem = off_stage + stage_bytes;
+        const bool split = c->split_finalize && (size_t)keep * c->pitch >= c->split_min_bytes;
+#ifdef PBX_USE_CDP
+        const bool finish = !split && keep <= (uint32_t)kScanThreads;
+#else
+        const bool finish = false;
+#endif
+        size_t scan_smem = (size_t)cap_scan * sizeof(u64);
+        FastFinish ff;
+        memset(&ff, 0, sizeof(ff));
+        if (finish) {
+            const size_t per_sm = (size_t)std::max(1, grid / c->sm_count);
+            constexpr size_t kStaticReserve = 4u << 10;
+            const size_t need = per_sm * (scan_smem + kStaticReserve);
+            size_t carve = 228u << 10;
+            for (size_t step : {32u, 64u, 100u, 132u, 164u, 196u, 228u})
+                if ((step << 10) >= need) { carve = step << 10; break; }
+            const size_t budget = std::min<size_t>(200u << 10, std::max(scan_smem, carve / per_sm - kStaticReserve));
+            const size_t keys = std::max<size_t>({(size_t)kFinishKeys * 8, (size_t)c->pitch * 4, (size_t)next_pow2(keep) * sizeof(RerankEntry)});
+            ff.off_sorted = (uint32_t)keys;
+            ff.off_dots = (uint32_t)(keys + (size_t)kFinishKeys * 8);
+            ff.off_q = (uint32_t)((ff.off_dots + (size_t)keep * 20 + 15) & ~(size_t)15);
+            ff.off_lut = (uint32_t)(ff.off_q + (size_t)c->pitch * 6);
+            ff.off_stage = (uint32_t)((ff.off_lut + 1024 + 15) & ~(size_t)15);
+            size_t finish_stage = 0;
+            if (ff.off_stage >= budget || !finalize_stage_layout(budget - ff.off_stage, keep, c->pitch16, &ff.stage_rows, &ff.slice16, &finish_stage))
+                return fail(PBX_E_INTERNAL, "scan finish layout does not fit shared memory (k=%u dim=%u)", k, c->dim);
+            scan_smem = std::max<size_t>(scan_smem, ff.off_stage + finish_stage);
+            ff.finish = 1;
+            ff.fin_smem = (uint32_t)fin_smem;
+            ff.fallbacks = c->d_finalize_fallbacks;
+        }
 
         for (uint32_t q = 0; q < nq; ++q) {
             ScanParams sp;
@@ -1419,14 +1470,11 @@
                 ps.do_seed = seeded ? 1u : 0u;
                 ps.seed_hist = c->d_hist + kHistBins; ps.ticket = c->d_tile_counter + 96; ps.gbin = c->d_tile_counter + 32;
                 ps.allow = c->cur_allow;
-                CU_TRY(launch_pdl<PrepSeedParams>(prep_seed_kernel, seeded ? seed_grid : 1, kSeedThreads, (size_t)c->pitch * 2, s, ps));
+                prep_seed_kernel<<<seeded ? seed_grid : 1, kSeedThreads, (size_t)c->pitch * 2, s>>>(ps);
+                CU_TRY(cudaGetLastError());
             }
-            const bool time_scan = timed && q + 1 == nq;
-            if (time_scan) CU_TRY(cudaEventRecord(c->ev_s0, s));
-            CU_TRY(launch_scan<false>(c, sp, grid, (size_t)cap_scan * sizeof(u64), s));
-            if (time_scan) { CU_TRY(cudaEventRecord(c->ev_s1, s)); c->scan_timed = true; }
-
-            FinalizeParams fp;
+
+            FinalizeParams& fp = ff.f;
             fp.cand = reinterpret_cast<const u64*>(c->d_cand);
             fp.cand_cnt = c->d_cand_cnt;
             fp.grid = (uint32_t)grid;
@@ -1470,7 +1518,12 @@
             fp.x_dots = reinterpret_cast<int*>(fp.x_fdots + kMaxKeep);
             fp.x_norms = fp.x_dots + kMaxKeep;
             fp.x_meta = reinterpret_cast<uint32_t*>(fp.x_norms + kMaxKeep);
-            if (c->split_finalize && (size_t)keep * c->pitch >= c->split_min_bytes) {
+            const bool time_scan = timed && q + 1 == nq;
+            if (time_scan) CU_TRY(cudaEventRecord(c->ev_s0, s));
+            CU_TRY(launch_scan<false>(c, sp, grid, scan_smem, s, ff));
+            if (time_scan) { CU_TRY(cudaEventRecord(c->ev_s1, s)); c->scan_timed = true; }
+            if (finish) {
+            } else if (split) {
                 fp.phase = 1;
                 CU_TRY(launch_pdl<FinalizeParams>(finalize_kernel<false>, 1, kFinalThreads, fin_smem, s, fp));
                 ReplayParams rp;
@@ -2105,10 +2158,11 @@
     out->dim = c->dim;
     out->row_pitch = c->pitch;
     out->queries = c->queries;
-    unsigned long long xp = 0;
+    unsigned long long xp[2] = {0, 0};
     CU_TRY(cudaSetDevice(c->device));
-    CU_TRY(cudaMemcpy(&xp, c->d_exact_passes, sizeof(xp), cudaMemcpyDeviceToHost));
-    out->exact_passes = xp;
+    CU_TRY(cudaMemcpy(xp, c->d_exact_passes, sizeof(xp), cudaMemcpyDeviceToHost));
+    out->exact_passes = xp[0];
+    out->finalize_fallbacks = xp[1];
     out->last_search_ms = c->last_search_ms;
     out->last_scan_ms = c->last_scan_ms;
     out->last_bytes_scanned = c->last_bytes;
diff --git a/pixelbox_b200/csrc/rerank.cuh b/pixelbox_b200/csrc/rerank.cuh
--- a/pixelbox_b200/csrc/rerank.cuh
+++ b/pixelbox_b200/csrc/rerank.cuh
@@ -248,16 +248,16 @@
 #ifdef PBX_USE_CDP
 __device__ inline bool launch_exact_tail(const ExactLaunch& x) {
 #define PBX_X_CASE(LL, CC) \
-    case LL * CC: scan_kernel<LL, CC, true><<<x.grid, kScanThreads, x.scan_smem, cudaStreamTailLaunch>>>(x.scan); break;
+    case LL * CC: scan_kernel<LL, CC, true><<<x.grid, kScanThreads, x.scan_smem, cudaStreamTailLaunch>>>(x.scan, NoFinish{}); break;
     switch (x.scan.pitch16) {
         PBX_X_CASE(1, 1) PBX_X_CASE(2, 1) PBX_X_CASE(4, 1) PBX_X_CASE(8, 1) PBX_X_CASE(16, 1) PBX_X_CASE(32, 1)
         PBX_X_CASE(32, 2) PBX_X_CASE(32, 4)
 #define PBX_X_CASE_M(LL, CC, MM) \
-    case (LL) * (CC): scan_kernel<LL, CC, true, MM><<<x.grid, kScanThreads, x.scan_smem, cudaStreamTailLaunch>>>(x.scan); break;
+    case (LL) * (CC): scan_kernel<LL, CC, true, MM><<<x.grid, kScanThreads, x.scan_smem, cudaStreamTailLaunch>>>(x.scan, NoFinish{}); break;
         PBX_EXTRA_SHAPES(PBX_X_CASE_M)
 #undef PBX_X_CASE_M
         default:
-            scan_generic_kernel<true><<<x.grid, kScanThreads, x.scan_smem + x.scan.pitch16 * 32, cudaStreamTailLaunch>>>(x.scan);
+            scan_generic_kernel<true><<<x.grid, kScanThreads, x.scan_smem + x.scan.pitch16 * 32, cudaStreamTailLaunch>>>(x.scan, NoFinish{});
             break;
     }
 #undef PBX_X_CASE
@@ -274,10 +274,82 @@
 #define PBX_FIN_STAMP(i) do { } while (0)
 #endif
 
+__device__ __forceinline__ void replay_candidates(const u64* sorted, uint32_t nc, uint32_t stage_rows, uint32_t slice16, uint32_t pitch,
+                                                  uint32_t dim, const uint8_t* rows, const float* s_qa, const int16_t* s_q16,
+                                                  const float* s_lut, unsigned char* stage, int sum_cq, float* sbs, float* fdots,
+                                                  int* dots, int* norms) {
+    const uint32_t tid = threadIdx.x;
+    const uint32_t pitch16 = pitch / 16;
+    const uint32_t srow = ((slice16 + 1) | 1u) * 16;
+    const uint32_t full = dim >> 4;
+    constexpr uint32_t kStageBatch = 6;
+    for (uint32_t c0 = 0; c0 < nc; c0 += stage_rows) {
+        const uint32_t cb = min(stage_rows, nc - c0);
+        float s = 0.0f, d = 0.0f;
+        int acc = 0;
+        unsigned s1 = 0, s2 = 0;
+        for (uint32_t ch0 = 0; ch0 < pitch16; ch0 += slice16) {
+            const uint32_t w16 = min(slice16, pitch16 - ch0);
+            const uint32_t total16 = cb * w16;
+            for (uint32_t e0 = tid; e0 < total16; e0 += kStageBatch * blockDim.x) {
+                uint4 v[kStageBatch];
+#pragma unroll
+                for (uint32_t u = 0; u < kStageBatch; ++u) {
+                    const uint32_t e = e0 + u * blockDim.x;
+                    if (e < total16) {
+                        const uint32_t ci = e / w16, ch = e - ci * w16;
+                        const uint32_t row = key64_row(sorted[c0 + ci]);
+                        v[u] = __ldg(reinterpret_cast<const uint4*>(rows + (size_t)row * pitch) + ch0 + ch);
+                    }
+                }
+#pragma unroll
+                for (uint32_t u = 0; u < kStageBatch; ++u) {
+                    const uint32_t e = e0 + u * blockDim.x;
+                    if (e < total16) {
+                        const uint32_t ci = e / w16, ch = e - ci * w16;
+                        *reinterpret_cast<uint4*>(stage + (size_t)ci * srow + 16 * ch) = v[u];
+                    }
+                }
+            }
+            __syncthreads();
+            PBX_FIN_STAMP(5);
+            if (tid < cb) {
+                const unsigned char* r = stage + (size_t)tid * srow;
+                for (uint32_t cl = 0; cl < w16; ++cl)
+                    replay_chunk(*reinterpret_cast<const uint4*>(r + 16 * cl), ch0 + cl, full, dim, s_qa, s_q16, s_lut, s, d, acc, s1, s2);
+            }
+            __syncthreads();
+        }
+        if (tid < cb) {
+            sbs[c0 + tid] = s;
+            fdots[c0 + tid] = d;
+            dots[c0 + tid] = 2 * acc - 255 * sum_cq;
+            norms[c0 + tid] = (int)(4u * s2 - 1020u * s1 + 65025u * dim);
+        }
+    }
+}
+
+__device__ inline SearchStatus fast_certificate(const FinalizeParams& p, uint32_t nc, uint32_t nonplateau, float kappa_k, float kappa_last) {
+    SearchStatus st;
+    st.n_candidates = nc;
+    st.reserved = 0;
+    st.need_exact = 0;
+    st.theta = 0.0f;
+    const u64 searchable = p.n_allowed ? *p.n_allowed : (u64)p.n;
+    if (searchable > nc) {
+        const bool plateau_reachable = p.max_dist > (double)PBX_PLATEAU_DIST && nonplateau < p.k;
+        const bool separated = (double)kappa_last < (double)kappa_k - (double)p.margin;
+        if (plateau_reachable) { st.need_exact = 1; st.theta = -__int_as_float(0x7f800000); }
+        else if (!separated) { st.need_exact = 1; st.theta = (float)((double)kappa_k - (double)p.margin - 1e-7); }
+    }
+    return st;
+}
+
+template <uint32_t NT>
 __device__ inline void block_order_keys(u64* buf, u64* sorted, uint32_t m) {
     const uint32_t tid = threadIdx.x;
-    if (m <= kFinalThreads) {
-        const uint32_t tpe = min(32u, (uint32_t)kFinalThreads / next_pow2(m < 2 ? 2 : m));
+    if (m <= NT) {
+        const uint32_t tpe = min(32u, NT / next_pow2(m < 2 ? 2 : m));
         const uint32_t e = tid / tpe, sub = tid - e * tpe;
         const u64 me = e < m ? buf[e] : 0ull;
         uint32_t rank = 0;
@@ -288,7 +360,7 @@
         for (uint32_t off = tpe >> 1; off; off >>= 1) rank += __shfl_xor_sync(0xFFFFFFFFu, rank, off);
         if (e < m && sub == 0) sorted[rank] = me;
         __syncthreads();
-    } else if (m <= 2 * kFinalThreads) {
+    } else if (m <= 2 * NT) {
         for (uint32_t t = tid; t < m; t += blockDim.x) {
             const u64 me = buf[t];
             uint32_t rank = 0;
@@ -323,11 +395,12 @@
     __syncthreads();
 }
 
+template <uint32_t NT>
 __device__ inline uint32_t block_candidates(u64* buf, u64* sorted, uint32_t m, uint32_t keep, uint32_t k, uint32_t cap,
                                             uint32_t* s_cnt, u64* s_tau, SelectScratch* s_sel, u64* s_scratch,
                                             float* s_kappa_k, float* s_kappa_last) {
-    if (m <= kFinalThreads) {
-        block_order_keys(buf, sorted, m);
+    if (m <= NT) {
+        block_order_keys<NT>(buf, sorted, m);
         const uint32_t nc = m < keep ? m : keep;
         if (threadIdx.x == 0) {
             *s_kappa_k = (nc >= k && k > 0) ? key64_kappa(sorted[k - 1]) : 0.0f;
@@ -470,7 +543,7 @@
             __syncthreads();
             PBX_FIN_STAMP(3);
             const uint32_t m = s_cnt;
-            nc = block_candidates(buf, sorted, m, p.keep, p.k, p.cap, &s_cnt, &s_tau, &s_sel, s_scratch64, &s_kappa_k, &s_kappa_last);
+            nc = block_candidates<kFinalThreads>(buf, sorted, m, p.keep, p.k, p.cap, &s_cnt, &s_tau, &s_sel, s_scratch64, &s_kappa_k, &s_kappa_last);
         } else {
             TopBuf<u64> tb{buf, &s_cnt, &s_tau, p.cap, p.keep};
             merge_rounds(p, tb, s_listcnt, s_maxcnt, &s_pushed);
@@ -499,7 +572,7 @@
             block_select_top(tb, &s_sel);
         }
         const uint32_t m = s_cnt;
-        nc = block_candidates(buf, sorted, m, p.keep, p.k, p.cap, &s_cnt, &s_tau, &s_sel, s_scratch64, &s_kappa_k, &s_kappa_last);
+        nc = block_candidates<kFinalThreads>(buf, sorted, m, p.keep, p.k, p.cap, &s_cnt, &s_tau, &s_sel, s_scratch64, &s_kappa_k, &s_kappa_last);
     }
 
     PBX_FIN_STAMP(4);
@@ -525,59 +598,13 @@
             qh_g->sa = sa;
         }
     }
-    const uint32_t pitch16 = p.pitch / 16, slice16 = p.slice16;
-    const uint32_t srow = ((slice16 + 1) | 1u) * 16;
-    const uint32_t full = p.dim >> 4;
-    const int sum_cq = qh_g->sum_cq;
-    constexpr uint32_t kStageBatch = 6;
     if (!BATCH && p.phase == 2) {
         for (uint32_t i = tid; i < nc; i += blockDim.x) {
             sbs[i] = p.x_sbs[i]; fdots[i] = p.x_fdots[i]; dots[i] = p.x_dots[i]; norms[i] = p.x_norms[i];
         }
-    } else
-    for (uint32_t c0 = 0; c0 < nc; c0 += p.stage_rows) {
-        const uint32_t cb = min(p.stage_rows, nc - c0);
-        float s = 0.0f, d = 0.0f;
-        int acc = 0;
-        unsigned s1 = 0, s2 = 0;
-        for (uint32_t ch0 = 0; ch0 < pitch16; ch0 += slice16) {
-            const uint32_t w16 = min(slice16, pitch16 - ch0);
-            const uint32_t total16 = cb * w16;
-            for (uint32_t e0 = tid; e0 < total16; e0 += kStageBatch * blockDim.x) {
-                uint4 v[kStageBatch];
-#pragma unroll
-                for (uint32_t u = 0; u < kStageBatch; ++u) {
-                    const uint32_t e = e0 + u * blockDim.x;
-                    if (e < total16) {
-                        const uint32_t ci = e / w16, ch = e - ci * w16;
-                        const uint32_t row = key64_row(sorted[c0 + ci]);
-                        v[u] = __ldg(reinterpret_cast<const uint4*>(p.rows + (size_t)row * p.pitch) + ch0 + ch);
-                    }
-                }
-#pragma unroll
-                for (uint32_t u = 0; u < kStageBatch; ++u) {
-                    const uint32_t e = e0 + u * blockDim.x;
-                    if (e < total16) {
-                        const uint32_t ci = e / w16, ch = e - ci * w16;
-                        *reinterpret_cast<uint4*>(stage + (size_t)ci * srow + 16 * ch) = v[u];
-                    }
-                }
-            }
-            __syncthreads();
-            PBX_FIN_STAMP(5);
-            if (tid < cb) {
-                const unsigned char* r = stage + (size_t)tid * srow;
-                for (uint32_t cl = 0; cl < w16; ++cl)
-                    replay_chunk(*reinterpret_cast<const uint4*>(r + 16 * cl), ch0 + cl, full, p.dim, s_qa, s_q16, s_lut, s, d, acc, s1, s2);
-            }
-            __syncthreads();
-        }
-        if (tid < cb) {
-            sbs[c0 + tid] = s;
-            fdots[c0 + tid] = d;
-            dots[c0 + tid] = 2 * acc - 255 * sum_cq;
-            norms[c0 + tid] = (int)(4u * s2 - 1020u * s1 + 65025u * p.dim);
-        }
+    } else {
+        replay_candidates(sorted, nc, p.stage_rows, p.slice16, p.pitch, p.dim, p.rows, s_qa, s_q16, s_lut, stage, qh_g->sum_cq,
+                          sbs, fdots, dots, norms);
     }
     __syncthreads();
     PBX_FIN_STAMP(6);
@@ -719,18 +746,7 @@
     if (tid == 0) {
         const uint32_t passing = s_cnt;
         *count_g = passing < p.k ? passing : p.k;
-        SearchStatus st;
-        st.n_candidates = nc;
-        st.reserved = 0;
-        st.need_exact = 0;
-        st.theta = 0.0f;
-        const u64 searchable = p.n_allowed ? *p.n_allowed : (u64)p.n;
-        if (searchable > nc) {
-            const bool plateau_reachable = p.max_dist > (double)PBX_PLATEAU_DIST && s_nonplateau < p.k;
-            const bool separated = (double)s_kappa_last < (double)s_kappa_k - (double)p.margin;
-            if (plateau_reachable) { st.need_exact = 1; st.theta = -__int_as_float(0x7f800000); }
-            else if (!separated) { st.need_exact = 1; st.theta = (float)((double)s_kappa_k - (double)p.margin - 1e-7); }
-        }
+        SearchStatus st = fast_certificate(p, nc, s_nonplateau, s_kappa_k, s_kappa_last);
         if constexpr (BATCH) {
             if (p.boverflow[q]) { st.need_exact = 1; st.theta = -__int_as_float(0x7f800000); }
         }
@@ -774,4 +790,195 @@
     }
 }
 
-}
+constexpr uint32_t kFinishKeys = 512;
+
+struct FastFinish {
+    FinalizeParams f;
+    uint32_t finish;
+    uint32_t fin_smem;
+    uint32_t stage_rows, slice16;
+    uint32_t off_sorted, off_dots, off_q, off_lut, off_stage;
+    unsigned long long* fallbacks;
+};
+
+__device__ inline void finish_publish(const FinalizeParams& p, bool exact_follows) {
+    if (p.done_flag && !exact_follows) {
+        __threadfence_system();
+        *reinterpret_cast<volatile uint32_t*>(p.done_flag) = p.done_seq;
+    }
+}
+
+__device__ __noinline__ void scan_finish(const FastFinish& x, unsigned char* smem) {
+    constexpr uint32_t NT = kScanThreads, BPT = kHistBins / NT;
+    const FinalizeParams& p = x.f;
+    u64* buf = reinterpret_cast<u64*>(smem);
+    u64* sorted = reinterpret_cast<u64*>(smem + x.off_sorted);
+    RerankEntry* ent = reinterpret_cast<RerankEntry*>(smem);
+    int* dots = reinterpret_cast<int*>(smem + x.off_dots);
+    int* norms = dots + p.keep;
+    float* dists = reinterpret_cast<float*>(norms + p.keep);
+    float* sbs = dists + p.keep;
+    float* fdots = sbs + p.keep;
+    float* s_qa = reinterpret_cast<float*>(smem + x.off_q);
+    int16_t* s_q16 = reinterpret_cast<int16_t*>(smem + x.off_q + 4 * p.pitch);
+    float* s_lut = reinterpret_cast<float*>(smem + x.off_lut);
+    unsigned char* stage = smem + x.off_stage;
+    __shared__ uint32_t f_cnt, f_bstar, f_mprime, f_total, f_nonplateau;
+    __shared__ uint32_t f_warp[NT / 32];
+    __shared__ u64 f_tau, f_scratch[NT / 32];
+    __shared__ float f_kappa_k, f_kappa_last, f_sa;
+    __shared__ SelectScratch f_sel;
+    const uint32_t tid = threadIdx.x, lane = tid & 31, warp = tid >> 5;
+
+    uint32_t h[BPT], mine = 0;
+#pragma unroll
+    for (uint32_t i = 0; i < BPT; i += 4) {
+        const uint4 v = __ldcg(reinterpret_cast<const uint4*>(p.hist + (size_t)tid * BPT + i));
+        h[i] = v.x; h[i + 1] = v.y; h[i + 2] = v.z; h[i + 3] = v.w;
+    }
+#pragma unroll
+    for (uint32_t i = 0; i < BPT; ++i) mine += h[i];
+    uint32_t incl = mine;
+#pragma unroll
+    for (int off = 1; off < 32; off <<= 1) {
+        const uint32_t v = __shfl_down_sync(0xFFFFFFFFu, incl, off);
+        if (lane + off < 32) incl += v;
+    }
+    if (lane == 0) f_warp[warp] = incl;
+    if (tid == 0) { f_cnt = 0; f_nonplateau = 0; f_bstar = 0; f_mprime = 0; f_tau = 0ull; p.tile_counter[112] = 0; }
+    __syncthreads();
+    uint32_t above = incl - mine;
+    for (uint32_t w = warp + 1; w < NT / 32; ++w) above += f_warp[w];
+    if (tid == 0) { uint32_t t = 0; for (uint32_t w = 0; w < NT / 32; ++w) t += f_warp[w]; f_total = t; }
+    if (above < p.keep && above + mine >= p.keep) {
+        uint32_t run = above;
+#pragma unroll
+        for (int i = BPT - 1; i >= 0; --i) {
+            run += h[i];
+            if (run >= p.keep) { f_bstar = tid * BPT + i; f_mprime = run; break; }
+        }
+    }
+    __syncthreads();
+    if (f_total < p.keep && tid == 0) { f_bstar = 0; f_mprime = f_total; }
+    __syncthreads();
+    const uint32_t mprime = f_mprime, bstar = f_bstar;
+    if (mprime > kFinishKeys) {
+        if (tid == 0) {
+            atomicAdd(x.fallbacks, 1ull);
+            bool launched = false;
+#ifdef PBX_USE_CDP
+            finalize_kernel<false><<<1, kFinalThreads, x.fin_smem, cudaStreamTailLaunch>>>(p);
+            launched = cudaGetLastError() == cudaSuccess;
+#endif
+            if (!launched) {
+                for (uint32_t i = 0; i < kHistBins; ++i) p.hist[i] = 0;
+                p.tile_counter[0] = 0;
+                p.tile_counter[32] = 0;
+                SearchStatus st; st.need_exact = 1; st.theta = -__int_as_float(0x7f800000); st.n_candidates = 0; st.reserved = 0;
+                *p.status = st;
+                *p.count = PBX_COUNT_EXACT_LAUNCH_FAILED;
+                finish_publish(p, false);
+            }
+        }
+        return;
+    }
+#pragma unroll
+    for (uint32_t i = 0; i < BPT; i += 4) reinterpret_cast<uint4*>(p.hist + (size_t)tid * BPT)[i / 4] = make_uint4(0, 0, 0, 0);
+
+    for (uint32_t b = tid; b < p.grid; b += NT) {
+        const uint32_t len = p.cand_cnt[b];
+        for (uint32_t r0 = 0; r0 < len; r0 += 4) {
+            u64 key[4];
+#pragma unroll
+            for (uint32_t i = 0; i < 4; ++i) key[i] = (r0 + i < len) ? p.cand[(size_t)(r0 + i) * p.grid + b] : 0ull;
+            uint32_t take = 0;
+#pragma unroll
+            for (uint32_t i = 0; i < 4; ++i)
+                if (take == i && r0 + i < len && kappa_bin(key64_kappa(key[i])) >= bstar) take = i + 1;
+            if (take) {
+                const uint32_t at = atomicAdd(&f_cnt, take);
+#pragma unroll
+                for (uint32_t i = 0; i < 4; ++i) if (i < take) buf[at + i] = key[i];
+            }
+            if (take < 4) break;
+        }
+    }
+    for (uint32_t i = tid; i < 256; i += NT) s_lut[i] = ref_decode(i);
+    for (uint32_t i = tid; i < p.pitch / 8; i += NT) reinterpret_cast<uint4*>(s_q16)[i] = __ldg(reinterpret_cast<const uint4*>(p.q16) + i);
+    __syncthreads();
+    for (uint32_t i = tid; i < p.pitch; i += NT) s_qa[i] = s_lut[p.qbytes[i]];
+    const uint32_t m = f_cnt;
+    const uint32_t nc = block_candidates<NT>(buf, sorted, m, p.keep, p.k, kFinishKeys, &f_cnt, &f_tau, &f_sel, f_scratch,
+                                             &f_kappa_k, &f_kappa_last);
+    {
+        float* sq = reinterpret_cast<float*>(buf);
+        for (uint32_t i = tid; i < p.dim; i += NT) { const float a = s_qa[i]; sq[i] = __fmul_rn(a, a); }
+        __syncthreads();
+        if (tid == NT - 1) {
+            float sa = 0.0f;
+            for (uint32_t i = 0; i < p.dim; ++i) sa = __fadd_rn(sa, sq[i]);
+            f_sa = sa;
+            p.qh->sa = sa;
+        }
+    }
+    replay_candidates(sorted, nc, x.stage_rows, x.slice16, p.pitch, p.dim, p.rows, s_qa, s_q16, s_lut, stage, p.qh->sum_cq,
+                      sbs, fdots, dots, norms);
+    __syncthreads();
+    const float sa = f_sa;
+    const int64_t my_id = tid < nc ? p.ids[key64_row(sorted[tid])] : INT64_MAX;
+    if (tid < nc) {
+        const float dist = ref_distance(sa, sbs[tid], fdots[tid]);
+        dists[tid] = dist;
+        RerankEntry e;
+        e.od = ord_f32(dist);
+        e.slot = tid;
+        e.id = my_id;
+        ent[tid] = e;
+        if (dist < PBX_PLATEAU_DIST) atomicAdd(&f_nonplateau, 1u);
+    }
+    if (tid == 0) f_cnt = 0;
+    __syncthreads();
+    {
+        const uint32_t tpe = min(32u, NT / next_pow2(nc < 2 ? 2 : nc));
+        const uint32_t c = tid / tpe, sub = tid - c * tpe;
+        RerankEntry me; me.od = 0; me.slot = 0; me.id = 0;
+        if (c < nc) me = ent[c];
+        uint32_t pos = 0;
+        if (c < nc) {
+#pragma unroll 4
+            for (uint32_t j = sub; j < nc; j += tpe) pos += rerank_before(ent[j], me) ? 1u : 0u;
+        }
+        for (uint32_t off = tpe >> 1; off; off >>= 1) pos += __shfl_xor_sync(0xFFFFFFFFu, pos, off);
+        if (c < nc && sub == 0) {
+            const float dist = dists[c];
+            const bool ok = (double)dist < p.max_dist;
+            if (ok) atomicAdd(&f_cnt, 1u);
+            if (pos < p.k) {
+                pbx_hit hh;
+                if (ok) { hh.image_id = me.id; hh.dist = dist; hh.dot = dots[c]; hh.norm2 = norms[c]; hh.flags = 0; }
+                else { hh.image_id = INT64_MAX; hh.dist = __int_as_float(0x7f800000); hh.dot = 0; hh.norm2 = 0; hh.flags = 0; }
+                p.hits[pos] = hh;
+            }
+        }
+    }
+    for (uint32_t c = nc + tid; c < p.k; c += NT) {
+        pbx_hit hh; hh.image_id = INT64_MAX; hh.dist = __int_as_float(0x7f800000); hh.dot = 0; hh.norm2 = 0; hh.flags = 0;
+        p.hits[c] = hh;
+    }
+    __syncthreads();
+    if (tid == 0) {
+        const uint32_t passing = f_cnt;
+        *p.count = passing < p.k ? passing : p.k;
+        const SearchStatus st = fast_certificate(p, nc, f_nonplateau, f_kappa_k, f_kappa_last);
+        *p.status = st;
+        p.tile_counter[0] = 0;
+        p.tile_counter[32] = 0;
+        bool exact_follows = st.need_exact != 0;
+#ifdef PBX_USE_CDP
+        if (st.need_exact) { __threadfence(); if (!launch_exact_tail(p.x)) { *p.count = PBX_COUNT_EXACT_LAUNCH_FAILED; exact_follows = false; } }
+#endif
+        finish_publish(p, exact_follows);
+    }
+}
+
+}
diff --git a/pixelbox_b200/csrc/scan.cuh b/pixelbox_b200/csrc/scan.cuh
--- a/pixelbox_b200/csrc/scan.cuh
+++ b/pixelbox_b200/csrc/scan.cuh
@@ -38,6 +38,12 @@
     const uint32_t* allow;
 };
 
+struct NoFinish {};
+struct FastFinish;
+template <bool EXACT> struct ScanFinish { using type = NoFinish; };
+template <> struct ScanFinish<false> { using type = FastFinish; };
+__device__ void scan_finish(const FastFinish& f, unsigned char* smem);
+
 __device__ __forceinline__ int dot16(const uint4& v, const int* q, int acc) {
     acc = dp2a_lo(q[0], v.x, acc); acc = dp2a_hi(q[1], v.x, acc);
     acc = dp2a_lo(q[2], v.y, acc); acc = dp2a_hi(q[3], v.y, acc);
@@ -155,7 +161,7 @@
 
 template <int L, int C, bool EXACT, int MINB = scan_minb(L * C), bool RAGGED = false, bool FILTER = false>
 __global__ void __launch_bounds__(kScanThreads, MINB)
-scan_kernel(const ScanParams p) {
+scan_kernel(const ScanParams p, const __grid_constant__ typename ScanFinish<EXACT>::type fin) {
     static_assert(!(FILTER && EXACT), "the exact pass tests the filter at run time");
     using K = typename std::conditional<EXACT, KeyX, u64>::type;
     constexpr int G = 32 / L;
@@ -166,7 +172,7 @@
     __shared__ ScanShared<K, EXACT> sh;
 
     pdl_wait();
-    pdl_trigger();
+    if constexpr (EXACT) pdl_trigger(); else if (!fin.finish) pdl_trigger();
     if constexpr (EXACT) {
         if (p.status->need_exact == 0) return;
         sh.lut[threadIdx.x & 255] = ref_decode(threadIdx.x & 255);
@@ -333,11 +339,23 @@
 #ifdef PBX_EXP_PROFILE
     if constexpr (!EXACT) PBX_PROF_ADD(4, clock64() - t_kernel0);
 #endif
+    if constexpr (!EXACT) {
+        if (fin.finish) {
+            __threadfence();
+            __syncthreads();
+            if (threadIdx.x == 0) sh.done = (atomicAdd(p.tile_counter + 112, 1u) == gridDim.x - 1) ? 1u : 0u;
+            __syncthreads();
+            if (sh.done) {
+                __threadfence();
+                scan_finish(fin, smem_raw);
+            }
+        }
+    }
 }
 
 template <bool EXACT>
 __global__ void __launch_bounds__(kScanThreads, 2)
-scan_generic_kernel(const ScanParams p) {
+scan_generic_kernel(const ScanParams p, const __grid_constant__ typename ScanFinish<EXACT>::type) {
     using K = typename std::conditional<EXACT, KeyX, u64>::type;
     extern __shared__ __align__(16) unsigned char smem_raw[];
     K* buf = reinterpret_cast<K*>(smem_raw);
```

Result: slower. 5972, median of 6 (-5.5%).
